# Prisma-Multimodal/ViT-Prisma

Measured on NVIDIA H100. Metric: SAE training tokens/sec (TopK SAE, d_model=768, dict=768x32, k=32), higher is better.
Workload: dtype fp32

## Files before the change

include/prisma_b200.h:

```cpp
#ifndef PRISMA_B200_H
#define PRISMA_B200_H

#include <stdint.h>

#ifdef __cplusplus
extern "C" {
#endif

typedef struct CUstream_st* pb_stream_t;

#if defined(__GNUC__)
#define PB_API __attribute__((visibility("default")))
#else
#define PB_API
#endif

enum { PB_OK = 0, PB_EINVAL = -1, PB_ECUDA = -2, PB_EUNSUPPORTED = -3, PB_ENODEVICE = -4 };
enum { PB_F32 = 0, PB_BF16 = 1 };
enum { PB_ACT_NONE = 0, PB_ACT_RELU = 1, PB_ACT_GELU = 2, PB_ACT_SILU = 3, PB_ACT_GELU_NEW = 4,
       PB_ACT_GELU_FAST = 5, PB_ACT_QUICK_GELU = 6, PB_ACT_TANH_RELU = 7, PB_ACT_EXP = 8 };
enum { PB_GEMM_AUTO = 0, PB_GEMM_SIMT = 1, PB_GEMM_TC = 2 };

PB_API int pb_version(void);
PB_API const char* pb_last_error(void);
PB_API unsigned long long pb_launch_count(void);
PB_API int pb_device_info(int* sm_count, int* cc_major, int* cc_minor);
PB_API int pb_abi_sizeof(int which);

typedef struct {
  int32_t M, N, K;
  int32_t dtype, act, impl;
  const void* A;  int64_t lda;
  const void* B;  int64_t ldb;
  const void* A_lo; const void* B_lo;
  const void* bias;
  const void* residual; int64_t ldr;
  void* out0; int64_t ld0;
  void* out1; int64_t ld1;
  float* out1_lo;
  int32_t n_split, split_n;
  void* out_split[4];
} PbGemm;
PB_API int pb_gemm(const PbGemm* g, pb_stream_t stream);
PB_API int pb_split_tf32(const float* x, float* lo, int64_t n, pb_stream_t stream);

typedef struct {
  int64_t rows; int32_t cols;
  int32_t dtype_in, dtype_out;
  float eps;
  const void* x; const void* w; const void* b;
  float* scale; float* norm_f32; void* out; float* out_lo;
  const float* scale_in;
} PbLayerNorm;
PB_API int pb_layernorm(const PbLayerNorm* p, pb_stream_t stream);

typedef struct {
  int32_t B, T, H, dh, dtype;
  float attn_scale;
  const void* q; const void* k; const void* v;
  void* scores; void* pattern; void* z;
} PbAttention;
PB_API int pb_attention(const PbAttention* p, pb_stream_t stream);
PB_API int pb_attn_scores(const PbAttention* p, pb_stream_t stream);
PB_API int pb_softmax_rows(const void* x, void* y, int64_t rows, int32_t cols, int32_t dtype,
                    pb_stream_t stream);
PB_API int pb_attn_pv(const PbAttention* p, pb_stream_t stream);

PB_API int pb_add(const void* a, const void* b, void* out, int64_t n, int32_t dtype, pb_stream_t s);
PB_API int pb_mul(const void* a, const void* b, void* out, int64_t n, int32_t dtype, pb_stream_t s);
PB_API int pb_activation(const void* x, void* y, int64_t n, int32_t act, int32_t dtype, pb_stream_t s);
PB_API int pb_l2_normalize_rows(const void* x, void* out, int64_t rows, int32_t cols, float eps,
                         int32_t dtype, pb_stream_t s);
PB_API int pb_mean_tokens(const void* x, void* out, int32_t B, int32_t T, int32_t d, int32_t dtype,
                   pb_stream_t s);
PB_API int pb_im2col_patches(const void* images, void* patches, int32_t B, int32_t C, int32_t S,
                      int32_t P, int32_t dtype, pb_stream_t s);
PB_API int pb_embed_assemble(const void* embed, const void* cls, const void* pos, void* full,
                      int32_t B, int32_t n_patches, int32_t d, int32_t use_cls, int32_t dtype,
                      pb_stream_t s);
PB_API int pb_cast(const void* x, int32_t dtype_in, void* y, int32_t dtype_out, int64_t n, pb_stream_t s);

typedef struct {
  const void *ln1_w, *ln1_b, *wqkv, *wqkv_lo, *bqkv, *wo, *wo_lo, *bo;
  const void *ln2_w, *ln2_b, *win, *win_lo, *bin, *wout, *wout_lo, *bout;
} PbVitLayerW;

typedef struct {
  float* ln1_scale;  float* ln1_norm_f32;  void* ln1_out;
  void *q, *k, *v;
  void *scores, *pattern;
  void* z;
  void* attn_out;    void* resid_mid;
  float* ln2_scale;  float* ln2_norm_f32;  void* ln2_out;
  void* pre;         void* post;
  void* mlp_out;     void* resid_post;
} PbVitLayerSpill;

typedef struct {
  int32_t batch, n_channels, image_size, patch_size, n_patches, n_tokens;
  int32_t d_model, n_heads, d_head, d_mlp, n_classes;
  int32_t n_layers_run;
  int32_t run_head;
  int32_t use_cls, layer_norm_pre, normalize_output, head_proj ;
  int32_t pool_gaap;
  int32_t act, dtype, gemm_impl;
  float eps, attn_scale;
  const void* images;
  const void *patch_w, *patch_w_lo, *patch_b, *cls, *pos;
  const void *lnpre_w, *lnpre_b, *lnf_w, *lnf_b, *head_w, *head_w_lo, *head_b;
  const PbVitLayerW* layers_host;
  void* patches;
  void* embed;
  void* full_embed;
  float* lnpre_scale; float* lnpre_norm_f32; void* lnpre_out;
  const PbVitLayerSpill* spills_host;
  float* lnf_scale; float* lnf_norm_f32; void* lnf_out;
  void* pooled;
  void* pre_normalize;
  void* out;
  float* lo_scratch;
} PbVitForward;
PB_API int pb_vit_forward(const PbVitForward* f, pb_stream_t stream);

typedef struct {
  int32_t rows, d, F, k;
  int32_t norm_mode;
  int32_t training;
  int32_t step;
  int32_t renorm_decoder;
  float lr, beta1, beta2, adam_eps, max_grad_norm ;
  const float* x;
  float* W_encT; float* W_encT_lo ; float* W_dec; float* b_enc; float* b_dec;
  float *sae_in, *mu, *sd, *xsum;
  int32_t* idx; float* val;
  float* feat_count;
  float *sae_out, *g, *dval;
  int32_t *csc_off, *csc_cursor, *csc_entries;
  float *gW_dec, *gW_encT, *gb_enc, *gb_dec;
  float *gcol, *gbdec2;
  float* fired;
  void* scalars;
  float *m_dec, *v_dec, *m_enc, *v_enc, *m_be, *v_be, *m_bd, *v_bd;
  float* since_fired; float* act_freq;
  int32_t global_rows; int32_t dist;
  void* work; int64_t work_bytes;
  float* enc_norm_max;
  int32_t pre_zeroed;
} PbSaeStep;

PB_API int pb_sae_prep(const float* x, const float* b_dec, float* sae_in, float* sae_in_lo, float* mu, float* sd,
                       float* xsum, int32_t rows, int32_t d, int32_t norm_mode, pb_stream_t stream);
PB_API int pb_sae_topk(const float* hidden_pre, int32_t rows, int32_t F, int32_t k, int32_t* idx, float* val,
                       float* feat_count, void* scratch, int64_t scratch_bytes, pb_stream_t stream);
PB_API int pb_sae_scatter_acts(const int32_t* idx, const float* val, float* dense, int32_t rows, int32_t k, int32_t F,
                               int32_t relu, pb_stream_t stream);
PB_API int pb_sae_step_reset(const PbSaeStep* s, int32_t* fb_count, pb_stream_t stream);
PB_API int pb_sae_decode(const PbSaeStep* s, pb_stream_t stream);
PB_API int pb_sae_backward(const PbSaeStep* s, pb_stream_t stream);
PB_API int pb_sae_adam(const PbSaeStep* s, pb_stream_t stream);
PB_API int pb_sae_mse(const float* x, const float* out, float* xsum_scratch, float* result, int32_t rows, int32_t d,
                      pb_stream_t stream);
PB_API int pb_unit_norm_rows(float* W, float* W_lo, int32_t F, int32_t d, pb_stream_t stream);

typedef struct {
  int32_t rows, d, F, k;
  int32_t c_keep;
  int32_t m_cand;
  int32_t phases;
  float err_coef;
  const float* sae_in;
  const float* W_encT;
  const float* b_enc;
  const float* enc_norm_max;
  int32_t* cand; int64_t cand_bytes;
  int32_t* idx; float* val;
  float* feat_count;
  int32_t* fb_count;
  int32_t* fb_rows;
  float* fb_scratch; int64_t fb_scratch_bytes;
} PbSaeEncode;
PB_API int pb_sae_fused_workspace(int32_t rows, int32_t F, int32_t c_keep, int64_t* cand_bytes, int64_t* fb_scratch_bytes);
PB_API int pb_sae_encode_topk_fused(const PbSaeEncode* e, pb_stream_t stream);
PB_API int pb_rownorm_max(const float* W, int32_t F, int32_t d, float* out, pb_stream_t stream);

PB_API int pb_transpose(const float* in, float* out, float* out_lo, int32_t rows, int32_t cols, pb_stream_t stream);
PB_API int pb_colsum(const float* x, float* out, int32_t rows, int32_t cols, int32_t accumulate, pb_stream_t stream);
PB_API int pb_gemv_rows(const float* W, const float* v, float* out, int32_t F, int32_t d, int32_t accumulate, pb_stream_t stream);
PB_API int pb_sae_dense_stats(const float* acts, int32_t rows, int32_t F, float* fired, float* l1_sum, void* scalars, pb_stream_t stream);
PB_API int pb_sae_dense_loss(const float* x, const float* out_n, const float* mu, const float* sd, const float* xsum, float* sae_out,
                             float* g, float* resid, void* scalars, int32_t rows, int32_t global_rows, int32_t d, int32_t norm_mode,
                             pb_stream_t stream);
PB_API int pb_sae_dense_dhid(float* d_acts, const float* acts, float* lo, float l1_grad, int64_t n, pb_stream_t stream);
PB_API int pb_sae_grad_finish(const float* gW_dec, const float* gW_encT, const float* gb_enc, const float* gb_dec, int32_t F, int32_t d,
                              void* scalars, float max_grad_norm, int32_t rows, pb_stream_t stream);
PB_API int pb_sae_ghost_gather(const float* hidden_pre, const int32_t* dead_idx, int32_t nd, int32_t rows, int32_t F, float* E, int32_t ldE,
                               pb_stream_t stream);
PB_API int pb_gather_rows(const float* W, const int32_t* idx, int32_t n, int32_t n_pad, int32_t d, float* out, pb_stream_t stream);
PB_API int pb_scatter_add_rows(float* dst, const int32_t* idx, int32_t n, int32_t d, const float* src, float scale, pb_stream_t stream);
PB_API int pb_mul_inplace(float* y, const float* x, int64_t n, pb_stream_t stream);
PB_API int pb_sae_ghost_rows(const float* resid, const float* rsum, float* G0, const void* scalars, float* ghost_sum, int32_t rows,
                             int32_t d, pb_stream_t stream);

PB_API int pb_gated_fwd(const float* pi, const float* b_gate, const float* r_mag, const float* b_mag, float* acts, float* acts_lo,
                        float* pi_act, float* pi_act_lo, float* fired, float* piact_colsum, void* scalars, int32_t rows, int32_t F,
                        pb_stream_t stream);
PB_API int pb_gated_aux(const float* via, const float* sae_in, float* ga, float* aux_sum, int32_t rows, int32_t d, pb_stream_t stream);
PB_API int pb_gated_bwd(float* d_acts, float* D_lo, const float* d_pia, const float* pi, const float* b_gate, const float* r_mag,
                        const float* b_mag, const float* wnorm, float l1_grad, float* gb_gate, float* gb_mag, float* gr_mag, float* dsum,
                        int32_t rows, int32_t F, pb_stream_t stream);
PB_API int pb_row_norms(const float* W, float* out, int32_t F, int32_t d, pb_stream_t stream);
PB_API int pb_gated_l1_rows(float* gW_dec, const float* W_dec, const float* piact_colsum, const float* wnorm, float l1_grad, float* l1_sum,
                            int32_t F, int32_t d, pb_stream_t stream);
PB_API int pb_sumsq(const float* a, int64_t n, float* acc, pb_stream_t stream);
PB_API int pb_sae_clip_finish(void* scalars, float max_grad_norm, int32_t rows, int32_t d, pb_stream_t stream);
PB_API int pb_adam_vec(float* p, const float* g, float* m, float* v, int32_t n, const void* scalars, float lr, float beta1, float beta2,
                       float eps, int32_t step, pb_stream_t stream);

#define PB_P2P_MAX_RANKS 8
typedef struct {
  int32_t rank, world, d, F, step, global_rows;
  float lr, beta1, beta2, adam_eps, max_grad_norm;
  float* gW_dec[PB_P2P_MAX_RANKS]; float* gW_encT[PB_P2P_MAX_RANKS]; float* gb_enc[PB_P2P_MAX_RANKS]; float* gb_dec[PB_P2P_MAX_RANKS];
  float* fired[PB_P2P_MAX_RANKS]; float* xsum[PB_P2P_MAX_RANKS];
  float* W_dec[PB_P2P_MAX_RANKS]; float* W_encT[PB_P2P_MAX_RANKS]; float* W_encT_lo[PB_P2P_MAX_RANKS]; float* b_enc[PB_P2P_MAX_RANKS];
  float* norm_parts[PB_P2P_MAX_RANKS]; uint32_t* flags[PB_P2P_MAX_RANKS];
  float *gb_enc_red, *gb_dec_red, *fired_red, *part_accum;
  float* b_dec; void* scalars;
  float *m_dec, *v_dec, *m_enc, *v_enc, *m_be, *v_be, *m_bd, *v_bd;
  float* since_fired; float* act_freq;
  const float *mc_gW_dec, *mc_gW_encT;
  float *mc_W_dec, *mc_W_encT, *mc_b_enc;
  int32_t defer_dec;
} PbP2PStep;
PB_API int pb_p2p_alloc(int64_t bytes, void** dev_ptr, unsigned char* handle64);
PB_API int pb_p2p_open(const unsigned char* handle64, void** peer_ptr);
PB_API int pb_p2p_close(void* peer_ptr);
PB_API int pb_p2p_free(void* dev_ptr);
PB_API int pb_p2p_barrier(const PbP2PStep* s, uint32_t epoch, pb_stream_t stream);
PB_API int pb_p2p_sum_xsum(const PbP2PStep* s, float* xsum_global, pb_stream_t stream);
PB_API int pb_p2p_reduce_scatter(const PbP2PStep* s, pb_stream_t stream);
PB_API int pb_p2p_adam_allgather(const PbP2PStep* s, pb_stream_t stream);
PB_API int pb_p2p_wmax(const PbP2PStep* s, float* enc_norm_max, pb_stream_t stream);
PB_API int pb_p2p_push_dec(const PbP2PStep* s, pb_stream_t stream);
PB_API int pb_mc_supported(int32_t* supported);
PB_API int pb_mc_round_size(int32_t world, int64_t bytes, int64_t* rounded);
PB_API int pb_mc_create(int32_t world, int64_t bytes, uint64_t* mc_handle, int32_t* fd);
PB_API int pb_mc_import(int32_t fd, uint64_t* mc_handle);
PB_API int pb_mc_add_device(uint64_t mc_handle);
PB_API int pb_mc_bind_alloc(uint64_t mc_handle, int64_t bytes, void** uc_ptr, void** mc_ptr, uint64_t* mem_handle);

#ifdef __cplusplus
}
#endif
#endif
```

vit-prisma_b200/csrc/common.cuh:

```cuda
#pragma once
#include <cuda_runtime.h>
#include <cuda_bf16.h>
#include <stdint.h>
#include <stdio.h>
#include <string.h>
#include <math.h>
#include "../../include/prisma_b200.h"

void pb_set_error(const char* fmt, ...);

#define PB_CHECK_ARG(cond, ...)                                   \
  do {                                                            \
    if (!(cond)) {                                                \
      pb_set_error(__VA_ARGS__);                                  \
      return PB_EINVAL;                                           \
    }                                                             \
  } while (0)

#define PB_CUDA(call)                                                                  \
  do {                                                                                 \
    cudaError_t e__ = (call);                                                          \
    if (e__ != cudaSuccess) {                                                          \
      pb_set_error("%s:%d: %s -> %s", __FILE__, __LINE__, #call, cudaGetErrorString(e__)); \
      return PB_ECUDA;                                                                 \
    }                                                                                  \
  } while (0)

extern unsigned long long g_pb_launches;

#define PB_LAUNCH_CHECK()                                                              \
  do {                                                                                 \
    ++g_pb_launches;                                                                   \
    cudaError_t e__ = cudaGetLastError();                                              \
    if (e__ != cudaSuccess) {                                                          \
      pb_set_error("%s:%d: kernel launch -> %s", __FILE__, __LINE__, cudaGetErrorString(e__)); \
      return PB_ECUDA;                                                                 \
    }                                                                                  \
  } while (0)

#define PB_TRY(expr)                \
  do {                              \
    int rc__ = (expr);              \
    if (rc__ != PB_OK) return rc__; \
  } while (0)

int pb_sm_count();

typedef __nv_bfloat16 bf16;

__device__ __forceinline__ float ld_as_float(const float* p) { return *p; }
__device__ __forceinline__ float ld_as_float(const bf16* p) { return __bfloat162float(*p); }
__device__ __forceinline__ void st_from_float(float* p, float v) { *p = v; }
__device__ __forceinline__ void st_from_float(bf16* p, float v) { *p = __float2bfloat16_rn(v); }
template <typename T> __device__ __forceinline__ float round_to(float v);
template <> __device__ __forceinline__ float round_to<float>(float v) { return v; }
template <> __device__ __forceinline__ float round_to<bf16>(float v) {
  return __bfloat162float(__float2bfloat16_rn(v));
}

struct alignas(8) bf16x4 { __nv_bfloat162 lo, hi; };
__device__ __forceinline__ void ld4(const float* p, float (&v)[4]) {
  float4 t = *reinterpret_cast<const float4*>(p);
  v[0] = t.x; v[1] = t.y; v[2] = t.z; v[3] = t.w;
}
__device__ __forceinline__ void ld4(const bf16* p, float (&v)[4]) {
  bf16x4 t = *reinterpret_cast<const bf16x4*>(p);
  float2 a = __bfloat1622float2(t.lo), b = __bfloat1622float2(t.hi);
  v[0] = a.x; v[1] = a.y; v[2] = b.x; v[3] = b.y;
}
__device__ __forceinline__ void st4(float* p, const float (&v)[4]) {
  *reinterpret_cast<float4*>(p) = make_float4(v[0], v[1], v[2], v[3]);
}
__device__ __forceinline__ void st4(bf16* p, const float (&v)[4]) {
  bf16x4 t;
  t.lo = __floats2bfloat162_rn(v[0], v[1]);
  t.hi = __floats2bfloat162_rn(v[2], v[3]);
  *reinterpret_cast<bf16x4*>(p) = t;
}

__device__ __forceinline__ float tf32_trunc(float x) {
  return __uint_as_float(__float_as_uint(x) & 0xFFFFE000u);
}
__device__ __forceinline__ float tf32_lo(float x) {
  uint32_t r;
  asm("cvt.rna.tf32.f32 %0, %1;" : "=r"(r) : "f"(x - tf32_trunc(x)));
  return __uint_as_float(r);
}

__device__ __forceinline__ float apply_act(float x, int act) {
  switch (act) {
    case PB_ACT_RELU: return fmaxf(x, 0.f);
    case PB_ACT_GELU: return 0.5f * x * (1.f + erff(x * 0.70710678118654752440f));
    case PB_ACT_SILU: return x / (1.f + expf(-x));
    case PB_ACT_GELU_NEW: {
      float inner = 0.79788456080286535588f * (x + 0.044715f * x * x * x);
      return 0.5f * x * (1.f + tanhf(inner));
    }
    case PB_ACT_GELU_FAST: return 0.5f * x * (1.f + tanhf(x * 0.7978845608f * (1.f + 0.044715f * x * x)));
    case PB_ACT_QUICK_GELU: return x / (1.f + expf(-1.702f * x));
    case PB_ACT_TANH_RELU: return tanhf(fmaxf(x, 0.f));
    case PB_ACT_EXP: return expf(x);
    default: return x;
  }
}

__device__ __forceinline__ float warp_sum(float v) {
#pragma unroll
  for (int o = 16; o > 0; o >>= 1) v += __shfl_xor_sync(0xffffffffu, v, o);
  return v;
}
__device__ __forceinline__ float warp_max(float v) {
#pragma unroll
  for (int o = 16; o > 0; o >>= 1) v = fmaxf(v, __shfl_xor_sync(0xffffffffu, v, o));
  return v;
}

static inline int64_t ceil_div64(int64_t a, int64_t b) { return (a + b - 1) / b; }

__device__ __forceinline__ void pb_pdl_trigger() { asm volatile("griddepcontrol.launch_dependents;"); }
__device__ __forceinline__ void pb_pdl_wait() { asm volatile("griddepcontrol.wait;" ::: "memory"); }
__device__ __forceinline__ void pb_pdl() { pb_pdl_trigger(); pb_pdl_wait(); }

bool pb_pdl_enabled();

template <typename... KArgs, typename... Args>
static inline cudaError_t pb_launch_pdl(void (*kern)(KArgs...), dim3 grid, dim3 block, size_t smem, cudaStream_t st, Args&&... args) {
  cudaLaunchConfig_t cfg;
  memset(&cfg, 0, sizeof(cfg));
  cfg.gridDim = grid;
  cfg.blockDim = block;
  cfg.dynamicSmemBytes = smem;
  cfg.stream = st;
  cudaLaunchAttribute attr[1];
  attr[0].id = cudaLaunchAttributeProgrammaticStreamSerialization;
  attr[0].val.programmaticStreamSerializationAllowed = 1;
  cfg.attrs = attr;
  cfg.numAttrs = pb_pdl_enabled() ? 1 : 0;
  return cudaLaunchKernelEx(&cfg, kern, static_cast<KArgs>(args)...);
}
#define PB_LAUNCH_PDL(kern, grid, block, smem, st, ...)                                  \
  do {                                                                                   \
    cudaError_t le__ = pb_launch_pdl(kern, dim3(grid), dim3(block), (size_t)(smem), st, __VA_ARGS__); \
    ++g_pb_launches;                                                                     \
    if (le__ != cudaSuccess) {                                                           \
      pb_set_error("%s:%d: kernel launch -> %s", __FILE__, __LINE__, cudaGetErrorString(le__)); \
      return PB_ECUDA;                                                                   \
    }                                                                                    \
  } while (0)
```

vit-prisma_b200/csrc/p2p.cu:

```cuda
#include "common.cuh"
#include "sae_optim.cuh"

#define PB_MAX_RANKS 8

__device__ __forceinline__ float4 mc_ld_reduce4(const float* mc_addr) {
  float4 v;
  asm volatile("multimem.ld_reduce.relaxed.sys.global.add.v4.f32 {%0, %1, %2, %3}, [%4];"
               : "=f"(v.x), "=f"(v.y), "=f"(v.z), "=f"(v.w)
               : "l"(mc_addr)
               : "memory");
  return v;
}
__device__ __forceinline__ void mc_st4(float* mc_addr, const float (&v)[4]) {
  asm volatile("multimem.st.global.v4.f32 [%0], {%1, %2, %3, %4};" ::"l"(mc_addr), "f"(v[0]), "f"(v[1]), "f"(v[2]), "f"(v[3]) : "memory");
}
__device__ __forceinline__ void mc_st1(float* mc_addr, float v) {
  asm volatile("multimem.st.global.f32 [%0], %1;" ::"l"(mc_addr), "f"(v) : "memory");
}

struct P2PTables {
  int rank, world;
  float* gW_dec[PB_MAX_RANKS];
  float* gW_encT[PB_MAX_RANKS];
  float* gb_enc[PB_MAX_RANKS];
// ... 34 lines not shown
  return PB_OK;
}

__global__ void k_p2p_barrier(P2PTables t, unsigned int epoch) {
  const int r = threadIdx.x;
  if (r < t.world) {
    __threadfence_system();
    asm volatile("st.release.sys.global.u32 [%0], %1;" ::"l"(t.flags[r] + t.rank), "r"(epoch) : "memory");
    const unsigned int* mine = t.flags[t.rank] + r;
    const long long t0 = clock64();
    for (;;) {
      unsigned int v;
      asm volatile("ld.acquire.sys.global.u32 %0, [%1];" : "=r"(v) : "l"(mine) : "memory");
      if ((int)(v - epoch) >= 0) break;
      if (clock64() - t0 > 20000000000LL) {
        printf("p2p barrier timeout: rank %d waiting for rank %d at epoch %u (have %u)\n", t.rank, r, epoch, v);
        __trap();
      }
    }
    __threadfence_system();
  }
}

__global__ void k_p2p_sum_small(P2PTables t, float* __restrict__ out, int which, int n) {
  for (int i = blockIdx.x * blockDim.x + threadIdx.x; i < n; i += gridDim.x * blockDim.x) {
    float acc = 0.f;
    for (int r = 0; r < t.world; ++r) {
      const float* src = which == 0 ? t.xsum[r] : which == 1 ? t.gb_enc[r] : which == 2 ? t.gb_dec[r] : t.fired[r];
      acc += src[i];
    }
    out[i] = acc;
  }
}

__global__ void __launch_bounds__(256) k_p2p_sum_small3(P2PTables t, float* __restrict__ gb_enc_red, float* __restrict__ gb_dec_red,
                                                       float* __restrict__ fired_red, int F, int d, float* __restrict__ part_accum) {
  if (blockIdx.x == 0 && threadIdx.x < 4) part_accum[threadIdx.x] = 0.f;
  const int n = 2 * F + d;
  for (int i = blockIdx.x * blockDim.x + threadIdx.x; i < n; i += gridDim.x * blockDim.x) {
    const int which = i < F ? 0 : i < 2 * F ? 1 : 2;
    const int j = which == 0 ? i : which == 1 ? i - F : i - 2 * F;
    float acc = 0.f;
    for (int r = 0; r < t.world; ++r) acc += (which == 0 ? t.gb_enc[r] : which == 1 ? t.fired[r] : t.gb_dec[r])[j];
    (which == 0 ? gb_enc_red : which == 1 ? fired_red : gb_dec_red)[j] = acc;
  }
}

template <int W, int U>
__device__ __forceinline__ float rs_peer_slice(const P2PTables& t, int m, int64_t base4, int64_t n4, float4* __restrict__ own, int64_t tid,
                                               int64_t stride) {
  const float4* src[W];
#pragma unroll
  for (int j = 0; j < W; ++j) {
    const int r = (t.rank + j) % t.world;
    src[j] = j < t.world ? reinterpret_cast<const float4*>(m == 0 ? t.gW_dec[r] : t.gW_encT[r]) + base4 : nullptr;
  }
  float nsq = 0.f;
  int64_t i = tid;
  for (; i + (U - 1) * stride < n4; i += U * stride) {
    float4 v[U][W];
#pragma unroll
    for (int u = 0; u < U; ++u)
#pragma unroll
      for (int r = 0; r < W; ++r)
        if (r < t.world) v[u][r] = src[r][i + u * stride];
#pragma unroll
    for (int u = 0; u < U; ++u) {
      float4 acc = v[u][0];
#pragma unroll
      for (int r = 1; r < W; ++r)
        if (r < t.world) { acc.x += v[u][r].x; acc.y += v[u][r].y; acc.z += v[u][r].z; acc.w += v[u][r].w; }
      own[i + u * stride] = acc;
      nsq += acc.x * acc.x + acc.y * acc.y + acc.z * acc.z + acc.w * acc.w;
    }
  }
  for (; i < n4; i += stride) {
    float4 acc = src[0][i];
#pragma unroll
    for (int r = 1; r < W; ++r)
      if (r < t.world) { const float4 b = src[r][i]; acc.x += b.x; acc.y += b.y; acc.z += b.z; acc.w += b.w; }
    own[i] = acc;
    nsq += acc.x * acc.x + acc.y * acc.y + acc.z * acc.z + acc.w * acc.w;
  }
  return nsq;
}

template <int W, int U>
__global__ void __launch_bounds__(256, 3) k_p2p_reduce_scatter(P2PTables t, int f0, int f1, int d, const float* __restrict__ gb_enc_red,
                                                              const float* __restrict__ gb_dec_red, int F, float* __restrict__ part_accum,
                                                              const float* __restrict__ mc_gW_dec, const float* __restrict__ mc_gW_encT) {
  const int64_t n4 = (int64_t)(f1 - f0) * d / 4;
  const int64_t base4 = (int64_t)f0 * d / 4;
  float nsq = 0.f;
  const int64_t tid = (int64_t)blockIdx.x * blockDim.x + threadIdx.x, stride = (int64_t)gridDim.x * blockDim.x;
  for (int m = 0; m < 2; ++m) {
    float4* own = reinterpret_cast<float4*>(m == 0 ? t.gW_dec[t.rank] : t.gW_encT[t.rank]) + base4;
    const float* mc = m == 0 ? mc_gW_dec : mc_gW_encT;
    if constexpr (W == 0) {
      const float* src = mc + 4 * base4;
      int64_t i = tid;
      for (; i + 3 * stride < n4; i += 4 * stride) {
        const float4 a0 = mc_ld_reduce4(src + 4 * i), a1 = mc_ld_reduce4(src + 4 * (i + stride)), a2 = mc_ld_reduce4(src + 4 * (i + 2 * stride)),
                     a3 = mc_ld_reduce4(src + 4 * (i + 3 * stride));
        own[i] = a0; own[i + stride] = a1; own[i + 2 * stride] = a2; own[i + 3 * stride] = a3;
        nsq += a0.x * a0.x + a0.y * a0.y + a0.z * a0.z + a0.w * a0.w + a1.x * a1.x + a1.y * a1.y + a1.z * a1.z + a1.w * a1.w +
               a2.x * a2.x + a2.y * a2.y + a2.z * a2.z + a2.w * a2.w + a3.x * a3.x + a3.y * a3.y + a3.z * a3.z + a3.w * a3.w;
      }
      for (; i < n4; i += stride) {
        const float4 a = mc_ld_reduce4(src + 4 * i);
        own[i] = a;
        nsq += a.x * a.x + a.y * a.y + a.z * a.z + a.w * a.w;
      }
      continue;
    }
    if constexpr (W != 0) nsq += rs_peer_slice<W, U>(t, m, base4, n4, own, tid, stride);
  }
  if (t.rank == 0) {
    for (int i = blockIdx.x * blockDim.x + threadIdx.x; i < F; i += gridDim.x * blockDim.x) nsq += gb_enc_red[i] * gb_enc_red[i];
    for (int i = blockIdx.x * blockDim.x + threadIdx.x; i < d; i += gridDim.x * blockDim.x) nsq += gb_dec_red[i] * gb_dec_red[i];
  }
  nsq = warp_sum(nsq);
  __shared__ float red[8];
  if ((threadIdx.x & 31) == 0) red[threadIdx.x >> 5] = nsq;
  __syncthreads();
  if (threadIdx.x == 0) {
    float a = 0.f;
    for (int i = 0; i < 8; ++i) a += red[i];
    atomicAdd(part_accum, a);
  }
}
__global__ void k_p2p_publish_norm(P2PTables t, float* part_accum) {
  const int r = threadIdx.x;
  if (r < t.world) t.norm_parts[r][t.rank] = *part_accum;
}

__global__ void k_p2p_finalize(P2PTables t, SaeScalars* sc, float max_norm, float inv_elems_global, float inv_rows_global) {
  float tot = 0.f;
  for (int r = 0; r < t.world; ++r) tot += t.norm_parts[t.rank][r];
  sae_publish_scalars(sc, tot, max_norm, inv_elems_global, inv_rows_global);
}

struct AdamPeerOut {
  float* const (&wdec_rot)[PB_MAX_RANKS];
  float* const (&wenc_rot)[PB_MAX_RANKS];
  float* const (&wlo_rot)[PB_MAX_RANKS];
  float *own_dec, *mc_W_dec, *mc_W_encT;
  int world, defer_dec;
  int64_t base;
  __device__ __forceinline__ void dec(int c4, const float (&w)[4]) const {
    if (defer_dec) st4(own_dec + base + 4 * c4, w);
    else if (mc_W_dec) mc_st4(mc_W_dec + base + 4 * c4, w);
    else for (int j = 0; j < world; ++j) st4(wdec_rot[j] + base + 4 * c4, w);
  }
  __device__ __forceinline__ void enc(int c4, const float (&p)[4], const float (&lo)[4]) const {
    if (mc_W_encT) {
      mc_st4(mc_W_encT + base + 4 * c4, p);
    } else {
      for (int j = 0; j < world; ++j) {
        st4(wenc_rot[j] + base + 4 * c4, p);
        if (wlo_rot[j]) st4(wlo_rot[j] + base + 4 * c4, lo);
      }
    }
  }
};

template <int CHUNKS>
__global__ void __launch_bounds__(256) k_p2p_adam_allgather(P2PTables t, int f0, int f1, int d, const float* __restrict__ gb_enc_red,
                                                           float* __restrict__ m_dec, float* __restrict__ v_dec, float* __restrict__ m_enc,
                                                           float* __restrict__ v_enc, float* __restrict__ m_be, float* __restrict__ v_be,
                                                           const SaeScalars* __restrict__ sc, AdamHyper h, float* __restrict__ mc_W_dec,
                                                           float* __restrict__ mc_W_encT, float* __restrict__ mc_b_enc, float* __restrict__ wmax_accum,
                                                           int defer_dec) {
  const int lane = threadIdx.x & 31, warp = threadIdx.x >> 5, nw = blockDim.x >> 5;
  float enc_best = 0.f, enc_best_lo = 0.f;
  const int nvec = d >> 2;
  const float clip = sc->clip_coef;
  float* W_dec = t.W_dec[t.rank];
  float* W_encT = t.W_encT[t.rank];
  const float* gWd = t.gW_dec[t.rank];
  const float* gWe = t.gW_encT[t.rank];
  float *wdec_rot[PB_MAX_RANKS], *wenc_rot[PB_MAX_RANKS], *wlo_rot[PB_MAX_RANKS];
#pragma unroll
  for (int j = 0; j < PB_MAX_RANKS; ++j) {
    const int r = (t.rank + j) % t.world;
    wdec_rot[j] = t.W_dec[r]; wenc_rot[j] = t.W_encT[r]; wlo_rot[j] = t.W_encT_lo[r];
  }
  for (int f = f0 + blockIdx.x * nw + warp; f < f1; f += gridDim.x * nw) {
    const int64_t base = (int64_t)f * d;
    float esq, elo;
    sae_adam_feature<CHUNKS>(W_dec + base, gWd + base, m_dec + base, v_dec + base, W_encT + base, gWe + base, m_enc + base, v_enc + base,
                             clip, h, nvec, true,
                             AdamPeerOut{wdec_rot, wenc_rot, wlo_rot, W_dec, mc_W_dec, mc_W_encT, t.world, defer_dec, base}, esq, elo);
    enc_best = fmaxf(enc_best, warp_sum(esq));
    enc_best_lo = fmaxf(enc_best_lo, warp_sum(elo));
    if (lane == 0) {
      float mm = m_be[f], vv = v_be[f];
      const float nb = adam_update(t.b_enc[t.rank][f], gb_enc_red[f] * clip, mm, vv, h);
      m_be[f] = mm;
      v_be[f] = vv;
      if (mc_b_enc) mc_st1(mc_b_enc + f, nb);
      else for (int r = 0; r < t.world; ++r) t.b_enc[r][f] = nb;
    }
  }
  if (wmax_accum && lane == 0 && enc_best > 0.f) {
    atomicMax(reinterpret_cast<unsigned int*>(wmax_accum), __float_as_uint(sqrtf(enc_best)));
    atomicMax(reinterpret_cast<unsigned int*>(wmax_accum) + 1, __float_as_uint(sqrtf(enc_best_lo)));
  }
}

__global__ void k_p2p_wmax_reduce(P2PTables t, float* __restrict__ enc_norm_max) {
  float a = 0.f, b = 0.f;
  for (int r = 0; r < t.world; ++r) {
    a = fmaxf(a, t.norm_parts[t.rank][PB_MAX_RANKS + r]);
    b = fmaxf(b, t.norm_parts[t.rank][2 * PB_MAX_RANKS + r]);
  }
  enc_norm_max[0] = a;
  enc_norm_max[1] = b;
}

__global__ void __launch_bounds__(256) k_p2p_small_updates(P2PTables t, const float* __restrict__ wmax_accum, float* __restrict__ b_dec,
                                                          const float* __restrict__ gb_dec_red, float* __restrict__ m_bd,
                                                          float* __restrict__ v_bd, const float* __restrict__ fired_red,
                                                          float* __restrict__ since_fired, float* __restrict__ act_freq,
                                                          const SaeScalars* __restrict__ sc, AdamHyper h, int d, int F) {
  if (blockIdx.x == 0 && threadIdx.x < t.world) {
    t.norm_parts[threadIdx.x][PB_MAX_RANKS + t.rank] = wmax_accum[0];
    t.norm_parts[threadIdx.x][2 * PB_MAX_RANKS + t.rank] = wmax_accum[1];
  }
  const float clip = sc->clip_coef;
  for (int i = blockIdx.x * blockDim.x + threadIdx.x; i < max(F, d); i += gridDim.x * blockDim.x) {
    if (i < d) {
      float mm = m_bd[i], vv = v_bd[i];
      b_dec[i] = adam_update(b_dec[i], gb_dec_red[i] * clip, mm, vv, h);
      m_bd[i] = mm;
      v_bd[i] = vv;
    }
    if (i < F) dead_feature_counters(since_fired, act_freq, i, fired_red[i], since_fired ? since_fired[i] : 0.f, act_freq ? act_freq[i] : 0.f);
  }
}

static int fill_tables(const PbP2PStep* s, P2PTables* t) {
  PB_CHECK_ARG(s && s->world >= 1 && s->world <= PB_MAX_RANKS && s->rank >= 0 && s->rank < s->world, "pb_p2p: bad rank/world");
  t->rank = s->rank;
  t->world = s->world;
  for (int r = 0; r < s->world; ++r) {
    t->gW_dec[r] = s->gW_dec[r]; t->gW_encT[r] = s->gW_encT[r]; t->gb_enc[r] = s->gb_enc[r]; t->gb_dec[r] = s->gb_dec[r];
    t->fired[r] = s->fired[r]; t->xsum[r] = s->xsum[r]; t->W_dec[r] = s->W_dec[r]; t->W_encT[r] = s->W_encT[r];
    t->W_encT_lo[r] = s->W_encT_lo[r]; t->b_enc[r] = s->b_enc[r]; t->norm_parts[r] = s->norm_parts[r]; t->flags[r] = s->flags[r];
  }
  return PB_OK;
}

extern "C" int pb_p2p_barrier(const PbP2PStep* s, uint32_t epoch, pb_stream_t stream) {
  P2PTables t;
  PB_TRY(fill_tables(s, &t));
  k_p2p_barrier<<<1, 32, 0, (cudaStream_t)stream>>>(t, epoch);
  PB_LAUNCH_CHECK();
  return PB_OK;
}

extern "C" int pb_p2p_sum_xsum(const PbP2PStep* s, float* xsum_global, pb_stream_t stream) {
  P2PTables t;
  PB_TRY(fill_tables(s, &t));
  k_p2p_sum_small<<<(s->d + 255) / 256, 256, 0, (cudaStream_t)stream>>>(t, xsum_global, 0, s->d);
  PB_LAUNCH_CHECK();
  return PB_OK;
}

extern "C" int pb_p2p_reduce_scatter(const PbP2PStep* s, pb_stream_t stream) {
  P2PTables t;
  PB_TRY(fill_tables(s, &t));
  PB_CHECK_ARG(s->gb_enc_red && s->gb_dec_red && s->fired_red && s->part_accum, "pb_p2p_reduce_scatter: reduction buffers missing");
  PB_CHECK_ARG((s->F % s->world) == 0 && (((int64_t)(s->F / s->world) * s->d) % 4) == 0, "pb_p2p_reduce_scatter: F must divide evenly by world");
  cudaStream_t st = (cudaStream_t)stream;
  const int per = s->F / s->world, f0 = s->rank * per, f1 = f0 + per;
  k_p2p_sum_small3<<<(2 * s->F + s->d + 255) / 256, 256, 0, st>>>(t, s->gb_enc_red, s->gb_dec_red, s->fired_red, s->F, s->d, s->part_accum);
  PB_LAUNCH_CHECK();
  PB_CHECK_ARG(!s->mc_gW_dec == !s->mc_gW_encT, "pb_p2p_reduce_scatter: both multicast gradient views or none");
#define PB_RS(W_, U_) k_p2p_reduce_scatter<W_, U_><<<pb_sm_count() * 3, 256, 0, st>>>(t, f0, f1, s->d, s->gb_enc_red, s->gb_dec_red, s->F, s->part_accum, s->mc_gW_dec, s->mc_gW_encT)
  if (s->mc_gW_dec) PB_RS(0, 0);
  else if (s->world == 2) PB_RS(2, 4);
  else if (s->world == 4) PB_RS(4, 2);
  else if (s->world == 8) PB_RS(8, 1);
  else PB_RS(PB_MAX_RANKS, 1);
#undef PB_RS
  PB_LAUNCH_CHECK();
  k_p2p_publish_norm<<<1, 32, 0, st>>>(t, s->part_accum);
  PB_LAUNCH_CHECK();
  return PB_OK;
}

extern "C" int pb_p2p_adam_allgather(const PbP2PStep* s, pb_stream_t stream) {
  P2PTables t;
  PB_TRY(fill_tables(s, &t));
  PB_CHECK_ARG(s->m_dec && s->v_dec && s->m_enc && s->v_enc && s->m_be && s->v_be && s->m_bd && s->v_bd && s->scalars && s->b_dec,
               "pb_p2p_adam_allgather: optimizer state missing");
  PB_CHECK_ARG(s->step >= 1, "pb_p2p_adam_allgather: step counter starts at 1");
  cudaStream_t st = (cudaStream_t)stream;
  const int per = s->F / s->world, f0 = s->rank * per, f1 = f0 + per;
  const AdamHyper h = adam_hyper(s->lr, s->beta1, s->beta2, s->adam_eps, s->step);
  k_p2p_finalize<<<1, 1, 0, st>>>(t, (SaeScalars*)s->scalars, s->max_grad_norm, 1.f / ((float)s->global_rows * (float)s->d),
                                  1.f / (float)s->global_rows);
  PB_LAUNCH_CHECK();
  const int d = s->d;
  int grid = pb_sm_count() * 4;
  if (grid > (per + 7) / 8) grid = (per + 7) / 8;
  PB_CHECK_ARG((!s->mc_W_dec == !s->mc_W_encT) && (!s->mc_W_dec == !s->mc_b_enc), "pb_p2p_adam_allgather: all three multicast parameter views or none");
  PB_DISPATCH_CHUNKS(chunks_for(d), (k_p2p_adam_allgather<C_><<<grid, 256, 0, st>>>(t, f0, f1, d, s->gb_enc_red, s->m_dec, s->v_dec, s->m_enc,
                                     s->v_enc, s->m_be, s->v_be, (const SaeScalars*)s->scalars, h, s->mc_W_dec, s->mc_W_encT, s->mc_b_enc,
                                     s->part_accum + 1, s->defer_dec)));
  PB_LAUNCH_CHECK();
  k_p2p_small_updates<<<((s->F > d ? s->F : d) + 255) / 256, 256, 0, st>>>(t, s->part_accum + 1, s->b_dec, s->gb_dec_red, s->m_bd, s->v_bd, s->fired_red, s->since_fired,
                                                        s->act_freq, (const SaeScalars*)s->scalars, h, d, s->F);
  PB_LAUNCH_CHECK();
  return PB_OK;
}

__global__ void __launch_bounds__(256) k_p2p_push_dec(P2PTables t, int f0, int f1, int d, float* __restrict__ mc_W_dec) {
  const int64_t n4 = (int64_t)(f1 - f0) * d / 4, base4 = (int64_t)f0 * d / 4;
  const float4* own = reinterpret_cast<const float4*>(t.W_dec[t.rank]) + base4;
  for (int64_t i = (int64_t)blockIdx.x * blockDim.x + threadIdx.x; i < n4; i += (int64_t)gridDim.x * blockDim.x) {
    const float4 v = own[i];
    if (mc_W_dec) {
      const float w[4] = {v.x, v.y, v.z, v.w};
      mc_st4(mc_W_dec + 4 * (base4 + i), w);
    } else {
      for (int j = 1; j < t.world; ++j)
        (reinterpret_cast<float4*>(t.W_dec[(t.rank + j) % t.world]) + base4)[i] = v;
    }
  }
}

extern "C" int pb_p2p_push_dec(const PbP2PStep* s, pb_stream_t stream) {
  P2PTables t;
  PB_TRY(fill_tables(s, &t));
  const int per = s->F / s->world, f0 = s->rank * per, f1 = f0 + per;
  k_p2p_push_dec<<<pb_sm_count() * 2, 256, 0, (cudaStream_t)stream>>>(t, f0, f1, s->d, s->mc_W_dec);
  PB_LAUNCH_CHECK();
  return PB_OK;
}

extern "C" int pb_p2p_wmax(const PbP2PStep* s, float* enc_norm_max, pb_stream_t stream) {
  P2PTables t;
  PB_TRY(fill_tables(s, &t));
  PB_CHECK_ARG(enc_norm_max, "pb_p2p_wmax: output missing");
// ... 8 lines not shown
```

vit-prisma_b200/csrc/sae.cu:

```cuda
#include "common.cuh"
#include "tc_common.cuh"
#include "sae_optim.cuh"

template <int CHUNKS>
__global__ void __launch_bounds__(256) k_sae_prep(const float* __restrict__ x, const float* __restrict__ b_dec, float* __restrict__ sae_in,
                                                  float* __restrict__ sae_in_lo, float* __restrict__ mu_out, float* __restrict__ std_out,
                                                  int rows, int d, int norm_mode, float eps) {
  pb_pdl();
  const int lane = threadIdx.x & 31;
  const int row = blockIdx.x * (blockDim.x >> 5) + (threadIdx.x >> 5);
  if (row >= rows) return;
  const int nvec = d >> 2;
  const float* xr = x + (int64_t)row * d;
  float v[CHUNKS][4];
  float sum = 0.f;
#pragma unroll
  for (int i = 0; i < CHUNKS; ++i) {
    const int c4 = i * 32 + lane;
    if (c4 < nvec) { ld4(xr + 4 * c4, v[i]); sum += (v[i][0] + v[i][1]) + (v[i][2] + v[i][3]); }
    else v[i][0] = v[i][1] = v[i][2] = v[i][3] = 0.f;
  }
  float mu = 0.f, inv = 1.f, sd = 1.f;
  if (norm_mode == 1) {
    mu = warp_sum(sum) / (float)d;
    float sq = 0.f;
#pragma unroll
    for (int i = 0; i < CHUNKS; ++i) {
      const int c4 = i * 32 + lane;
      if (c4 < nvec) {
#pragma unroll
        for (int j = 0; j < 4; ++j) { v[i][j] -= mu; sq += v[i][j] * v[i][j]; }
      }
    }
    sd = sqrtf(warp_sum(sq) / (float)(d - 1));
    inv = 1.f / (sd + eps);
  } else if (norm_mode == 2) {
    float sq = 0.f;
#pragma unroll
    for (int i = 0; i < CHUNKS; ++i)
#pragma unroll
      for (int j = 0; j < 4; ++j) sq += v[i][j] * v[i][j];
    sd = sqrtf(warp_sum(sq)) / sqrtf((float)d);
    inv = 1.f / sd;
  }
  if (lane == 0) {
    if (mu_out) mu_out[row] = mu;
    if (std_out) std_out[row] = sd;
  }
#pragma unroll
  for (int i = 0; i < CHUNKS; ++i) {
    const int c4 = i * 32 + lane;
    if (c4 < nvec) {
      float bd[4], o[4], lo[4];
      ld4(b_dec + 4 * c4, bd);
#pragma unroll
      for (int j = 0; j < 4; ++j) {
        o[j] = (norm_mode == 1 ? v[i][j] / (sd + eps) : v[i][j] * inv) - bd[j];
        lo[j] = tf32_lo(o[j]);
      }
      (void)inv;
      st4(sae_in + (int64_t)row * d + 4 * c4, o);
      if (sae_in_lo) st4(sae_in_lo + (int64_t)row * d + 4 * c4, lo);
    }
  }
}

__global__ void __launch_bounds__(256) k_colsum(const float* __restrict__ x, float* __restrict__ out, int rows, int d, int rows_per_cta) {
  pb_pdl();
  const int r0 = blockIdx.x * rows_per_cta, r1 = min(rows, r0 + rows_per_cta);
  for (int c = threadIdx.x; c < d; c += blockDim.x) {
    float acc = 0.f;
    for (int r = r0; r < r1; ++r) acc += x[(int64_t)r * d + c];
    atomicAdd(out + c, acc);
  }
}

__device__ __forceinline__ bool key_gt(float va, int ia, float vb, int ib) { return va > vb || (va == vb && ia < ib); }

template <int IPT>
__global__ void __launch_bounds__(256) k_topk(const float* __restrict__ vals, const int* __restrict__ idx_map, int64_t row_stride, int F,
                                              int seg_len, int k, int* __restrict__ out_idx, float* __restrict__ out_val,
                                              int64_t out_row_stride, float* __restrict__ feat_count, int cand_cap) {
  extern __shared__ __align__(16) unsigned char smem_raw[];
  float* best_v = reinterpret_cast<float*>(smem_raw);
  int* best_i = reinterpret_cast<int*>(best_v + 256);
  float* cand_v = reinterpret_cast<float*>(best_i + 256);
  int* cand_i = reinterpret_cast<int*>(cand_v + cand_cap);
  __shared__ float tau_v;
  __shared__ int tau_i, cand_n;
  const int t = threadIdx.x;
  const int row = blockIdx.x, seg = blockIdx.y;
  const int s0 = seg * seg_len, s1 = min(F, s0 + seg_len);
  const float* vr = vals + (int64_t)row * row_stride;
  const int* mr = idx_map ? idx_map + (int64_t)row * row_stride : nullptr;

  float v[IPT];
  float bv = -INFINITY;
  int bi = 0x7fffffff;
#pragma unroll
  for (int i = 0; i < IPT; ++i) {
    const int p = s0 + t + 256 * i;
    v[i] = p < s1 ? vr[p] : -INFINITY;
    const int gi = p < s1 ? (mr ? mr[p] : p) : 0x7fffffff;
    if (key_gt(v[i], gi, bv, bi)) { bv = v[i]; bi = gi; }
  }
  best_v[t] = bv;
  best_i[t] = bi;
  if (t == 0) cand_n = 0;
  __syncthreads();
  {
    int rank = 0;
    for (int j = 0; j < 256; ++j) rank += key_gt(best_v[j], best_i[j], bv, bi) ? 1 : 0;
    const int kk = min(k, 256);
    if (rank == kk - 1) { tau_v = bv; tau_i = bi; }
  }
  __syncthreads();
  const float tv = tau_v;
  const int ti = tau_i;
#pragma unroll
  for (int i = 0; i < IPT; ++i) {
    const int p = s0 + t + 256 * i;
    if (p < s1) {
      const int gi = mr ? mr[p] : p;
      if (!key_gt(tv, ti, v[i], gi)) {
        const int slot = atomicAdd(&cand_n, 1);
        if (slot < cand_cap) { cand_v[slot] = v[i]; cand_i[slot] = gi; }
      }
    }
  }
  __syncthreads();
  const int C = min(cand_n, cand_cap);
  for (int c = t; c < C; c += 256) {
    const float cv = cand_v[c];
    const int ci = cand_i[c];
    int rank = 0;
    for (int j = 0; j < C; ++j) rank += key_gt(cand_v[j], cand_i[j], cv, ci) ? 1 : 0;
    if (rank < k) {
      const int64_t o = (int64_t)row * out_row_stride + (int64_t)seg * k + rank;
      out_idx[o] = ci;
      out_val[o] = cv;
      if (feat_count) atomicAdd(feat_count + ci, 1.0f);
    }
  }
  if (C < k) {
    for (int r = C + t; r < k; r += 256) {
      const int64_t o = (int64_t)row * out_row_stride + (int64_t)seg * k + r;
      out_idx[o] = 0x7fffffff;
      out_val[o] = -INFINITY;
    }
  }
}

__global__ void __launch_bounds__(256) k_scatter_acts(const int* __restrict__ idx, const float* __restrict__ val, float* __restrict__ dense,
                                                      int rows, int k, int F, int relu) {
  const int64_t n = (int64_t)rows * k;
  for (int64_t e = (int64_t)blockIdx.x * blockDim.x + threadIdx.x; e < n; e += (int64_t)gridDim.x * blockDim.x) {
    const int r = (int)(e / k);
    float v = val[e];
    if (relu) v = fmaxf(v, 0.f);
    dense[(int64_t)r * F + idx[e]] = v;
  }
}

template <int CHUNKS>
__global__ void __launch_bounds__(256) k_sae_decode(const float* __restrict__ x, const float* __restrict__ xsum, const float* __restrict__ mu,
                                                    const float* __restrict__ sd, const int* __restrict__ idx, const float* __restrict__ val,
                                                    const float* __restrict__ W_dec, const float* __restrict__ b_dec,
                                                    float* __restrict__ sae_out, float* __restrict__ g_out, float* __restrict__ dval,
                                                    SaeScalars* __restrict__ sc, int rows, int d, int k, int norm_mode, int training,
                                                    float inv_rows) {
  pb_pdl();
  const int lane = threadIdx.x & 31;
  const int row = blockIdx.x * (blockDim.x >> 5) + (threadIdx.x >> 5);
  const bool active = row < rows;
  const int nvec = d >> 2;
  float loss_part = 0.f, pos_part = 0.f;
  if (active) {
    const int* ir = idx + (int64_t)row * k;
    const float* vr = val + (int64_t)row * k;
    float acc[CHUNKS][4];
#pragma unroll
    for (int i = 0; i < CHUNKS; ++i) {
      const int c4 = i * 32 + lane;
      if (c4 < nvec) ld4(b_dec + 4 * c4, acc[i]);
      else acc[i][0] = acc[i][1] = acc[i][2] = acc[i][3] = 0.f;
    }
    for (int j0 = 0; j0 < k; j0 += 32) {
      const int jn = min(32, k - j0);
      const int my_i = lane < jn ? ir[j0 + lane] : 0;
      const float my_a = lane < jn ? fmaxf(vr[j0 + lane], 0.f) : 0.f;
      pos_part += (float)__popc(__ballot_sync(0xffffffffu, my_a > 0.f));
#pragma unroll 4
      for (int j = 0; j < jn; ++j) {
        const float a = __shfl_sync(0xffffffffu, my_a, j);
        const float* wr = W_dec + (int64_t)__shfl_sync(0xffffffffu, my_i, j) * d;
#pragma unroll
        for (int i = 0; i < CHUNKS; ++i) {
          const int c4 = i * 32 + lane;
          if (c4 < nvec) {
            float w[4];
            ld4(wr + 4 * c4, w);
#pragma unroll
            for (int q = 0; q < 4; ++q) acc[i][q] = fmaf(a, w[q], acc[i][q]);
          }
        }
      }
    }
    const float m = norm_mode ? mu[row] : 0.f;
    const float s = norm_mode ? sd[row] : 1.f;
    float nsq = 0.f;
    float e[CHUNKS][4];
#pragma unroll
    for (int i = 0; i < CHUNKS; ++i) {
      const int c4 = i * 32 + lane;
      if (c4 < nvec) {
// ... 256 lines not shown
    const int c4 = i * 32 + lane;
    if (c4 < nvec) {
#pragma unroll
      for (int q = 0; q < 4; ++q)
        if (bd[i][q] != 0.f) atomicAdd(&sm_bd[4 * c4 + q], bd[i][q]);
    }
  }
  nsq = warp_sum(nsq);
  __shared__ float red[8];
  if (lane == 0) red[warp] = nsq;
  __syncthreads();
  if (threadIdx.x == 0) {
    float a = 0.f;
    for (int i = 0; i < nw; ++i) a += red[i];
    atomicAdd(&sc->gnorm_sq, a);
  }
  for (int c = threadIdx.x; c < d; c += blockDim.x)
    if (sm_bd[c] != 0.f) atomicAdd(gbdec2 + c, sm_bd[c]);
}

template <int CHUNKS>
__global__ void __launch_bounds__(256) k_sae_grads_long(const int* __restrict__ off, const int* __restrict__ entries, const float* __restrict__ val,
                                                        const float* __restrict__ dval, const float* __restrict__ g,
                                                        const float* __restrict__ sae_in, const float* __restrict__ W_encT,
                                                        float* __restrict__ gW_dec, float* __restrict__ gW_encT, float* __restrict__ gb_enc,
                                                        float* __restrict__ gbdec2, float* __restrict__ fired, int d, int k,
                                                        const SaeWorkHeader* __restrict__ work, const int* __restrict__ work_chunks) {
  pb_pdl();
  extern __shared__ __align__(16) float sm_bd[];
  const int lane = threadIdx.x & 31, warp = threadIdx.x >> 5, nw = blockDim.x >> 5;
  const int nvec = d >> 2;
  const int n_items = work->n_chunks;
  if (n_items == 0) return;
  for (int c = threadIdx.x; c < d; c += blockDim.x) sm_bd[c] = 0.f;
  __syncthreads();
  float bd[CHUNKS][4];
#pragma unroll
  for (int i = 0; i < CHUNKS; ++i) bd[i][0] = bd[i][1] = bd[i][2] = bd[i][3] = 0.f;
  for (int item = blockIdx.x * nw + warp; item < n_items; item += gridDim.x * nw) {
    const int f = work_chunks[2 * item], p0 = work_chunks[2 * item + 1];
    const int p1 = min(off[f + 1], p0 + SAE_LONG_CHUNK);
    float ad[CHUNKS][4], ae[CHUNKS][4];
#pragma unroll
    for (int i = 0; i < CHUNKS; ++i) ad[i][0] = ad[i][1] = ad[i][2] = ad[i][3] = ae[i][0] = ae[i][1] = ae[i][2] = ae[i][3] = 0.f;
    const int n = p1 - p0;
    int my_b = 0;
    float my_a = 0.f, my_dp = 0.f;
    if (lane < n) {
      const int e = entries[p0 + lane];
      my_b = e / k;
      my_a = fmaxf(val[e], 0.f);
      my_dp = dval[e];
    }
    float gbe = 0.f;
    const float npos = (float)__popc(__ballot_sync(0xffffffffu, my_a > 0.f));
#pragma unroll 2
    for (int j = 0; j < n; ++j) {
      const float a = __shfl_sync(0xffffffffu, my_a, j), dp = __shfl_sync(0xffffffffu, my_dp, j);
      const int b = __shfl_sync(0xffffffffu, my_b, j);
      gbe += dp;
      const float* gr = g + (int64_t)b * d;
      const float* sr = sae_in + (int64_t)b * d;
#pragma unroll
      for (int i = 0; i < CHUNKS; ++i) {
        const int c4 = i * 32 + lane;
        if (c4 < nvec) {
          float gv[4], sv[4];
          ld4(gr + 4 * c4, gv);
          ld4(sr + 4 * c4, sv);
#pragma unroll
          for (int q = 0; q < 4; ++q) { ad[i][q] = fmaf(a, gv[q], ad[i][q]); ae[i][q] = fmaf(dp, sv[q], ae[i][q]); }
        }
      }
    }
#pragma unroll
    for (int i = 0; i < CHUNKS; ++i) {
      const int c4 = i * 32 + lane;
      if (c4 < nvec) {
        atomicAdd(reinterpret_cast<float4*>(gW_dec + (int64_t)f * d + 4 * c4), make_float4(ad[i][0], ad[i][1], ad[i][2], ad[i][3]));
        atomicAdd(reinterpret_cast<float4*>(gW_encT + (int64_t)f * d + 4 * c4), make_float4(ae[i][0], ae[i][1], ae[i][2], ae[i][3]));
        if (gbe != 0.f) {
          float w[4];
          ld4(W_encT + (int64_t)f * d + 4 * c4, w);
#pragma unroll
          for (int q = 0; q < 4; ++q) bd[i][q] = fmaf(gbe, w[q], bd[i][q]);
        }
      }
    }
    if (lane == 0) {
      atomicAdd(gb_enc + f, gbe);
      atomicAdd(fired + f, npos);
    }
  }
#pragma unroll
  for (int i = 0; i < CHUNKS; ++i) {
    const int c4 = i * 32 + lane;
    if (c4 < nvec) {
#pragma unroll
      for (int q = 0; q < 4; ++q)
        if (bd[i][q] != 0.f) atomicAdd(&sm_bd[4 * c4 + q], bd[i][q]);
    }
  }
  __syncthreads();
  for (int c = threadIdx.x; c < d; c += blockDim.x)
    if (sm_bd[c] != 0.f) atomicAdd(gbdec2 + c, sm_bd[c]);
}

__global__ void __launch_bounds__(256) k_sae_norm_long(const float* __restrict__ gW_dec, const float* __restrict__ gW_encT,
                                                       const float* __restrict__ gb_enc, SaeScalars* __restrict__ sc, int d,
                                                       const SaeWorkHeader* work, const int* __restrict__ work_feats) {
  pb_pdl();
  const int lane = threadIdx.x & 31, warp = threadIdx.x >> 5, nw = blockDim.x >> 5;
  const int n = *reinterpret_cast<const volatile int*>(&work->n_long);
  float nsq = 0.f;
  for (int li = blockIdx.x * nw + warp; li < n; li += gridDim.x * nw) {
    const int f = work_feats[li];
    for (int c = lane; c < d; c += 32) {
      const float a = gW_dec[(int64_t)f * d + c], b = gW_encT[(int64_t)f * d + c];
      nsq += a * a + b * b;
    }
    if (lane == 0) nsq += gb_enc[f] * gb_enc[f];
  }
  nsq = warp_sum(nsq);
  if (lane == 0 && nsq != 0.f) atomicAdd(&sc->gnorm_sq, nsq);
}

__global__ void k_sae_gbdec(const float* __restrict__ gcol, const float* __restrict__ gbdec2, float* __restrict__ gb_dec, int d) {
  const int c = blockIdx.x * blockDim.x + threadIdx.x;
  if (c < d) gb_dec[c] = gcol[c] - gbdec2[c];
}

__global__ void __launch_bounds__(256) k_sae_finalize(const float* __restrict__ gcol, const float* __restrict__ gbdec2, float* __restrict__ gb_dec,
                                                      SaeScalars* __restrict__ sc, int d, float max_norm, float inv_elems, float inv_rows) {
  pb_pdl();
  __shared__ float red[8];
  float s = 0.f;
  for (int c = threadIdx.x; c < d; c += blockDim.x) {
    const float v = gcol[c] - gbdec2[c];
    gb_dec[c] = v;
    s += v * v;
  }
  s = warp_sum(s);
  if ((threadIdx.x & 31) == 0) red[threadIdx.x >> 5] = s;
  __syncthreads();
  if (threadIdx.x == 0) {
    float t = sc->gnorm_sq;
    for (int i = 0; i < 8; ++i) t += red[i];
    sae_publish_scalars(sc, t, max_norm, inv_elems, inv_rows);
  }
}

struct AdamRowsOut {
  float *W_dec, *W_encT, *W_encT_lo;
  int64_t base;
  __device__ __forceinline__ void dec(int c4, const float (&w)[4]) const { st4(W_dec + base + 4 * c4, w); }
  __device__ __forceinline__ void enc(int c4, const float (&p)[4], const float (&lo)[4]) const {
    st4(W_encT + base + 4 * c4, p);
    if (W_encT_lo) st4(W_encT_lo + base + 4 * c4, lo);
  }
};

template <int CHUNKS>
__global__ void __launch_bounds__(256) k_sae_adam_rows(float* __restrict__ W_dec, float* __restrict__ W_encT, float* __restrict__ W_encT_lo,
                                                       float* __restrict__ b_enc, const float* __restrict__ gW_dec,
                                                       const float* __restrict__ gW_encT, const float* __restrict__ gb_enc,
                                                       float* __restrict__ m_dec, float* __restrict__ v_dec, float* __restrict__ m_enc,
                                                       float* __restrict__ v_enc, float* __restrict__ m_be, float* __restrict__ v_be,
                                                       const float* __restrict__ fired, float* __restrict__ since_fired,
                                                       float* __restrict__ act_freq, const SaeScalars* __restrict__ sc, AdamHyper h,
                                                       int F, int d, int renorm, float* __restrict__ enc_norm_max) {
  const int lane = threadIdx.x & 31, warp = threadIdx.x >> 5, nw = blockDim.x >> 5;
  const int nvec = d >> 2;
  const float clip = sc->clip_coef;
  float enc_best = 0.f, enc_best_lo = 0.f;
  for (int f = blockIdx.x * nw + warp; f < F; f += gridDim.x * nw) {
    const int64_t base = (int64_t)f * d;
    float esq, elo;
    sae_adam_feature<CHUNKS>(W_dec + base, gW_dec + base, m_dec + base, v_dec + base, W_encT + base, gW_encT + base, m_enc + base,
                             v_enc + base, clip, h, nvec, renorm, AdamRowsOut{W_dec, W_encT, W_encT_lo, base}, esq, elo);
    if (enc_norm_max) { enc_best = fmaxf(enc_best, warp_sum(esq)); enc_best_lo = fmaxf(enc_best_lo, warp_sum(elo)); }
    if (lane == 0) {
      float mm = m_be[f], vv = v_be[f];
      b_enc[f] = adam_update(b_enc[f], gb_enc[f] * clip, mm, vv, h);
      m_be[f] = mm;
      v_be[f] = vv;
      dead_feature_counters(since_fired, act_freq, f, fired[f], since_fired ? since_fired[f] : 0.f, act_freq ? act_freq[f] : 0.f);
    }
  }
  if (enc_norm_max && lane == 0 && enc_best > 0.f) {
    atomicMax(reinterpret_cast<unsigned int*>(enc_norm_max), __float_as_uint(sqrtf(enc_best)));
    atomicMax(reinterpret_cast<unsigned int*>(enc_norm_max) + 1, __float_as_uint(sqrtf(enc_best_lo)));
  }
}

constexpr int AB_MAX_STAGES = 12;
constexpr int AB_THREADS = 32 * (1 + AB_MAX_STAGES);

struct AdamSlotOut {
  float *wd, *we;
  __device__ __forceinline__ void dec(int c4, const float (&w)[4]) const { st4(wd + 4 * c4, w); }
  __device__ __forceinline__ void enc(int c4, const float (&p)[4], const float (&)[4]) const { st4(we + 4 * c4, p); }
};

__device__ __forceinline__ void bulk_load(uint32_t dst, const void* src, uint32_t bytes, uint32_t bar) {
  asm volatile("cp.async.bulk.shared::cluster.global.mbarrier::complete_tx::bytes [%0], [%1], %2, [%3];" ::"r"(dst), "l"(src), "r"(bytes), "r"(bar)
               : "memory");
}
__device__ __forceinline__ void bulk_store(void* dst, uint32_t src, uint32_t bytes) {
  asm volatile("cp.async.bulk.global.shared::cta.bulk_group [%0], [%1], %2;" ::"l"(dst), "r"(src), "r"(bytes) : "memory");
}

template <int CHUNKS>
__global__ void __launch_bounds__(AB_THREADS, 1)
k_sae_adam_bulk(float* __restrict__ W_dec, float* __restrict__ W_encT, float* __restrict__ b_enc, const float* __restrict__ gW_dec,
                const float* __restrict__ gW_encT, const float* __restrict__ gb_enc, float* __restrict__ m_dec, float* __restrict__ v_dec,
                float* __restrict__ m_enc, float* __restrict__ v_enc, float* __restrict__ m_be, float* __restrict__ v_be,
                const float* __restrict__ fired, float* __restrict__ since_fired, float* __restrict__ act_freq,
                const SaeScalars* __restrict__ sc, AdamHyper h, int F, int d, int renorm, float* __restrict__ enc_norm_max, int S,
                float* __restrict__ b_dec, const float* __restrict__ gb_dec, float* __restrict__ m_bd, float* __restrict__ v_bd) {
  pb_pdl_trigger();
  extern __shared__ __align__(128) unsigned char ab_smem[];
  const uint32_t s0 = smem_u32(ab_smem);
  const uint32_t row_bytes = (uint32_t)d * 4u, stage_bytes = 8u * row_bytes;
  auto full_bar = [&](int s) { return s0 + 8u * s; };
  auto empty_bar = [&](int s) { return s0 + 8u * (S + s); };
  const uint32_t data0 = s0 + 256u;
  float* data_generic = reinterpret_cast<float*>(ab_smem + 256);
  const int warp = threadIdx.x >> 5, lane = threadIdx.x & 31;
  const int n_mine = F > (int)blockIdx.x ? (F - (int)blockIdx.x + (int)gridDim.x - 1) / (int)gridDim.x : 0;
  if (threadIdx.x == 0) {
    for (int s = 0; s < S; ++s) { mbar_init(full_bar(s), 1); mbar_init(empty_bar(s), 1); }
    asm volatile("fence.mbarrier_init.release.cluster;" ::: "memory");
  }
  __syncthreads();
  pb_pdl_wait();
  if (warp == 0) {
    if (blockIdx.x == 0 && b_dec) {
      const float clip0 = sc->clip_coef;
      for (int c = lane; c < d; c += 32) {
        float mm = m_bd[c], vv = v_bd[c];
        b_dec[c] = adam_update(b_dec[c], gb_dec[c] * clip0, mm, vv, h);
        m_bd[c] = mm;
        v_bd[c] = vv;
      }
    }
    if (lane == 0) {
      for (int i = 0; i < n_mine; ++i) {
        const int s = i % S;
        const uint32_t ph = (uint32_t)(i / S) & 1u;
        const int64_t base = (int64_t)(blockIdx.x + (int64_t)i * gridDim.x) * d;
        mbar_wait(empty_bar(s), ph ^ 1u);
        mbar_expect_tx(full_bar(s), stage_bytes);
        const uint32_t dst = data0 + (uint32_t)s * stage_bytes;
        bulk_load(dst + 0 * row_bytes, W_dec + base, row_bytes, full_bar(s));
        bulk_load(dst + 1 * row_bytes, gW_dec + base, row_bytes, full_bar(s));
        bulk_load(dst + 2 * row_bytes, m_dec + base, row_bytes, full_bar(s));
        bulk_load(dst + 3 * row_bytes, v_dec + base, row_bytes, full_bar(s));
        bulk_load(dst + 4 * row_bytes, W_encT + base, row_bytes, full_bar(s));
        bulk_load(dst + 5 * row_bytes, gW_encT + base, row_bytes, full_bar(s));
        bulk_load(dst + 6 * row_bytes, m_enc + base, row_bytes, full_bar(s));
        bulk_load(dst + 7 * row_bytes, v_enc + base, row_bytes, full_bar(s));
      }
    }
    return;
  }
  const int nvec = d >> 2;
  const float clip = sc->clip_coef;
  float enc_best = 0.f, enc_best_lo = 0.f;
  for (int i = warp - 1; i < n_mine; i += S) {
    const int s = i % S;
    const uint32_t ph = (uint32_t)(i / S) & 1u;
    const int f = blockIdx.x + i * gridDim.x;
    const int64_t base = (int64_t)f * d;
    float be = 0.f, gbe = 0.f, mbe = 0.f, vbe = 0.f, fr = 0.f, sf = 0.f, af = 0.f;
    if (lane == 0) {
      be = b_enc[f]; gbe = gb_enc[f]; mbe = m_be[f]; vbe = v_be[f]; fr = fired[f];
      if (since_fired) sf = since_fired[f];
      if (act_freq) af = act_freq[f];
    }
    mbar_wait(full_bar(s), ph);
    float* st = data_generic + (size_t)s * 8 * d;
    float esq, elo;
    sae_adam_feature<CHUNKS>(st, st + d, st + 2 * d, st + 3 * d, st + 4 * d, st + 5 * d, st + 6 * d, st + 7 * d, clip, h, nvec, renorm,
                             AdamSlotOut{st, st + 4 * d}, esq, elo);
    enc_best = fmaxf(enc_best, warp_sum(esq));
    enc_best_lo = fmaxf(enc_best_lo, warp_sum(elo));
    __syncwarp();
    asm volatile("fence.proxy.async.shared::cta;" ::: "memory");
    __syncwarp();
    if (lane == 0) {
      const uint32_t src = data0 + (uint32_t)s * stage_bytes;
      bulk_store(W_dec + base, src + 0 * row_bytes, row_bytes);
      bulk_store(m_dec + base, src + 2 * row_bytes, row_bytes);
      bulk_store(v_dec + base, src + 3 * row_bytes, row_bytes);
      bulk_store(W_encT + base, src + 4 * row_bytes, row_bytes);
      bulk_store(m_enc + base, src + 6 * row_bytes, row_bytes);
      bulk_store(v_enc + base, src + 7 * row_bytes, row_bytes);
      asm volatile("cp.async.bulk.commit_group;" ::: "memory");
      b_enc[f] = adam_update(be, gbe * clip, mbe, vbe, h);
      m_be[f] = mbe;
      v_be[f] = vbe;
      dead_feature_counters(since_fired, act_freq, f, fr, sf, af);
      asm volatile("cp.async.bulk.wait_group.read 0;" ::: "memory");
      mbar_arrive(empty_bar(s));
    }
  }
  if (enc_norm_max && lane == 0 && enc_best > 0.f) {
    atomicMax(reinterpret_cast<unsigned int*>(enc_norm_max), __float_as_uint(sqrtf(enc_best)));
    atomicMax(reinterpret_cast<unsigned int*>(enc_norm_max) + 1, __float_as_uint(sqrtf(enc_best_lo)));
  }
  asm volatile("cp.async.bulk.wait_group 0;" ::: "memory");
}

__global__ void __launch_bounds__(256) k_sae_adam_vec(float* __restrict__ p, const float* __restrict__ g, float* __restrict__ m,
                                                      float* __restrict__ v, const SaeScalars* __restrict__ sc, AdamHyper h, int n) {
  const float clip = sc->clip_coef;
  for (int i = blockIdx.x * blockDim.x + threadIdx.x; i < n; i += gridDim.x * blockDim.x) {
    float mm = m[i], vv = v[i];
    p[i] = adam_update(p[i], g[i] * clip, mm, vv, h);
    m[i] = mm;
    v[i] = vv;
  }
}

template <int CHUNKS>
__global__ void __launch_bounds__(256) k_unit_rows(float* __restrict__ W, float* __restrict__ W_lo, int F, int d) {
  const int lane = threadIdx.x & 31, warp = threadIdx.x >> 5, nw = blockDim.x >> 5;
  const int nvec = d >> 2;
  for (int f = blockIdx.x * nw + warp; f < F; f += gridDim.x * nw) {
    float w[CHUNKS][4];
    float nsq = 0.f;
#pragma unroll
    for (int i = 0; i < CHUNKS; ++i) {
      const int c4 = i * 32 + lane;
      if (c4 < nvec) {
        ld4(W + (int64_t)f * d + 4 * c4, w[i]);
#pragma unroll
        for (int q = 0; q < 4; ++q) nsq += w[i][q] * w[i][q];
      }
    }
    const float nrm = sqrtf(warp_sum(nsq));
#pragma unroll
    for (int i = 0; i < CHUNKS; ++i) {
      const int c4 = i * 32 + lane;
      if (c4 < nvec) {
        float lo[4];
#pragma unroll
        for (int q = 0; q < 4; ++q) { w[i][q] = w[i][q] / nrm; lo[q] = tf32_lo(w[i][q]); }
        st4(W + (int64_t)f * d + 4 * c4, w[i]);
        if (W_lo) st4(W_lo + (int64_t)f * d + 4 * c4, lo);
      }
    }
  }
}

static int persistent_grid(int warps_per_cta, int items) {
  int ctas = pb_sm_count() * 4;
  const int need = (items + warps_per_cta - 1) / warps_per_cta;
  if (ctas > need) ctas = need;
  return ctas < 1 ? 1 : ctas;
}

extern "C" int pb_sae_prep(const float* x, const float* b_dec, float* sae_in, float* sae_in_lo, float* mu, float* sd, float* xsum, int32_t rows,
                           int32_t d, int32_t norm_mode, pb_stream_t stream) {
  PB_CHECK_ARG(x && b_dec && sae_in && rows >= 0 && d > 0, "pb_sae_prep: bad arguments");
  PB_CHECK_ARG(norm_mode == 0 || (mu && sd), "pb_sae_prep: mu/std buffers required when normalising");
  if (rows == 0) return PB_OK;
  cudaStream_t st = (cudaStream_t)stream;
  const int ch = chunks_for(d);
  PB_DISPATCH_CHUNKS(ch, PB_LAUNCH_PDL(k_sae_prep<C_>, (rows + 7) / 8, 256, 0, st, x, b_dec, sae_in, sae_in_lo, mu, sd, rows, d, norm_mode, 1e-5f));
  if (xsum) {
    PB_CUDA(cudaMemsetAsync(xsum, 0, sizeof(float) * d, st));
    const int rpc = 8;
    k_colsum<<<(rows + rpc - 1) / rpc, 256, 0, st>>>(x, xsum, rows, d, rpc);
    PB_LAUNCH_CHECK();
  }
  return PB_OK;
}

static int launch_topk(const float* vals, const int* map, int64_t row_stride, int F, int seg_len, int nseg, int k, int* oi, float* ov,
                       int64_t out_stride, float* feat_count, int rows, cudaStream_t st) {
  const int ipt_needed = (seg_len + 255) / 256;
  const int ipt = ipt_needed <= 8 ? 8 : ipt_needed <= 24 ? 24 : ipt_needed <= 48 ? 48 : 96;
  int cap = ipt * k;
  if (cap > seg_len) cap = seg_len;
  if (cap < k) cap = k;
  const size_t smem = 256 * 8 + (size_t)cap * 8;
  if (smem > 200 * 1024) { pb_set_error("pb_sae_topk: k=%d too large for the candidate buffer", k); return PB_EUNSUPPORTED; }
  dim3 grid(rows, nseg);
#define PB_TOPK(IPT)                                                                                                      \
  do {                                                                                                                    \
    auto kern = k_topk<IPT>;                                                                                              \
    if (smem > 48 * 1024) PB_CUDA(cudaFuncSetAttribute(kern, cudaFuncAttributeMaxDynamicSharedMemorySize, (int)smem));    \
    kern<<<grid, 256, smem, st>>>(vals, map, row_stride, F, seg_len, k, oi, ov, out_stride, feat_count, cap);             \
  } while (0)
  if (ipt == 8) PB_TOPK(8);
  else if (ipt == 24) PB_TOPK(24);
  else if (ipt == 48) PB_TOPK(48);
  else PB_TOPK(96);
#undef PB_TOPK
  PB_LAUNCH_CHECK();
  return PB_OK;
}

extern "C" int pb_sae_topk(const float* hidden_pre, int32_t rows, int32_t F, int32_t k, int32_t* idx, float* val, float* feat_count,
                           void* scratch, int64_t scratch_bytes, pb_stream_t stream) {
  PB_CHECK_ARG(hidden_pre && idx && val && rows >= 0 && F > 0 && k > 0 && k <= F, "pb_sae_topk: bad arguments");
  PB_CHECK_ARG(k <= 256, "pb_sae_topk: k=%d > 256 unsupported", k);
  if (rows == 0) return PB_OK;
  cudaStream_t st = (cudaStream_t)stream;
  const int SEG = 256 * 96;
  if (F <= SEG) return launch_topk(hidden_pre, nullptr, F, F, F, 1, k, idx, val, k, feat_count, rows, st);
  const int nseg = (F + SEG - 1) / SEG;
  const int seg_len = ((F + nseg - 1) / nseg + 255) / 256 * 256;
  const int64_t need = (int64_t)rows * nseg * k * 8;
  PB_CHECK_ARG(scratch && scratch_bytes >= need, "pb_sae_topk: scratch too small (%lld < %lld)", (long long)scratch_bytes, (long long)need);
  int* ci = (int*)scratch;
  float* cv = (float*)(ci + (int64_t)rows * nseg * k);
  PB_TRY(launch_topk(hidden_pre, nullptr, F, F, seg_len, nseg, k, ci, cv, (int64_t)nseg * k, nullptr, rows, st));
  return launch_topk(cv, ci, (int64_t)nseg * k, nseg * k, nseg * k, 1, k, idx, val, k, feat_count, rows, st);
}

extern "C" int pb_sae_scatter_acts(const int32_t* idx, const float* val, float* dense, int32_t rows, int32_t k, int32_t F, int32_t relu,
                                   pb_stream_t stream) {
  PB_CHECK_ARG(idx && val && dense && rows >= 0, "pb_sae_scatter_acts: bad arguments");
  if (rows == 0) return PB_OK;
  cudaStream_t st = (cudaStream_t)stream;
  PB_CUDA(cudaMemsetAsync(dense, 0, sizeof(float) * (size_t)rows * F, st));
  k_scatter_acts<<<pb_sm_count() * 4, 256, 0, st>>>(idx, val, dense, rows, k, F, relu);
  PB_LAUNCH_CHECK();
  return PB_OK;
}

__global__ void k_sae_fwd_scalars(SaeScalars* sc, float inv_elems, float inv_rows) {
  sc->mse = sc->loss_sum * inv_elems;
  sc->l0 = sc->pos_count * inv_rows;
}

__global__ void __launch_bounds__(256) k_sae_step_reset(float* __restrict__ feat_count, int F, float* __restrict__ scalars, float* __restrict__ gcol,
                                                        float* __restrict__ gbdec2, int d, int* __restrict__ work_hdr, int* __restrict__ fb_count) {
  pb_pdl();
  const int i = blockIdx.x * blockDim.x + threadIdx.x;
  for (int f = i; f < F; f += gridDim.x * blockDim.x) feat_count[f] = 0.f;
  if (i < d) { gcol[i] = 0.f; gbdec2[i] = 0.f; }
  if (i < 8) scalars[i] = 0.f;
  if (i < 4 && work_hdr) work_hdr[i] = 0;
  if (i < 2 && fb_count) fb_count[i] = 0;
}

extern "C" int pb_sae_step_reset(const PbSaeStep* s, int32_t* fb_count, pb_stream_t stream) {
  PB_CHECK_ARG(s && s->feat_count && s->scalars && s->gcol && s->gbdec2, "pb_sae_step_reset: missing pointers");
  PB_CHECK_ARG(!s->work || s->work_bytes >= (int64_t)sizeof(SaeWorkHeader), "pb_sae_step_reset: work buffer too small");
  const int n = s->F > s->d ? s->F : s->d;
  int grid = (n + 255) / 256;
  if (grid > pb_sm_count() * 2) grid = pb_sm_count() * 2;
  if (grid * 256 < s->d) grid = (s->d + 255) / 256;
  PB_LAUNCH_PDL(k_sae_step_reset, grid, 256, 0, (cudaStream_t)stream, s->feat_count, s->F, (float*)s->scalars, s->gcol, s->gbdec2, s->d, (int*)s->work, fb_count);
  return PB_OK;
}

extern "C" int pb_sae_decode(const PbSaeStep* s, pb_stream_t stream) {
  PB_CHECK_ARG(s && s->x && s->xsum && s->idx && s->val && s->W_dec && s->b_dec && s->scalars, "pb_sae_decode: missing pointers");
  PB_CHECK_ARG(!s->training || (s->g && s->dval), "pb_sae_decode: training needs g and dval buffers");
  if (s->rows == 0) return PB_OK;
  cudaStream_t st = (cudaStream_t)stream;
  const int d = s->d, ch = chunks_for(d);
  PB_DISPATCH_CHUNKS(ch, PB_LAUNCH_PDL(k_sae_decode<C_>, (s->rows + 7) / 8, 256, 0, st,
      s->x, s->xsum, s->mu, s->sd, s->idx, s->val, s->W_dec, s->b_dec, s->sae_out, s->g, s->dval, (SaeScalars*)s->scalars, s->rows, d, s->k,
      s->norm_mode, s->training, 1.f / (float)(s->global_rows > 0 ? s->global_rows : s->rows)));
  if (!s->training) {
    k_sae_fwd_scalars<<<1, 1, 0, st>>>((SaeScalars*)s->scalars, 1.f / ((float)s->rows * (float)d), 1.f / (float)s->rows);
    PB_LAUNCH_CHECK();
  }
  return PB_OK;
}

extern "C" int pb_sae_backward(const PbSaeStep* s, pb_stream_t stream) {
  PB_CHECK_ARG(s && s->idx && s->val && s->dval && s->g && s->sae_in && s->W_encT && s->feat_count && s->csc_off && s->csc_cursor &&
               s->csc_entries && s->gW_dec && s->gW_encT && s->gb_enc && s->gb_dec && s->gcol && s->gbdec2 && s->fired && s->scalars,
               "pb_sae_backward: missing pointers");
  if (s->rows == 0) return PB_OK;
  cudaStream_t st = (cudaStream_t)stream;
  const int d = s->d, F = s->F, ch = chunks_for(d);
  {
    const int per = ((F + 1023) / 1024 + 3) / 4 * 4;
    PB_CHECK_ARG(per <= 128, "pb_sae_backward: d_sae=%d too large for the offset scan (max 131072)", F);
    if (per <= 8) PB_LAUNCH_PDL(k_scan_counts<8>, 1, 1024, 0, st, s->feat_count, s->csc_off, s->csc_cursor, F);
    else if (per <= 24) PB_LAUNCH_PDL(k_scan_counts<24>, 1, 1024, 0, st, s->feat_count, s->csc_off, s->csc_cursor, F);
    else if (per <= 48) PB_LAUNCH_PDL(k_scan_counts<48>, 1, 1024, 0, st, s->feat_count, s->csc_off, s->csc_cursor, F);
    else if (per <= 64) PB_LAUNCH_PDL(k_scan_counts<64>, 1, 1024, 0, st, s->feat_count, s->csc_off, s->csc_cursor, F);
    else PB_LAUNCH_PDL(k_scan_counts<128>, 1, 1024, 0, st, s->feat_count, s->csc_off, s->csc_cursor, F);
  }
  const int64_t n = (int64_t)s->rows * s->k;
  PB_LAUNCH_PDL(k_csc_fill, pb_sm_count() * 4, 256, 0, st, (const int*)s->idx, s->csc_cursor, s->csc_entries, n);
  if (!s->pre_zeroed) {
    PB_CUDA(cudaMemsetAsync(s->gcol, 0, sizeof(float) * d, st));
    PB_CUDA(cudaMemsetAsync(s->gbdec2, 0, sizeof(float) * d, st));
  }
  const int rpc = 8;
  PB_LAUNCH_PDL(k_colsum, (s->rows + rpc - 1) / rpc, 256, 0, st, (const float*)s->g, s->gcol, s->rows, d, rpc);
  const int64_t cap = n / SAE_LONG_CHUNK + F + 1;
  const int64_t need = (int64_t)sizeof(SaeWorkHeader) + 4 * (int64_t)F + 8 * cap;
  PB_CHECK_ARG(s->work && s->work_bytes >= need, "pb_sae_backward: work buffer too small (%lld < %lld bytes)", (long long)s->work_bytes,
               (long long)need);
  SaeWorkHeader* wh = (SaeWorkHeader*)s->work;
  int* work_feats = (int*)(wh + 1);
  int* work_chunks = work_feats + F;
  if (!s->pre_zeroed) PB_CUDA(cudaMemsetAsync(wh, 0, sizeof(SaeWorkHeader), st));
  const int grid = persistent_grid(8, F);
  PB_DISPATCH_CHUNKS(ch, PB_LAUNCH_PDL(k_sae_grads<C_>, grid, 256, sizeof(float) * d, st, s->csc_off, s->csc_entries, s->val, s->dval, s->g, s->sae_in,
                                       s->W_encT, s->gW_dec, s->gW_encT, s->gb_enc, s->gbdec2, s->fired, (SaeScalars*)s->scalars, F, d, s->k, wh,
                                       work_feats, work_chunks));
  PB_DISPATCH_CHUNKS(ch, PB_LAUNCH_PDL(k_sae_grads_long<C_>, pb_sm_count() * 4, 256, sizeof(float) * d, st, s->csc_off, s->csc_entries, s->val, s->dval,
                                       s->g, s->sae_in, s->W_encT, s->gW_dec, s->gW_encT, s->gb_enc, s->gbdec2, s->fired, d, s->k, wh, work_chunks));
  if (!s->dist) {
    PB_LAUNCH_PDL(k_sae_norm_long, pb_sm_count(), 256, 0, st, s->gW_dec, s->gW_encT, s->gb_enc, (SaeScalars*)s->scalars, d, wh, work_feats);
  }
  if (s->dist) {
    k_sae_gbdec<<<(d + 255) / 256, 256, 0, st>>>(s->gcol, s->gbdec2, s->gb_dec, d);
    PB_LAUNCH_CHECK();
    return PB_OK;
  }
  PB_LAUNCH_PDL(k_sae_finalize, 1, 256, 0, st, s->gcol, s->gbdec2, s->gb_dec, (SaeScalars*)s->scalars, d, s->max_grad_norm,
                1.f / ((float)s->rows * (float)d), 1.f / (float)s->rows);
  return PB_OK;
}

extern "C" int pb_sae_adam(const PbSaeStep* s, pb_stream_t stream) {
  PB_CHECK_ARG(s && s->W_dec && s->W_encT && s->b_enc && s->b_dec && s->gW_dec && s->gW_encT && s->gb_enc && s->gb_dec && s->m_dec &&
               s->v_dec && s->m_enc && s->v_enc && s->m_be && s->v_be && s->m_bd && s->v_bd && s->fired && s->scalars,
               "pb_sae_adam: missing pointers");
  PB_CHECK_ARG(s->step >= 1, "pb_sae_adam: step counter starts at 1");
  cudaStream_t st = (cudaStream_t)stream;
  const int d = s->d, F = s->F, ch = chunks_for(d);
  const AdamHyper h = adam_hyper(s->lr, s->beta1, s->beta2, s->adam_eps, s->step);
  const int grid = persistent_grid(8, F);
  if (s->enc_norm_max) PB_CUDA(cudaMemsetAsync(s->enc_norm_max, 0, 2 * sizeof(float), st));
  if (!s->W_encT_lo && d >= 64) {
    const size_t stage = (size_t)8 * d * 4;
    int S = (int)((200 * 1024) / stage);
    if (S > 12) S = 12;
    if (S >= 3) {
      const size_t smem = 256 + (size_t)S * stage;
      int g2 = pb_sm_count();
      if (g2 > F) g2 = F;
      PB_DISPATCH_CHUNKS(ch, {
        auto kern = k_sae_adam_bulk<C_>;
        PB_CUDA(cudaFuncSetAttribute(kern, cudaFuncAttributeMaxDynamicSharedMemorySize, (int)smem));
        PB_LAUNCH_PDL(kern, g2, 32 * (1 + S), smem, st, s->W_dec, s->W_encT, s->b_enc, s->gW_dec, s->gW_encT, s->gb_enc, s->m_dec, s->v_dec,
                      s->m_enc, s->v_enc, s->m_be, s->v_be, s->fired, s->since_fired, s->act_freq, (const SaeScalars*)s->scalars, h, F, d,
                      s->renorm_decoder, s->enc_norm_max, S, s->b_dec, s->gb_dec, s->m_bd, s->v_bd);
      });
      return PB_OK;
    }
  }
  PB_DISPATCH_CHUNKS(ch, (k_sae_adam_rows<C_><<<grid, 256, 0, st>>>(s->W_dec, s->W_encT, s->W_encT_lo, s->b_enc, s->gW_dec, s->gW_encT, s->gb_enc,
                                                                     s->m_dec, s->v_dec, s->m_enc, s->v_enc, s->m_be, s->v_be, s->fired,
                                                                     s->since_fired, s->act_freq, (const SaeScalars*)s->scalars, h,
                                                                     F, d, s->renorm_decoder, s->enc_norm_max)));
  PB_LAUNCH_CHECK();
  k_sae_adam_vec<<<(d + 255) / 256, 256, 0, st>>>(s->b_dec, s->gb_dec, s->m_bd, s->v_bd, (const SaeScalars*)s->scalars, h, d);
  PB_LAUNCH_CHECK();
  return PB_OK;
}

extern "C" int pb_adam_vec(float* p, const float* g, float* m, float* v, int32_t n, const void* scalars, float lr, float beta1, float beta2,
                           float eps, int32_t step, pb_stream_t stream) {
  PB_CHECK_ARG(p && g && m && v && scalars && n >= 0 && step >= 1, "pb_adam_vec: bad arguments");
  if (n == 0) return PB_OK;
  const int grid = (n + 255) / 256 < pb_sm_count() * 8 ? (n + 255) / 256 : pb_sm_count() * 8;
  k_sae_adam_vec<<<grid, 256, 0, (cudaStream_t)stream>>>(p, g, m, v, (const SaeScalars*)scalars, adam_hyper(lr, beta1, beta2, eps, step), n);
  PB_LAUNCH_CHECK();
  return PB_OK;
}

extern "C" int pb_unit_norm_rows(float* W, float* W_lo, int32_t F, int32_t d, pb_stream_t stream) {
  PB_CHECK_ARG(W && F >= 0 && d > 0, "pb_unit_norm_rows: bad arguments");
  if (F == 0) return PB_OK;
  const int ch = chunks_for(d);
  cudaStream_t st = (cudaStream_t)stream;
  PB_DISPATCH_CHUNKS(ch, (k_unit_rows<C_><<<persistent_grid(8, F), 256, 0, st>>>(W, W_lo, F, d)));
  PB_LAUNCH_CHECK();
  return PB_OK;
}

__global__ void __launch_bounds__(256) k_sae_mse_rows(const float* __restrict__ x, const float* __restrict__ xsum, const float* __restrict__ out,
                                                      float* __restrict__ acc, int rows, int d, float inv_rows) {
  const int lane = threadIdx.x & 31;
  const int row = blockIdx.x * (blockDim.x >> 5) + (threadIdx.x >> 5);
  float part = 0.f;
  if (row < rows) {
    float nsq = 0.f, esq = 0.f;
    for (int c = lane; c < d; c += 32) {
      const float xv = x[(int64_t)row * d + c];
      const float xc = xv - xsum[c] * inv_rows;
      const float e = out[(int64_t)row * d + c] - xv;
      nsq += xc * xc;
      esq += e * e;
    }
    part = warp_sum(esq) / sqrtf(warp_sum(nsq));
  }
  if (lane == 0 && row < rows) atomicAdd(acc, part);
}
__global__ void k_scale_scalar(float* v, float s) { v[0] *= s; }

extern "C" int pb_sae_mse(const float* x, const float* out, float* xsum_scratch, float* result, int32_t rows, int32_t d, pb_stream_t stream) {
  PB_CHECK_ARG(x && out && xsum_scratch && result && rows > 0 && d > 0, "pb_sae_mse: bad arguments");
  cudaStream_t st = (cudaStream_t)stream;
  PB_CUDA(cudaMemsetAsync(xsum_scratch, 0, sizeof(float) * d, st));
  PB_CUDA(cudaMemsetAsync(result, 0, sizeof(float), st));
  const int rpc = 32;
  k_colsum<<<(rows + rpc - 1) / rpc, 256, 0, st>>>(x, xsum_scratch, rows, d, rpc);
  PB_LAUNCH_CHECK();
  k_sae_mse_rows<<<(rows + 7) / 8, 256, 0, st>>>(x, xsum_scratch, out, result, rows, d, 1.f / (float)rows);
  PB_LAUNCH_CHECK();
  k_scale_scalar<<<1, 1, 0, st>>>(result, 1.f / ((float)rows * (float)d));
  PB_LAUNCH_CHECK();
  return PB_OK;
}

int pb_abi_sizeof_p2p(int which);
int pb_abi_sizeof_sae(int which) {
  if (which == 6) return (int)sizeof(PbSaeStep);
  if (which == 7) return (int)sizeof(SaeScalars);
  return pb_abi_sizeof_p2p(which);
}
```

vit-prisma_b200/csrc/sae_fused.cu:

```cuda
#include "tc_common.cuh"
#include "gemm_epi.cuh"
#include <limits.h>

namespace {

__device__ __forceinline__ int f2ord(float v) {
  const int k = __float_as_int(v);
  return k ^ ((k >> 31) & 0x7fffffff);
}
__device__ __forceinline__ float ord2f(int k) { return __int_as_float(k ^ ((k >> 31) & 0x7fffffff)); }
__device__ __forceinline__ bool key_gt_f(float va, int ia, float vb, int ib) { return va > vb || (va == vb && ia < ib); }

constexpr int FZ_SEG = 128;
constexpr int FZ_BM = 128;
constexpr int FZ_BN = 2 * FZ_SEG;
constexpr int FZ_BK = 32;
constexpr int FZ_KSTEPS = 4;
constexpr int FZ_A_BYTES = FZ_BM * 128;
constexpr int FZ_STAGE_BYTES = FZ_A_BYTES + FZ_BN * 128;
constexpr int FZ_STAGES = 4;
constexpr int FZ_SMEM = FZ_STAGES * FZ_STAGE_BYTES + 1024 + 256;

__device__ __forceinline__ void key_cas(int& a, int& b) {
  const int hi = max(a, b);
  b = min(a, b);
  a = hi;
}
__device__ __forceinline__ void key_sort8(int* v) {
  key_cas(v[0], v[2]); key_cas(v[1], v[3]); key_cas(v[4], v[6]); key_cas(v[5], v[7]);
  key_cas(v[0], v[4]); key_cas(v[1], v[5]); key_cas(v[2], v[6]); key_cas(v[3], v[7]);
  key_cas(v[0], v[1]); key_cas(v[2], v[3]); key_cas(v[4], v[5]); key_cas(v[6], v[7]);
  key_cas(v[2], v[4]); key_cas(v[3], v[5]);
  key_cas(v[1], v[4]); key_cas(v[3], v[6]);
  key_cas(v[1], v[2]); key_cas(v[3], v[4]); key_cas(v[5], v[6]);
}
__device__ __forceinline__ void key_merge8(int* a, const int* b) {
#pragma unroll
  for (int i = 0; i < 8; ++i) a[i] = max(a[i], b[7 - i]);
  key_cas(a[0], a[4]); key_cas(a[1], a[5]); key_cas(a[2], a[6]); key_cas(a[3], a[7]);
  key_cas(a[0], a[2]); key_cas(a[1], a[3]); key_cas(a[4], a[6]); key_cas(a[5], a[7]);
  key_cas(a[0], a[1]); key_cas(a[2], a[3]); key_cas(a[4], a[5]); key_cas(a[6], a[7]);
}
__device__ __forceinline__ void key_top8_of32(int (&v)[32]) {
  key_sort8(v); key_sort8(v + 8); key_sort8(v + 16); key_sort8(v + 24);
  key_merge8(v, v + 8);
  key_merge8(v + 16, v + 24);
  key_merge8(v, v + 16);
}

template <int C_KEEP>
__global__ void __launch_bounds__(TC_THREADS, 1)
k_enc_cand(const __grid_constant__ CUtensorMap tmA, const __grid_constant__ CUtensorMap tmB, int K, int M, int N,
           const float* __restrict__ bias, int* __restrict__ cand, int num_m_tiles, int num_n_tiles) {
  pb_pdl_trigger();
  extern __shared__ uint8_t smem_raw[];
  const uint32_t smem0 = smem_u32(smem_raw);
  const uint32_t ring = (smem0 + 1023u) & ~1023u;
  const uint32_t bar_base = ring + FZ_STAGES * FZ_STAGE_BYTES;
  auto full_bar = [&](int s) { return bar_base + 8u * s; };
  auto empty_bar = [&](int s) { return bar_base + 8u * (FZ_STAGES + s); };

  const int warp = threadIdx.x >> 5, lane = threadIdx.x & 31;
  const int wg = warp >> 2;
  const int num_kb = (K + FZ_BK - 1) / FZ_BK;
  const int num_tiles = num_m_tiles * num_n_tiles;
  const int nseg = N / FZ_SEG;
  auto tile_m = [&](int tile) { return tile % num_m_tiles; };
  auto tile_n = [&](int tile) { return tile / num_m_tiles; };

  if (threadIdx.x == 0) {
    prefetch_tmap(&tmA);
    prefetch_tmap(&tmB);
    for (int s = 0; s < FZ_STAGES; ++s) { mbar_init(full_bar(s), 1); mbar_init(empty_bar(s), 2); }
    asm volatile("fence.mbarrier_init.release.cluster;" ::: "memory");
  }
  __syncthreads();
  pb_pdl_wait();

  if (wg == 0) {
    reg_dealloc<40>();
    if (threadIdx.x == 0) {
      uint32_t it = 0;
      for (int tile = blockIdx.x; tile < num_tiles; tile += gridDim.x) {
        const int m0 = tile_m(tile) * FZ_BM, n0 = tile_n(tile) * FZ_BN;
        for (int kb = 0; kb < num_kb; ++kb, ++it) {
          const int s = it % FZ_STAGES;
          const uint32_t ph = (it / FZ_STAGES) & 1;
          mbar_wait<false>(empty_bar(s), ph ^ 1);
          mbar_expect_tx(full_bar(s), FZ_STAGE_BYTES);
          const uint32_t sa = ring + s * FZ_STAGE_BYTES;
          tma_load_2d(sa, &tmA, full_bar(s), kb * FZ_BK, m0);
          tma_load_2d(sa + FZ_A_BYTES, &tmB, full_bar(s), kb * FZ_BK, n0);
        }
      }
    }
    return;
  }
  reg_alloc<232>();
  const int c = wg - 1, wq = warp & 3, tid = threadIdx.x & 127;
  float acc[128];
  uint32_t it = 0;
  for (int tile = blockIdx.x; tile < num_tiles; tile += gridDim.x) {
    const int m0 = tile_m(tile) * FZ_BM, n0 = tile_n(tile) * FZ_BN;
    int prev_s = -1;
    for (int kb = 0; kb < num_kb; ++kb, ++it) {
      const int s = it % FZ_STAGES;
      const uint32_t ph = (it / FZ_STAGES) & 1;
      mbar_wait<false>(full_bar(s), ph);
      const uint32_t sa = ring + s * FZ_STAGE_BYTES + c * 64 * 128;
      const uint32_t sb = ring + s * FZ_STAGE_BYTES + FZ_A_BYTES;
      wgmma_fence();
#pragma unroll
      for (int k = 0; k < FZ_KSTEPS; ++k) wgmma_tf32_n256(acc, make_smem_desc(sa + 32 * k), make_smem_desc(sb + 32 * k), (kb | k) != 0 ? 1u : 0u);
      wgmma_commit();
      wgmma_wait<1>();
      if (prev_s >= 0 && tid == 0) mbar_arrive(empty_bar(prev_s));
      prev_s = s;
    }
    wgmma_wait<0>();
    wgmma_fence_acc(acc);
    if (tid == 0) mbar_arrive(empty_bar(prev_s));

    const int row = m0 + 64 * c + 16 * wq + (lane >> 2);
#pragma unroll
    for (int g = 0; g < 2; ++g) {
      const int f0 = n0 + g * FZ_SEG;
      if (f0 >= N) break;
      int s0[32], s1[32];
#pragma unroll
      for (int j = 0; j < 16; ++j) {
        const int col = 8 * j + 2 * (lane & 3);
        const float2 bb = *reinterpret_cast<const float2*>(bias + f0 + col);
        const float* a = acc + 64 * g + 4 * j;
        s0[2 * j] = (f2ord(a[0] + bb.x) & ~127) | col;
        s0[2 * j + 1] = (f2ord(a[1] + bb.y) & ~127) | (col + 1);
        s1[2 * j] = (f2ord(a[2] + bb.x) & ~127) | col;
        s1[2 * j + 1] = (f2ord(a[3] + bb.y) & ~127) | (col + 1);
      }
      key_top8_of32(s0);
      key_top8_of32(s1);
#pragma unroll
      for (int off = 1; off <= 2; off <<= 1) {
        int t0[8], t1[8];
#pragma unroll
        for (int i = 0; i < 8; ++i) { t0[i] = __shfl_xor_sync(0xffffffffu, s0[i], off); t1[i] = __shfl_xor_sync(0xffffffffu, s1[i], off); }
        key_merge8(s0, t0);
        key_merge8(s1, t1);
      }
      if ((lane & 3) == 0) {
#pragma unroll
        for (int h = 0; h < 2; ++h) {
          const int* sv = h == 0 ? s0 : s1;
          if (row + 8 * h < M) {
            int* dst = cand + ((int64_t)(row + 8 * h) * nseg + f0 / FZ_SEG) * C_KEEP;
            if (C_KEEP % 4 == 0) {
#pragma unroll
              for (int i = 0; i < C_KEEP / 4; ++i) reinterpret_cast<int4*>(dst)[i] = make_int4(sv[4 * i], sv[4 * i + 1], sv[4 * i + 2], sv[4 * i + 3]);
            } else {
#pragma unroll
              for (int i = 0; i < C_KEEP / 2; ++i) reinterpret_cast<int2*>(dst)[i] = make_int2(sv[2 * i], sv[2 * i + 1]);
            }
          }
        }
      }
    }
  }
}

__device__ __forceinline__ float warp_dot(const float4* __restrict__ a4, const float4* __restrict__ w4, int nvec, int lane) {
  float acc = 0.f;
  for (int i = lane; i < nvec; i += 32) {
    const float4 a = a4[i], w = __ldg(w4 + i);
    acc = fmaf(a.x, w.x, acc); acc = fmaf(a.y, w.y, acc); acc = fmaf(a.z, w.z, acc); acc = fmaf(a.w, w.w, acc);
  }
  return warp_sum(acc);
}
__device__ __forceinline__ void warp_dot2(const float4* __restrict__ a4, const float4* __restrict__ w0, const float4* __restrict__ w1, int nvec,
                                          int lane, float& o0, float& o1) {
  float x = 0.f, y = 0.f;
  for (int i = lane; i < nvec; i += 32) {
    const float4 a = a4[i], u = __ldg(w0 + i), v = __ldg(w1 + i);
    x = fmaf(a.x, u.x, x); x = fmaf(a.y, u.y, x); x = fmaf(a.z, u.z, x); x = fmaf(a.w, u.w, x);
    y = fmaf(a.x, v.x, y); y = fmaf(a.y, v.y, y); y = fmaf(a.z, v.z, y); y = fmaf(a.w, v.w, y);
  }
  o0 = warp_sum(x);
  o1 = warp_sum(y);
}

constexpr int SEL_MAX_CAND = 128;
constexpr int SEL_EXTEND = 16;
constexpr int SEL_TAU_RANK = 96;
constexpr int SEL_SLOTS = 512;

__device__ __forceinline__ unsigned long long sel_pack(int key, int pos) {
  return ((unsigned long long)((unsigned)key ^ 0x80000000u) << 32) | (unsigned)(0xFFFFFFFFu - (unsigned)pos);
}
__device__ __forceinline__ int sel_key(unsigned long long it) { return (int)((unsigned)(it >> 32) ^ 0x80000000u); }
__device__ __forceinline__ int sel_pos(unsigned long long it) { return (int)(0xFFFFFFFFu - (unsigned)it); }

template <int SPT>
__global__ void __launch_bounds__(256) k_cand_select(const int* __restrict__ cand, int nseg, int c_keep, const float* __restrict__ sae_in,
                                                     const float* __restrict__ W_encT, const float* __restrict__ b_enc,
                                                     const float* __restrict__ wnorm_max, float err_scale, int d, int k, int m_cand,
                                                     int* __restrict__ out_idx, float* __restrict__ out_val, float* __restrict__ feat_count,
                                                     int* __restrict__ fb_count, int* __restrict__ fb_rows, int* __restrict__ stats) {
  pb_pdl();
  extern __shared__ __align__(16) unsigned char sm_raw[];
  float* a_row = reinterpret_cast<float*>(sm_raw);
  __shared__ unsigned long long items[SEL_SLOTS];
  __shared__ int ex_idx[SEL_MAX_CAND], win_idx[64], warp_tau[8];
  __shared__ float ex_val[SEL_MAX_CAND];
  __shared__ float red[2][8];
  __shared__ int g_n, u_below, sat_key;
  __shared__ float tau_exact, a_norm, a_lo_norm;
  const int t = threadIdx.x, lane = t & 31, warp = t >> 5;
  const int row = blockIdx.x;
  const int nvec = d >> 2;
  const int nkeys = nseg * c_keep;

  {
    const float4* src = reinterpret_cast<const float4*>(sae_in + (int64_t)row * d);
    float4* dst = reinterpret_cast<float4*>(a_row);
    float nsq = 0.f, lsq = 0.f;
    for (int i = t; i < nvec; i += 256) {
      const float4 v = src[i];
      dst[i] = v;
      nsq += v.x * v.x + v.y * v.y + v.z * v.z + v.w * v.w;
      const float lx = v.x - tf32_trunc(v.x), ly = v.y - tf32_trunc(v.y), lz = v.z - tf32_trunc(v.z), lw = v.w - tf32_trunc(v.w);
      lsq += lx * lx + ly * ly + lz * lz + lw * lw;
    }
    nsq = warp_sum(nsq);
    lsq = warp_sum(lsq);
    if (lane == 0) { red[0][warp] = nsq; red[1][warp] = lsq; }
  }
  int key[SPT][8];
  int bk = INT_MIN;
  const int* kr = cand + (int64_t)row * nkeys;
#pragma unroll
  for (int i = 0; i < SPT; ++i) {
    const int sg = t + 256 * i;
#pragma unroll
    for (int j = 0; j < 8; j += 2) {
      int2 v = make_int2(INT_MIN, INT_MIN);
      if (sg < nseg && j < c_keep) v = *reinterpret_cast<const int2*>(kr + sg * c_keep + j);
      key[i][j] = v.x;
      key[i][j + 1] = v.y;
    }
    bk = max(bk, key[i][0]);
  }
  {
    int v = bk;
#pragma unroll
    for (int kk = 2; kk <= 32; kk <<= 1) {
#pragma unroll
      for (int j = kk >> 1; j > 0; j >>= 1) {
        const int o = __shfl_xor_sync(0xffffffffu, v, j);
        const bool keep_max = ((lane & kk) == 0) == ((lane & j) == 0);
        v = keep_max ? max(v, o) : min(v, o);
      }
    }
    const int nthr = min(256, nseg);
    const int m_tau = min(SEL_TAU_RANK, nthr);
    const int cnt_w = max(0, min(32, nthr - 32 * warp));
    const int q_w = (m_tau * cnt_w + nthr - 1) / nthr;
    const int rep = __shfl_sync(0xffffffffu, v, max(q_w - 1, 0));
    if (lane == 0) warp_tau[warp] = q_w > 0 ? rep : INT_MAX;
  }
  if (t == 0) { g_n = 0; u_below = INT_MIN; }
  __syncthreads();
  if (t == 0) {
    float s0 = 0.f, s1 = 0.f;
    for (int i = 0; i < 8; ++i) { s0 += red[0][i]; s1 += red[1][i]; }
    a_norm = sqrtf(s0);
    a_lo_norm = sqrtf(s1);
  }
  int tau = INT_MAX;
#pragma unroll
  for (int w = 0; w < 8; ++w) tau = min(tau, warp_tau[w]);
  int lower = INT_MIN;
#pragma unroll
  for (int i = 0; i < SPT; ++i) {
    const int sg = t + 256 * i;
    if (sg < nseg) {
#pragma unroll
      for (int j = 0; j < 8; ++j) {
        if (j < c_keep) {
          if (key[i][j] >= tau) {
            const int slot = atomicAdd(&g_n, 1);
            if (slot < SEL_SLOTS) items[slot] = sel_pack(key[i][j], sg * c_keep + j);
          } else {
            lower = max(lower, key[i][j]);
          }
        }
      }
    }
  }
  if (lower != INT_MIN) atomicMax(&u_below, lower);
  __syncthreads();
  const bool overflow = g_n > SEL_SLOTS;
  const int G = min(g_n, SEL_SLOTS);
  const int n_sort = G <= 256 ? 256 : SEL_SLOTS;
  for (int i = G + t; i < n_sort; i += 256) items[i] = 0ull;
  __syncthreads();
  for (int kk = 2; kk <= n_sort; kk <<= 1) {
    for (int j = kk >> 1; j > 0; j >>= 1) {
      for (int p = t; p < (n_sort >> 1); p += 256) {
        const int i = 2 * j * (p / j) + (p % j);
        const int o = i + j;
        const unsigned long long x = items[i], y = items[o];
        const bool desc = (i & kk) == 0;
        if ((x < y) == desc) { items[i] = y; items[o] = x; }
      }
      __syncthreads();
    }
  }
  const int Gs = min(G, SEL_MAX_CAND);
  const float4* a4 = reinterpret_cast<const float4*>(a_row);
  int m_prev = 0, m_cur = min(m_cand, Gs);
  bool ok = false;
  for (;;) {
    if (t == 0) sat_key = INT_MIN;
    for (int c = m_prev + 2 * warp; c < m_cur; c += 16) {
      const unsigned long long it0 = items[c];
      const int f0 = (sel_pos(it0) / c_keep) * FZ_SEG + (sel_key(it0) & 127);
      if (c + 1 < m_cur) {
        const unsigned long long it1 = items[c + 1];
        const int f1 = (sel_pos(it1) / c_keep) * FZ_SEG + (sel_key(it1) & 127);
        float v0, v1;
        warp_dot2(a4, reinterpret_cast<const float4*>(W_encT + (int64_t)f0 * d), reinterpret_cast<const float4*>(W_encT + (int64_t)f1 * d), nvec,
                  lane, v0, v1);
        if (lane == 0) { ex_val[c] = v0 + b_enc[f0]; ex_idx[c] = f0; ex_val[c + 1] = v1 + b_enc[f1]; ex_idx[c + 1] = f1; }
      } else {
        const float v0 = warp_dot(a4, reinterpret_cast<const float4*>(W_encT + (int64_t)f0 * d), nvec, lane);
        if (lane == 0) { ex_val[c] = v0 + b_enc[f0]; ex_idx[c] = f0; }
      }
    }
    __syncthreads();
    if (t < m_cur) {
      const float v = ex_val[t];
      const int f = ex_idx[t];
      int rank = 0;
      for (int j = 0; j < m_cur; ++j) rank += key_gt_f(ex_val[j], ex_idx[j], v, f) ? 1 : 0;
      if (rank < k) {
        out_idx[(int64_t)row * k + rank] = f;
        out_val[(int64_t)row * k + rank] = v;
        win_idx[rank] = f;
        if (rank == k - 1) tau_exact = v;
      }
    }
    if (m_cur > 0) {
      const int key_m = sel_key(items[m_cur - 1]);
      int sat = INT_MIN;
#pragma unroll
      for (int i = 0; i < SPT; ++i) {
        if (t + 256 * i < nseg) {
          int last = key[i][3];
          if (c_keep == 6) last = key[i][5];
          if (c_keep == 8) last = key[i][7];
          if (last >= key_m) sat = max(sat, last);
        }
      }
      if (sat != INT_MIN) atomicMax(&sat_key, sat);
    }
    __syncthreads();
    {
      const int u_rest = m_cur < G ? sel_key(items[m_cur]) : u_below;
      const int u = max(u_rest, sat_key);
      const float u_val = u == INT_MIN ? -INFINITY : ord2f((u & ~127) | 127);
      const float acc_err = (float)((d + 7) / 8) * 4.76837158e-7f * a_norm * wnorm_max[0];
      const float E = err_scale * (a_lo_norm * wnorm_max[0] + a_norm * wnorm_max[1]) + acc_err + fabsf(tau_exact) * 1.2207031e-4f;
      ok = !overflow && m_cur >= k && (u_val + E < tau_exact);
    }
    if (ok || m_cur >= Gs) break;
    __syncthreads();
    m_prev = m_cur;
    m_cur = min(m_cur + SEL_EXTEND, Gs);
  }
  if (ok) {
    if (t < k && feat_count) atomicAdd(feat_count + win_idx[t], 1.0f);
    if (stats && t == 0) atomicAdd(stats, m_cur);
  } else if (t == 0) {
    fb_rows[atomicAdd(fb_count, 1)] = row;
  }
}

__global__ void __launch_bounds__(256) k_topk_fallback(const int* __restrict__ fb_count, const int* __restrict__ fb_rows,
                                                       const float* __restrict__ sae_in, const float* __restrict__ W_encT,
                                                       const float* __restrict__ b_enc, float* __restrict__ scratch, int d, int F, int k, int cap,
                                                       int* __restrict__ out_idx, float* __restrict__ out_val, float* __restrict__ feat_count) {
  pb_pdl();
  const int n_items = *fb_count;
  if (n_items == 0) return;
  extern __shared__ __align__(16) unsigned char sm_raw[];
  float* a_row = reinterpret_cast<float*>(sm_raw);
  float* cand_v = a_row + d;
  int* cand_i = reinterpret_cast<int*>(cand_v + cap);
  __shared__ float best_v[256];
  __shared__ int best_i[256];
  __shared__ float tau_v;
  __shared__ int tau_i, cand_n;
  const int t = threadIdx.x, lane = t & 31, warp = t >> 5;
  const int nvec = d >> 2;
  float* h = scratch + (int64_t)blockIdx.x * F;
  for (int item = blockIdx.x; item < n_items; item += gridDim.x) {
    const int row = fb_rows[item];
    __syncthreads();
    for (int i = t; i < nvec; i += 256) reinterpret_cast<float4*>(a_row)[i] = reinterpret_cast<const float4*>(sae_in + (int64_t)row * d)[i];
    if (t == 0) cand_n = 0;
    __syncthreads();
    const float4* a4 = reinterpret_cast<const float4*>(a_row);
    for (int f = 2 * warp; f < F; f += 16) {
      float v0, v1;
      warp_dot2(a4, reinterpret_cast<const float4*>(W_encT + (int64_t)f * d), reinterpret_cast<const float4*>(W_encT + (int64_t)(f + 1) * d), nvec, lane,
                v0, v1);
      if (lane == 0) { h[f] = v0 + b_enc[f]; h[f + 1] = v1 + b_enc[f + 1]; }
    }
    __syncthreads();
    float bv = -INFINITY;
    int bi = 0x7fffffff;
    for (int p = t; p < F; p += 256) {
      const float v = h[p];
      if (key_gt_f(v, p, bv, bi)) { bv = v; bi = p; }
    }
    best_v[t] = bv;
    best_i[t] = bi;
    __syncthreads();
    {
      int rank = 0;
      for (int j = 0; j < 256; ++j) rank += key_gt_f(best_v[j], best_i[j], bv, bi) ? 1 : 0;
      if (rank == min(k, 256) - 1) { tau_v = bv; tau_i = bi; }
    }
    __syncthreads();
    const float tv = tau_v;
    const int ti = tau_i;
    for (int p = t; p < F; p += 256) {
      const float v = h[p];
      if (!key_gt_f(tv, ti, v, p)) {
        const int slot = atomicAdd(&cand_n, 1);
        if (slot < cap) { cand_v[slot] = v; cand_i[slot] = p; }
      }
    }
    __syncthreads();
    const int C = min(cand_n, cap);
    for (int c = t; c < C; c += 256) {
      const float cv = cand_v[c];
      const int ci = cand_i[c];
      int rank = 0;
      for (int j = 0; j < C; ++j) rank += key_gt_f(cand_v[j], cand_i[j], cv, ci) ? 1 : 0;
      if (rank < k) {
        out_idx[(int64_t)row * k + rank] = ci;
        out_val[(int64_t)row * k + rank] = cv;
        if (feat_count) atomicAdd(feat_count + ci, 1.0f);
      }
    }
  }
}

__global__ void __launch_bounds__(256) k_rownorm_max(const float* __restrict__ W, int F, int d, float* __restrict__ out) {
  const int lane = threadIdx.x & 31, warp = threadIdx.x >> 5, nw = blockDim.x >> 5;
  const int nvec = d >> 2;
  float best = 0.f, best_lo = 0.f;
  for (int f = blockIdx.x * nw + warp; f < F; f += gridDim.x * nw) {
    const float4* w4 = reinterpret_cast<const float4*>(W + (int64_t)f * d);
    float s = 0.f, l = 0.f;
    for (int i = lane; i < nvec; i += 32) {
      const float4 v = w4[i];
      s += v.x * v.x + v.y * v.y + v.z * v.z + v.w * v.w;
      const float lx = v.x - tf32_trunc(v.x), ly = v.y - tf32_trunc(v.y), lz = v.z - tf32_trunc(v.z), lw = v.w - tf32_trunc(v.w);
      l += lx * lx + ly * ly + lz * lz + lw * lw;
    }
    best = fmaxf(best, warp_sum(s));
    best_lo = fmaxf(best_lo, warp_sum(l));
  }
  if (lane == 0 && best > 0.f) {
    atomicMax(reinterpret_cast<unsigned int*>(out), __float_as_uint(sqrtf(best)));
    atomicMax(reinterpret_cast<unsigned int*>(out) + 1, __float_as_uint(sqrtf(best_lo)));
  }
}

template <int C_KEEP>
int launch_enc_cand(const PbSaeEncode* e, cudaStream_t st) {
  CUtensorMap tmA, tmB;
  PB_TRY(make_map(&tmA, e->sae_in, PB_F32, e->rows, e->d, e->d, FZ_BM));
  PB_TRY(make_map(&tmB, e->W_encT, PB_F32, e->F, e->d, e->d, FZ_BN));
  auto kern = k_enc_cand<C_KEEP>;
  static bool attr_done = false;
  if (!attr_done) {
    PB_CUDA(cudaFuncSetAttribute(kern, cudaFuncAttributeMaxDynamicSharedMemorySize, FZ_SMEM));
    attr_done = true;
  }
  const int num_m = (e->rows + FZ_BM - 1) / FZ_BM, num_n = (e->F + FZ_BN - 1) / FZ_BN;
  int grid = pb_sm_count();
  if (grid > num_m * num_n) grid = num_m * num_n;
  PB_LAUNCH_PDL(kern, grid, TC_THREADS, FZ_SMEM, st, tmA, tmB, e->d, e->rows, e->F, e->b_enc, e->cand, num_m, num_n);
  return PB_OK;
}

template <int SPT>
int launch_select(const PbSaeEncode* e, int nseg, float scale, cudaStream_t st) {
  const size_t smem = sizeof(float) * e->d;
  PB_LAUNCH_PDL(k_cand_select<SPT>, e->rows, 256, smem, st, (const int*)e->cand, nseg, e->c_keep, e->sae_in, e->W_encT, e->b_enc, e->enc_norm_max, scale,
                e->d, e->k, e->m_cand, e->idx, e->val, e->feat_count, e->fb_count, e->fb_rows, e->fb_count + 1);
  return PB_OK;
}

}

extern "C" int pb_sae_fused_workspace(int32_t rows, int32_t F, int32_t c_keep, int64_t* cand_bytes, int64_t* fb_scratch_bytes) {
  PB_CHECK_ARG(rows >= 0 && F > 0 && F % FZ_SEG == 0 && (c_keep == 4 || c_keep == 6 || c_keep == 8) && cand_bytes && fb_scratch_bytes,
               "pb_sae_fused_workspace: needs d_sae %% 128 == 0 and c_keep in {4, 6, 8}");
  *cand_bytes = (int64_t)rows * (F / FZ_SEG) * c_keep * 4;
  *fb_scratch_bytes = (int64_t)2 * pb_sm_count() * F * 4;
  return PB_OK;
}

extern "C" int pb_sae_encode_topk_fused(const PbSaeEncode* e, pb_stream_t stream) {
  PB_CHECK_ARG(e && e->sae_in && e->W_encT && e->b_enc && e->cand && e->enc_norm_max && e->idx && e->val && e->fb_count && e->fb_rows,
               "pb_sae_encode_topk_fused: missing pointers");
  PB_CHECK_ARG(e->rows >= 0 && e->d >= 32 && e->d % 4 == 0 && e->d <= 8192 && e->F % FZ_SEG == 0 && e->F >= FZ_SEG,
               "pb_sae_encode_topk_fused: needs d_in %% 4 == 0, 32 <= d_in <= 8192, d_sae %% 128 == 0 (d=%d F=%d)", e->d, e->F);
  PB_CHECK_ARG(e->c_keep == 4 || e->c_keep == 6 || e->c_keep == 8, "pb_sae_encode_topk_fused: c_keep must be 4, 6 or 8");
  PB_CHECK_ARG(e->k >= 1 && e->k <= 64 && e->k <= e->m_cand && e->m_cand <= SEL_MAX_CAND && e->k <= e->F,
               "pb_sae_encode_topk_fused: needs k <= 64 and k <= m_cand <= %d", SEL_MAX_CAND);
  PB_CHECK_ARG(pb_aligned16(e->sae_in) && pb_aligned16(e->W_encT) && pb_aligned16(e->b_enc) && pb_aligned16(e->cand),
               "pb_sae_encode_topk_fused: operands must be 16-byte aligned");
  const int nkeys = e->F / FZ_SEG * e->c_keep;
  PB_CHECK_ARG(e->F / FZ_SEG <= 256 * 4, "pb_sae_encode_topk_fused: d_sae=%d too large for the selection kernel (max 131072)", e->F);
  PB_CHECK_ARG(e->cand_bytes >= (int64_t)e->rows * nkeys * 4, "pb_sae_encode_topk_fused: candidate buffer too small");
  if (e->rows == 0) return PB_OK;
  cudaStream_t st = (cudaStream_t)stream;
  const int phases = (e->phases & 7) ? e->phases : (e->phases | 7);
  if (phases & 1) {
    if (e->c_keep == 4) PB_TRY(launch_enc_cand<4>(e, st));
    else if (e->c_keep == 6) PB_TRY(launch_enc_cand<6>(e, st));
    else PB_TRY(launch_enc_cand<8>(e, st));
  }
  if (phases & 2) {
    if (!(phases & 8)) PB_CUDA(cudaMemsetAsync(e->fb_count, 0, 2 * sizeof(int), st));
    const float coef = e->err_coef > 0.f ? e->err_coef : 1.05f;
    const int nseg = e->F / FZ_SEG, spt = (nseg + 255) / 256;
    if (spt <= 1) PB_TRY(launch_select<1>(e, nseg, coef, st));
    else if (spt <= 2) PB_TRY(launch_select<2>(e, nseg, coef, st));
    else PB_TRY(launch_select<4>(e, nseg, coef, st));
  }
  if (phases & 4) {
    PB_CHECK_ARG(e->fb_scratch && e->fb_scratch_bytes >= (int64_t)e->F * 4, "pb_sae_encode_topk_fused: fallback scratch missing");
    int grid = (int)(e->fb_scratch_bytes / ((int64_t)e->F * 4));
    if (grid > 2 * pb_sm_count()) grid = 2 * pb_sm_count();
    int cap = ((e->F + 255) / 256) * e->k;
    if (cap > e->F) cap = e->F;
    const size_t smem = sizeof(float) * e->d + 8 * (size_t)cap;
    PB_CHECK_ARG(smem <= 200 * 1024, "pb_sae_encode_topk_fused: k=%d x d_sae=%d too large for the exact-path candidate buffer", e->k, e->F);
    static size_t attr_smem = 0;
    if (smem > 48 * 1024 && smem > attr_smem) {
      PB_CUDA(cudaFuncSetAttribute(k_topk_fallback, cudaFuncAttributeMaxDynamicSharedMemorySize, (int)smem));
      attr_smem = smem;
    }
    PB_LAUNCH_PDL(k_topk_fallback, grid, 256, smem, st, (const int*)e->fb_count, (const int*)e->fb_rows, e->sae_in, e->W_encT, e->b_enc, e->fb_scratch,
                  e->d, e->F, e->k, cap, e->idx, e->val, e->feat_count);
  }
  return PB_OK;
}

extern "C" int pb_rownorm_max(const float* W, int32_t F, int32_t d, float* out, pb_stream_t stream) {
  PB_CHECK_ARG(W && out && F >= 0 && d > 0 && d % 4 == 0, "pb_rownorm_max: bad arguments");
  cudaStream_t st = (cudaStream_t)stream;
  PB_CUDA(cudaMemsetAsync(out, 0, 2 * sizeof(float), st));
  if (F == 0) return PB_OK;
  int grid = pb_sm_count() * 4;
  if (grid > (F + 7) / 8) grid = (F + 7) / 8;
  k_rownorm_max<<<grid, 256, 0, st>>>(W, F, d, out);
  PB_LAUNCH_CHECK();
  return PB_OK;
}

int pb_abi_sizeof_fused(int which) { return which == 9 ? (int)sizeof(PbSaeEncode) : -1; }
```

vit-prisma_b200/csrc/sae_optim.cuh:

```cuda
#pragma once
#include <stddef.h>
#include "common.cuh"

struct SaeScalars {
  float loss_sum;
  float gnorm_sq;
  float clip_coef;
  float mse;
  float l0;
  float pos_count;
  float grad_norm;
  float reserved;
};
static_assert(sizeof(SaeScalars) == 32, "SaeScalars is 8 floats");
static_assert(offsetof(SaeScalars, clip_coef) == 8, "SaeScalars.clip_coef is float 2");

__device__ __forceinline__ float sae_clip_coef(float norm, float max_norm) {
  return max_norm > 0.f ? fminf(1.f, max_norm / (norm + 1e-6f)) : 1.f;
}

__device__ __forceinline__ void sae_publish_scalars(SaeScalars* sc, float gnorm_sq, float max_norm, float inv_elems, float inv_rows) {
  const float norm = sqrtf(gnorm_sq);
  sc->gnorm_sq = gnorm_sq;
  sc->grad_norm = norm;
  sc->clip_coef = sae_clip_coef(norm, max_norm);
  sc->mse = sc->loss_sum * inv_elems;
  sc->l0 = sc->pos_count * inv_rows;
}

struct AdamHyper { float lr, beta1, beta2, eps, bc1, bc2_sqrt; };

static inline AdamHyper adam_hyper(float lr, float beta1, float beta2, float eps, int step) {
  AdamHyper h;
  h.lr = lr; h.beta1 = beta1; h.beta2 = beta2; h.eps = eps;
  h.bc1 = 1.f - powf(beta1, (float)step);
  h.bc2_sqrt = sqrtf(1.f - powf(beta2, (float)step));
  return h;
}

__device__ __forceinline__ float adam_update(float p, float gr, float& m, float& v, const AdamHyper& h) {
  m = fmaf(h.beta1, m, (1.f - h.beta1) * gr);
  v = fmaf(h.beta2, v, (1.f - h.beta2) * gr * gr);
  float sq, rc;
  asm("sqrt.approx.ftz.f32 %0, %1;" : "=f"(sq) : "f"(v));
  const float denom = fmaf(sq, __frcp_rn(h.bc2_sqrt), h.eps);
  asm("rcp.approx.ftz.f32 %0, %1;" : "=f"(rc) : "f"(denom));
  return fmaf(-(h.lr * __frcp_rn(h.bc1)) * m, rc, p);
}

__device__ __forceinline__ void dead_feature_counters(float* since_fired, float* act_freq, int f, float fired, float sf, float af) {
  if (since_fired) since_fired[f] = fired > 0.f ? 0.f : sf + 1.f;
  if (act_freq) act_freq[f] = af + fired;
}

template <int CHUNKS, class Out>
__device__ __forceinline__ void sae_adam_feature(const float* wd, const float* gd, float* md, float* vd, const float* we, const float* ge,
                                                 float* me, float* ve, float clip, const AdamHyper& h, int nvec, bool renorm,
                                                 const Out& out, float& esq, float& elo) {
  const int lane = threadIdx.x & 31;
  float w[CHUNKS][4], gq[CHUNKS][4];
  float par = 0.f;
#pragma unroll
  for (int i = 0; i < CHUNKS; ++i) {
    const int c4 = i * 32 + lane;
    if (c4 < nvec) {
      ld4(wd + 4 * c4, w[i]);
      ld4(gd + 4 * c4, gq[i]);
#pragma unroll
      for (int q = 0; q < 4; ++q) { gq[i][q] *= clip; par = fmaf(gq[i][q], w[i][q], par); }
    } else {
      w[i][0] = w[i][1] = w[i][2] = w[i][3] = gq[i][0] = gq[i][1] = gq[i][2] = gq[i][3] = 0.f;
    }
  }
  par = warp_sum(par);
  float nsq = 0.f;
#pragma unroll
  for (int i = 0; i < CHUNKS; ++i) {
    const int c4 = i * 32 + lane;
    if (c4 < nvec) {
      float mm[4], vv[4];
      ld4(md + 4 * c4, mm);
      ld4(vd + 4 * c4, vv);
#pragma unroll
      for (int q = 0; q < 4; ++q) {
        w[i][q] = adam_update(w[i][q], gq[i][q] - par * w[i][q], mm[q], vv[q], h);
        nsq += w[i][q] * w[i][q];
      }
      st4(md + 4 * c4, mm);
      st4(vd + 4 * c4, vv);
    }
  }
  const float inv_nrm = 1.f / sqrtf(warp_sum(nsq));
#pragma unroll
  for (int i = 0; i < CHUNKS; ++i) {
    const int c4 = i * 32 + lane;
    if (c4 < nvec) {
      if (renorm) {
#pragma unroll
        for (int q = 0; q < 4; ++q) w[i][q] = w[i][q] * inv_nrm;
      }
      out.dec(c4, w[i]);
    }
  }
  esq = 0.f;
  elo = 0.f;
#pragma unroll
  for (int i = 0; i < CHUNKS; ++i) {
    const int c4 = i * 32 + lane;
    if (c4 < nvec) {
      float p[4], gr[4], mm[4], vv[4], lo[4];
      ld4(we + 4 * c4, p);
      ld4(ge + 4 * c4, gr);
      ld4(me + 4 * c4, mm);
      ld4(ve + 4 * c4, vv);
#pragma unroll
      for (int q = 0; q < 4; ++q) {
        p[q] = adam_update(p[q], gr[q] * clip, mm[q], vv[q], h);
        lo[q] = tf32_lo(p[q]);
        esq = fmaf(p[q], p[q], esq);
        const float tl = p[q] - tf32_trunc(p[q]);
        elo = fmaf(tl, tl, elo);
      }
      st4(me + 4 * c4, mm);
      st4(ve + 4 * c4, vv);
      out.enc(c4, p, lo);
    }
  }
}

static inline int chunks_for(int d) {
  if (d % 4 != 0) return -1;
  const int nvec = d / 4;
  if (nvec <= 32) return 1;
  if (nvec <= 64) return 2;
  if (nvec <= 128) return 4;
  if (nvec <= 192) return 6;
  if (nvec <= 256) return 8;
  if (nvec <= 384) return 12;
  return -1;
}
#define PB_DISPATCH_CHUNKS(CH, ...)                                                    \
  switch (CH) {                                                                        \
    case 1: { constexpr int C_ = 1; __VA_ARGS__; } break;                              \
    case 2: { constexpr int C_ = 2; __VA_ARGS__; } break;                              \
    case 4: { constexpr int C_ = 4; __VA_ARGS__; } break;                              \
    case 6: { constexpr int C_ = 6; __VA_ARGS__; } break;                              \
    case 8: { constexpr int C_ = 8; __VA_ARGS__; } break;                              \
    case 12: { constexpr int C_ = 12; __VA_ARGS__; } break;                            \
    default: pb_set_error("sae: d_in=%d unsupported (needs d %% 4 == 0 and d <= 1536)", d); return PB_EUNSUPPORTED; \
  }
```

vit-prisma_b200/csrc/tc_common.cuh:

```cuda
#pragma once
#include "common.cuh"
#include <cuda.h>

namespace {


__device__ __forceinline__ uint32_t smem_u32(const void* p) { return (uint32_t)__cvta_generic_to_shared(p); }

__device__ __forceinline__ void mbar_init(uint32_t bar, uint32_t count) {
  asm volatile("mbarrier.init.shared::cta.b64 [%0], %1;" ::"r"(bar), "r"(count) : "memory");
}
__device__ __forceinline__ void mbar_expect_tx(uint32_t bar, uint32_t bytes) {
  asm volatile("mbarrier.arrive.expect_tx.shared::cta.b64 _, [%0], %1;" ::"r"(bar), "r"(bytes) : "memory");
}
template <bool REPORT = true>
__device__ __forceinline__ void mbar_wait(uint32_t bar, uint32_t parity) {
  const long long t0 = clock64();
  for (;;) {
    uint32_t done;
    asm volatile(
        "{\n\t.reg .pred p;\n\t"
        "mbarrier.try_wait.parity.shared::cta.b64 p, [%1], %2;\n\t"
        "selp.u32 %0, 1, 0, p;\n\t}"
        : "=r"(done)
        : "r"(bar), "r"(parity)
        : "memory");
    if (done) return;
    if (clock64() - t0 > 4000000000LL) {
      if (REPORT)
        printf("prisma: mbarrier wait timed out (block %d thread %d bar 0x%x parity %u)\n", blockIdx.x, threadIdx.x, bar, parity);
      __trap();
    }
  }
}
__device__ __forceinline__ void tma_load_2d(uint32_t dst, const CUtensorMap* map, uint32_t bar, int c0, int c1) {
  asm volatile("cp.async.bulk.tensor.2d.shared::cluster.global.mbarrier::complete_tx::bytes [%0], [%1, {%3, %4}], [%2];" ::"r"(dst),
               "l"(reinterpret_cast<uint64_t>(map)), "r"(bar), "r"(c0), "r"(c1)
               : "memory");
}
__device__ __forceinline__ void prefetch_tmap(const CUtensorMap* map) {
  asm volatile("prefetch.tensormap [%0];" ::"l"(reinterpret_cast<uint64_t>(map)) : "memory");
}
__device__ __forceinline__ void wgmma_fence() { asm volatile("wgmma.fence.sync.aligned;" ::: "memory"); }
__device__ __forceinline__ void wgmma_commit() { asm volatile("wgmma.commit_group.sync.aligned;" ::: "memory"); }
template <int N>
__device__ __forceinline__ void wgmma_wait() { asm volatile("wgmma.wait_group.sync.aligned %0;" ::"n"(N) : "memory"); }
template <int N>
__device__ __forceinline__ void wgmma_fence_acc(float (&d)[N]) {
#pragma unroll
  for (int i = 0; i < N; ++i) asm volatile("" : "+f"(d[i])::"memory");
}
#define PB_ACC64_REGS "%0, %1, %2, %3, %4, %5, %6, %7, %8, %9, %10, %11, %12, %13, %14, %15, %16, %17, %18, %19, %20, %21, %22, %23, %24, %25, %26, %27, %28, %29, %30, %31, %32, %33, %34, %35, %36, %37, %38, %39, %40, %41, %42, %43, %44, %45, %46, %47, %48, %49, %50, %51, %52, %53, %54, %55, %56, %57, %58, %59, %60, %61, %62, %63"
#define PB_ACC64_OUT "+f"(d[0]), "+f"(d[1]), "+f"(d[2]), "+f"(d[3]), "+f"(d[4]), "+f"(d[5]), "+f"(d[6]), "+f"(d[7]), "+f"(d[8]), "+f"(d[9]), "+f"(d[10]), "+f"(d[11]), "+f"(d[12]), "+f"(d[13]), "+f"(d[14]), "+f"(d[15]), "+f"(d[16]), "+f"(d[17]), "+f"(d[18]), "+f"(d[19]), "+f"(d[20]), "+f"(d[21]), "+f"(d[22]), "+f"(d[23]), "+f"(d[24]), "+f"(d[25]), "+f"(d[26]), "+f"(d[27]), "+f"(d[28]), "+f"(d[29]), "+f"(d[30]), "+f"(d[31]), "+f"(d[32]), "+f"(d[33]), "+f"(d[34]), "+f"(d[35]), "+f"(d[36]), "+f"(d[37]), "+f"(d[38]), "+f"(d[39]), "+f"(d[40]), "+f"(d[41]), "+f"(d[42]), "+f"(d[43]), "+f"(d[44]), "+f"(d[45]), "+f"(d[46]), "+f"(d[47]), "+f"(d[48]), "+f"(d[49]), "+f"(d[50]), "+f"(d[51]), "+f"(d[52]), "+f"(d[53]), "+f"(d[54]), "+f"(d[55]), "+f"(d[56]), "+f"(d[57]), "+f"(d[58]), "+f"(d[59]), "+f"(d[60]), "+f"(d[61]), "+f"(d[62]), "+f"(d[63])
__device__ __forceinline__ void wgmma_tf32_n128(float (&d)[64], uint64_t adesc, uint64_t bdesc, uint32_t accumulate) {
  asm volatile(
      "{\n\t.reg .pred p;\n\tsetp.ne.b32 p, %66, 0;\n\t"
      "wgmma.mma_async.sync.aligned.m64n128k8.f32.tf32.tf32 "
      "{" PB_ACC64_REGS "}, "
      "%64, %65, p, 1, 1;\n\t}"
      : PB_ACC64_OUT
      : "l"(adesc), "l"(bdesc), "r"(accumulate));
}
#define PB_ACC128_REGS "%0, %1, %2, %3, %4, %5, %6, %7, %8, %9, %10, %11, %12, %13, %14, %15, %16, %17, %18, %19, %20, %21, %22, %23, %24, %25, %26, %27, %28, %29, %30, %31, %32, %33, %34, %35, %36, %37, %38, %39, %40, %41, %42, %43, %44, %45, %46, %47, %48, %49, %50, %51, %52, %53, %54, %55, %56, %57, %58, %59, %60, %61, %62, %63, %64, %65, %66, %67, %68, %69, %70, %71, %72, %73, %74, %75, %76, %77, %78, %79, %80, %81, %82, %83, %84, %85, %86, %87, %88, %89, %90, %91, %92, %93, %94, %95, %96, %97, %98, %99, %100, %101, %102, %103, %104, %105, %106, %107, %108, %109, %110, %111, %112, %113, %114, %115, %116, %117, %118, %119, %120, %121, %122, %123, %124, %125, %126, %127"
#define PB_ACC128_OUT "+f"(d[0]), "+f"(d[1]), "+f"(d[2]), "+f"(d[3]), "+f"(d[4]), "+f"(d[5]), "+f"(d[6]), "+f"(d[7]), "+f"(d[8]), "+f"(d[9]), "+f"(d[10]), "+f"(d[11]), "+f"(d[12]), "+f"(d[13]), "+f"(d[14]), "+f"(d[15]), "+f"(d[16]), "+f"(d[17]), "+f"(d[18]), "+f"(d[19]), "+f"(d[20]), "+f"(d[21]), "+f"(d[22]), "+f"(d[23]), "+f"(d[24]), "+f"(d[25]), "+f"(d[26]), "+f"(d[27]), "+f"(d[28]), "+f"(d[29]), "+f"(d[30]), "+f"(d[31]), "+f"(d[32]), "+f"(d[33]), "+f"(d[34]), "+f"(d[35]), "+f"(d[36]), "+f"(d[37]), "+f"(d[38]), "+f"(d[39]), "+f"(d[40]), "+f"(d[41]), "+f"(d[42]), "+f"(d[43]), "+f"(d[44]), "+f"(d[45]), "+f"(d[46]), "+f"(d[47]), "+f"(d[48]), "+f"(d[49]), "+f"(d[50]), "+f"(d[51]), "+f"(d[52]), "+f"(d[53]), "+f"(d[54]), "+f"(d[55]), "+f"(d[56]), "+f"(d[57]), "+f"(d[58]), "+f"(d[59]), "+f"(d[60]), "+f"(d[61]), "+f"(d[62]), "+f"(d[63]), "+f"(d[64]), "+f"(d[65]), "+f"(d[66]), "+f"(d[67]), "+f"(d[68]), "+f"(d[69]), "+f"(d[70]), "+f"(d[71]), "+f"(d[72]), "+f"(d[73]), "+f"(d[74]), "+f"(d[75]), "+f"(d[76]), "+f"(d[77]), "+f"(d[78]), "+f"(d[79]), "+f"(d[80]), "+f"(d[81]), "+f"(d[82]), "+f"(d[83]), "+f"(d[84]), "+f"(d[85]), "+f"(d[86]), "+f"(d[87]), "+f"(d[88]), "+f"(d[89]), "+f"(d[90]), "+f"(d[91]), "+f"(d[92]), "+f"(d[93]), "+f"(d[94]), "+f"(d[95]), "+f"(d[96]), "+f"(d[97]), "+f"(d[98]), "+f"(d[99]), "+f"(d[100]), "+f"(d[101]), "+f"(d[102]), "+f"(d[103]), "+f"(d[104]), "+f"(d[105]), "+f"(d[106]), "+f"(d[107]), "+f"(d[108]), "+f"(d[109]), "+f"(d[110]), "+f"(d[111]), "+f"(d[112]), "+f"(d[113]), "+f"(d[114]), "+f"(d[115]), "+f"(d[116]), "+f"(d[117]), "+f"(d[118]), "+f"(d[119]), "+f"(d[120]), "+f"(d[121]), "+f"(d[122]), "+f"(d[123]), "+f"(d[124]), "+f"(d[125]), "+f"(d[126]), "+f"(d[127])
__device__ __forceinline__ void wgmma_tf32_n256(float (&d)[128], uint64_t adesc, uint64_t bdesc, uint32_t accumulate) {
  asm volatile(
      "{\n\t.reg .pred p;\n\tsetp.ne.b32 p, %130, 0;\n\t"
      "wgmma.mma_async.sync.aligned.m64n256k8.f32.tf32.tf32 "
      "{" PB_ACC128_REGS "}, "
      "%128, %129, p, 1, 1;\n\t}"
      : PB_ACC128_OUT
      : "l"(adesc), "l"(bdesc), "r"(accumulate));
}
__device__ __forceinline__ void wgmma_bf16_n128(float (&d)[64], uint64_t adesc, uint64_t bdesc, uint32_t accumulate) {
  asm volatile(
      "{\n\t.reg .pred p;\n\tsetp.ne.b32 p, %66, 0;\n\t"
      "wgmma.mma_async.sync.aligned.m64n128k16.f32.bf16.bf16 "
      "{" PB_ACC64_REGS "}, "
      "%64, %65, p, 1, 1, 0, 0;\n\t}"
      : PB_ACC64_OUT
      : "l"(adesc), "l"(bdesc), "r"(accumulate));
}

template <int N> __device__ __forceinline__ void reg_dealloc() { asm volatile("setmaxnreg.dec.sync.aligned.u32 %0;" ::"n"(N)); }
template <int N> __device__ __forceinline__ void reg_alloc() { asm volatile("setmaxnreg.inc.sync.aligned.u32 %0;" ::"n"(N)); }
__device__ __forceinline__ void wg_sync(int id) { asm volatile("bar.sync %0, 128;" ::"r"(id) : "memory"); }

__device__ __forceinline__ uint64_t make_smem_desc(uint32_t saddr) {
  uint64_t d = 0;
  d |= (uint64_t)((saddr & 0x3FFFFu) >> 4);
  d |= (uint64_t)1 << 16;
  d |= (uint64_t)(1024 >> 4) << 32;
  d |= (uint64_t)1 << 62;
  return d;
}

constexpr int TC_BM = 128;
constexpr int TC_BN = 128;
constexpr int TC_THREADS = 384;

template <typename T, int NPASS, int STAGES>
struct TcCfg {
  static constexpr int ES = sizeof(T);
  static constexpr int BK = 128 / ES;
  static constexpr int KSTEPS = 4;
  static constexpr int A_BYTES = TC_BM * 128;
  static constexpr int B_BYTES = TC_BN * 128;
  static constexpr int NOP = NPASS == 3 ? 2 : 1;
  static constexpr int STAGE_BYTES = NOP * (A_BYTES + B_BYTES);
  static constexpr int RING_BYTES = STAGES * STAGE_BYTES;
};

__device__ __forceinline__ void mbar_arrive(uint32_t bar) {
  asm volatile("mbarrier.arrive.shared::cta.b64 _, [%0];" ::"r"(bar) : "memory");
}

typedef CUresult (*EncodeTiledFn)(CUtensorMap*, CUtensorMapDataType, cuuint32_t, void*, const cuuint64_t*, const cuuint64_t*,
                                  const cuuint32_t*, const cuuint32_t*, CUtensorMapInterleave, CUtensorMapSwizzle,
                                  CUtensorMapL2promotion, CUtensorMapFloatOOBfill);

EncodeTiledFn get_encode_fn() {
  static EncodeTiledFn fn = nullptr;
  if (!fn) {
    void* p = nullptr;
    cudaDriverEntryPointQueryResult qres;
    if (cudaGetDriverEntryPoint("cuTensorMapEncodeTiled", &p, cudaEnableDefault, &qres) == cudaSuccess && qres == cudaDriverEntryPointSuccess)
      fn = (EncodeTiledFn)p;
  }
  return fn;
}

int make_map(CUtensorMap* map, const void* ptr, int dtype, int64_t rows, int64_t cols, int64_t ld, int box_rows) {
  EncodeTiledFn fn = get_encode_fn();
  if (!fn) { pb_set_error("gemm_tc: cuTensorMapEncodeTiled entry point unavailable"); return PB_ECUDA; }
  const int es = dtype == PB_BF16 ? 2 : 4;
  cuuint64_t gdim[2] = {(cuuint64_t)cols, (cuuint64_t)rows};
  cuuint64_t gstride[1] = {(cuuint64_t)ld * es};
  cuuint32_t box[2] = {(cuuint32_t)(128 / es), (cuuint32_t)box_rows};
  cuuint32_t estr[2] = {1, 1};
  CUresult rc = fn(map, dtype == PB_BF16 ? CU_TENSOR_MAP_DATA_TYPE_BFLOAT16 : CU_TENSOR_MAP_DATA_TYPE_FLOAT32, 2, const_cast<void*>(ptr), gdim,
                   gstride, box, estr, CU_TENSOR_MAP_INTERLEAVE_NONE, CU_TENSOR_MAP_SWIZZLE_128B, CU_TENSOR_MAP_L2_PROMOTION_L2_256B,
                   CU_TENSOR_MAP_FLOAT_OOB_FILL_NONE);
  if (rc != CUDA_SUCCESS) {
    pb_set_error("gemm_tc: cuTensorMapEncodeTiled failed (%d) rows=%lld cols=%lld ld=%lld", (int)rc, (long long)rows, (long long)cols, (long long)ld);
    return PB_ECUDA;
  }
  return PB_OK;
}

}
```

vit-prisma_b200/vit_prisma/b200/sae_engine.py:

```python
from __future__ import annotations

import ctypes as C
from typing import Optional

import torch

from . import _lib as L
from .ops import _need_cuda, _stream, cast as _cast


def ops_cast_f32(x: torch.Tensor) -> torch.Tensor:
    return _cast(x.contiguous(), torch.float32)

vp, i32, i64, f32 = C.c_void_p, C.c_int32, C.c_int64, C.c_float


class PbSaeStep(C.Structure):
    _fields_ = (
        [(n, i32) for n in ("rows", "d", "F", "k", "norm_mode", "training", "step", "renorm_decoder")]
        + [(n, f32) for n in ("lr", "beta1", "beta2", "adam_eps", "max_grad_norm")]
        + [(n, vp) for n in (
            "x", "W_encT", "W_encT_lo", "W_dec", "b_enc", "b_dec",
            "sae_in", "mu", "sd", "xsum", "idx", "val", "feat_count", "sae_out", "g", "dval",
            "csc_off", "csc_cursor", "csc_entries", "gW_dec", "gW_encT", "gb_enc", "gb_dec", "gcol", "gbdec2",
            "fired", "scalars", "m_dec", "v_dec", "m_enc", "v_enc", "m_be", "v_be", "m_bd", "v_bd",
            "since_fired", "act_freq")]
        + [("global_rows", i32), ("dist", i32), ("work", vp), ("work_bytes", i64), ("enc_norm_max", vp), ("pre_zeroed", i32)]
    )


class PbSaeEncode(C.Structure):
    _fields_ = (
        [(n, i32) for n in ("rows", "d", "F", "k", "c_keep", "m_cand", "phases")] + [("err_coef", f32)]
        + [(n, vp) for n in ("sae_in", "W_encT", "b_enc", "enc_norm_max", "cand")] + [("cand_bytes", i64)]
        + [(n, vp) for n in ("idx", "val", "feat_count", "fb_count", "fb_rows", "fb_scratch")] + [("fb_scratch_bytes", i64)]
    )


L.ABI_STRUCTS.append(PbSaeStep)
L.register_signatures({
    "pb_sae_prep": (i32, [vp, vp, vp, vp, vp, vp, vp, i32, i32, i32, vp]),
    "pb_sae_topk": (i32, [vp, i32, i32, i32, vp, vp, vp, vp, i64, vp]),
    "pb_sae_scatter_acts": (i32, [vp, vp, vp, i32, i32, i32, i32, vp]),
    "pb_sae_step_reset": (i32, [C.POINTER(PbSaeStep), vp, vp]),
    "pb_sae_decode": (i32, [C.POINTER(PbSaeStep), vp]),
    "pb_sae_backward": (i32, [C.POINTER(PbSaeStep), vp]),
    "pb_sae_adam": (i32, [C.POINTER(PbSaeStep), vp]),
    "pb_unit_norm_rows": (i32, [vp, vp, i32, i32, vp]),
    "pb_sae_mse": (i32, [vp, vp, vp, vp, i32, i32, vp]),
    "pb_sae_fused_workspace": (i32, [i32, i32, i32, C.POINTER(i64), C.POINTER(i64)]),
    "pb_sae_encode_topk_fused": (i32, [C.POINTER(PbSaeEncode), vp]),
    "pb_rownorm_max": (i32, [vp, i32, i32, vp, vp]),
    "pb_sumsq": (i32, [vp, i64, vp, vp]),
    "pb_sae_clip_finish": (i32, [vp, f32, i32, i32, vp]),
    "pb_adam_vec": (i32, [vp, vp, vp, vp, i32, vp, f32, f32, f32, f32, i32, vp]),
})

NORM_MODE = {"none": 0, None: 0, "layer_norm": 1, "constant_norm_rescale": 2}
SCALAR_NAMES = ("loss_sum", "gnorm_sq", "clip_coef", "mse", "l0", "pos_count", "grad_norm", "reserved")
TOPK_SEG = 256 * 96


def unit_norm_rows_(w: torch.Tensor, w_lo: Optional[torch.Tensor] = None) -> None:
    _need_cuda(w)
    assert w.is_contiguous() and w.dtype == torch.float32
    L.check(L.get_lib().pb_unit_norm_rows(w.data_ptr(), None if w_lo is None else w_lo.data_ptr(), w.shape[0], w.shape[1], _stream()),
            "pb_unit_norm_rows")


def sae_prep(x2: torch.Tensor, b_dec: torch.Tensor, norm_mode: str):
    _need_cuda(x2, b_dec)
    rows, d = x2.shape
    sae_in = torch.empty_like(x2)
    mu = torch.empty(rows, device=x2.device)
    sd = torch.empty(rows, device=x2.device)
    L.check(L.get_lib().pb_sae_prep(x2.data_ptr(), b_dec.data_ptr(), sae_in.data_ptr(), None, mu.data_ptr(), sd.data_ptr(), None,
                                    rows, d, NORM_MODE[norm_mode], _stream()), "pb_sae_prep")
    return sae_in, mu, sd


def topk_support(hidden_pre2: torch.Tensor, k: int):
    _need_cuda(hidden_pre2)
    rows, F = hidden_pre2.shape
    idx = torch.empty(rows, k, dtype=torch.int32, device=hidden_pre2.device)
    val = torch.empty(rows, k, device=hidden_pre2.device)
    nseg = (F + TOPK_SEG - 1) // TOPK_SEG
    scratch = torch.empty(max(rows * nseg * k * 8, 16), dtype=torch.uint8, device=hidden_pre2.device) if F > TOPK_SEG else None
    L.check(L.get_lib().pb_sae_topk(hidden_pre2.data_ptr(), rows, F, k, idx.data_ptr(), val.data_ptr(), None,
                                    None if scratch is None else scratch.data_ptr(), 0 if scratch is None else scratch.numel(),
                                    _stream()), "pb_sae_topk")
    return idx, val


def topk_dense(x: torch.Tensor, k: int) -> torch.Tensor:
    _need_cuda(x)
    lead, F = x.shape[:-1], x.shape[-1]
    x2 = x.reshape(-1, F).contiguous().float()
    idx, val = topk_support(x2, k)
    dense = torch.empty_like(x2)
    L.check(L.get_lib().pb_sae_scatter_acts(idx.data_ptr(), val.data_ptr(), dense.data_ptr(), x2.shape[0], k, F, 1, _stream()),
            "pb_sae_scatter_acts")
    return dense.view(*lead, F).to(x.dtype)


def sae_mse(x2: torch.Tensor, out2: torch.Tensor) -> torch.Tensor:
    _need_cuda(x2, out2)
    rows, d = x2.shape
    xsum = torch.empty(d, device=x2.device)
    res = torch.empty(1, device=x2.device)
    L.check(L.get_lib().pb_sae_mse(x2.data_ptr(), out2.data_ptr(), xsum.data_ptr(), res.data_ptr(), rows, d, _stream()), "pb_sae_mse")
    return res[0]


class SaeStepEngine:
    is_data_parallel = False

    def __init__(self, W_encT: torch.Tensor, W_dec: torch.Tensor, b_enc: torch.Tensor, b_dec: torch.Tensor, k: int,
                 normalize_activations: str = "layer_norm", max_grad_norm: float = 1.0, betas=(0.9, 0.999), adam_eps: float = 1e-8,
                 gemm_impl: int = L.GEMM_AUTO, encoder: str = "auto", c_keep: int = 8, m_cand: Optional[int] = None):
        _need_cuda(W_encT, W_dec, b_enc, b_dec)
        for t in (W_encT, W_dec, b_enc, b_dec):
            if t.dtype != torch.float32 or not t.is_contiguous():
                raise L.PrismaB200Error("SaeStepEngine: parameters must be contiguous fp32 CUDA tensors")
        self.F, self.d = W_dec.shape
        assert W_encT.shape == (self.F, self.d) and b_enc.shape == (self.F,) and b_dec.shape == (self.d,)
        self.k = int(k)
        self.W_encT, self.W_dec, self.b_enc, self.b_dec = W_encT, W_dec, b_enc, b_dec
        self.norm_mode = NORM_MODE[normalize_activations]
        self.max_grad_norm = float(max_grad_norm or 0.0)
        self.betas, self.adam_eps = betas, adam_eps
        self.gemm_impl = gemm_impl
        dev = W_dec.device
        z = lambda *s, dt=torch.float32: torch.zeros(*s, dtype=dt, device=dev)
        fused_ok = self.d % 4 == 0 and self.d >= 32 and self.F % 128 == 0 and self.k <= 48 and self.F <= 131072
        if encoder == "auto":
            encoder = "fused" if (fused_ok and gemm_impl == L.GEMM_AUTO) else "dense"
        if encoder == "fused" and not fused_ok:
            raise L.PrismaB200Error(f"fused encoder->TopK needs d_in % 4 == 0, d_sae % 128 == 0, k <= 48 (d={self.d} F={self.F} k={self.k})")
        import os
        self.encoder, self.c_keep = encoder, int(os.environ.get("PRISMA_SAE_C_KEEP", c_keep))
        self.m_cand = int(os.environ.get("PRISMA_SAE_M_CAND", 0)) or (int(m_cand) if m_cand else self.k + 8)
        self.enc_norm_max = z(2)
        self.fb_count = z(2, dt=torch.int32)
        self.W_encT_lo = torch.empty_like(W_encT) if encoder == "dense" else None
        self.refresh_lo()
        self.m_dec, self.v_dec, self.m_enc, self.v_enc = z(self.F, self.d), z(self.F, self.d), z(self.F, self.d), z(self.F, self.d)
        self.m_be, self.v_be, self.m_bd, self.v_bd = z(self.F), z(self.F), z(self.d), z(self.d)
        self.gW_dec, self.gW_encT = torch.empty(self.F, self.d, device=dev), torch.empty(self.F, self.d, device=dev)
        self.gb_enc, self.gb_dec = z(self.F), z(self.d)
        self.gcol, self.gbdec2, self.xsum = z(self.d), z(self.d), z(self.d)
        self.feat_count, self.fired = z(self.F), z(self.F)
        self.csc_off, self.csc_cursor = z(self.F + 1, dt=torch.int32), z(self.F, dt=torch.int32)
        self.scalars = z(8)
        self.step_count = 0
        self._rows = -1

    def refresh_lo(self) -> None:
        if self.W_encT_lo is not None:
            from . import ops
            self.W_encT_lo.copy_(ops.split_tf32(self.W_encT))
        L.check(L.get_lib().pb_rownorm_max(self.W_encT.data_ptr(), self.F, self.d, self.enc_norm_max.data_ptr(), _stream()), "pb_rownorm_max")

    def _ensure_rows(self, rows: int) -> None:
        if rows == self._rows:
            return
        dev, d, F, k = self.W_dec.device, self.d, self.F, self.k
        e = lambda *s, dt=torch.float32: torch.empty(*s, dtype=dt, device=dev)
        self.sae_in, self.g, self.sae_out = e(rows, d), e(rows, d), e(rows, d)
        self.mu, self.sd = e(rows), e(rows)
        if self.encoder == "fused":
            cb, sb = i64(0), i64(0)
            L.check(L.get_lib().pb_sae_fused_workspace(rows, F, self.c_keep, C.byref(cb), C.byref(sb)), "pb_sae_fused_workspace")
            self.cand = e(max(cb.value // 4, 4), dt=torch.int32)
            self.fb_rows = e(max(rows, 1), dt=torch.int32)
            self.fb_scratch = e(min(64, max(sb.value // (4 * F), 1)) * F)
            self.sae_in_lo = self.hidden_pre = None
        else:
            self.sae_in_lo, self.hidden_pre = e(rows, d), e(rows, F)
        self.idx, self.val, self.dval = e(rows, k, dt=torch.int32), e(rows, k), e(rows, k)
        self.csc_entries = e(rows * k, dt=torch.int32)
        self.work = e(8 + 4 * F + 8 * (rows * k // 32 + F + 1) + 64, dt=torch.uint8)
        nseg = (F + TOPK_SEG - 1) // TOPK_SEG
        self.topk_scratch = e(max(rows * nseg * k * 8, 16), dt=torch.uint8) if F > TOPK_SEG else None
        self._rows = rows

    def _desc(self, x: torch.Tensor, training: bool, lr: float = 0.0, since_fired=None, act_freq=None, want_out=True) -> PbSaeStep:
        s = PbSaeStep()
        s.rows, s.d, s.F, s.k = x.shape[0], self.d, self.F, self.k
        s.norm_mode, s.training, s.step, s.renorm_decoder = self.norm_mode, int(training), max(self.step_count, 1), 1
        s.lr, s.beta1, s.beta2, s.adam_eps, s.max_grad_norm = lr, self.betas[0], self.betas[1], self.adam_eps, self.max_grad_norm
        p = lambda t: None if t is None else t.data_ptr()
        s.x = p(x)
        s.W_encT, s.W_encT_lo, s.W_dec, s.b_enc, s.b_dec = p(self.W_encT), p(self.W_encT_lo), p(self.W_dec), p(self.b_enc), p(self.b_dec)
        s.sae_in, s.mu, s.sd, s.xsum = p(self.sae_in), p(self.mu), p(self.sd), p(self.xsum)
        s.idx, s.val, s.feat_count = p(self.idx), p(self.val), p(self.feat_count)
        s.sae_out, s.g, s.dval = (p(self.sae_out) if want_out else None), p(self.g), p(self.dval)
        s.csc_off, s.csc_cursor, s.csc_entries = p(self.csc_off), p(self.csc_cursor), p(self.csc_entries)
        s.gW_dec, s.gW_encT, s.gb_enc, s.gb_dec = p(self.gW_dec), p(self.gW_encT), p(self.gb_enc), p(self.gb_dec)
        s.gcol, s.gbdec2, s.fired, s.scalars = p(self.gcol), p(self.gbdec2), p(self.fired), p(self.scalars)
        s.m_dec, s.v_dec, s.m_enc, s.v_enc = p(self.m_dec), p(self.v_dec), p(self.m_enc), p(self.v_enc)
        s.m_be, s.v_be, s.m_bd, s.v_bd = p(self.m_be), p(self.v_be), p(self.m_bd), p(self.v_bd)
        s.since_fired, s.act_freq = p(since_fired), p(act_freq)
        s.work, s.work_bytes = p(self.work), self.work.numel()
        s.enc_norm_max = p(self.enc_norm_max)
        return s

    def _enc_desc(self, rows: int, phases: int = 0) -> PbSaeEncode:
        e = PbSaeEncode()
        e.rows, e.d, e.F, e.k, e.c_keep, e.m_cand, e.phases, e.err_coef = rows, self.d, self.F, self.k, self.c_keep, self.m_cand, phases, 0.0
        e.sae_in, e.W_encT, e.b_enc, e.enc_norm_max = self.sae_in.data_ptr(), self.W_encT.data_ptr(), self.b_enc.data_ptr(), self.enc_norm_max.data_ptr()
        e.cand, e.cand_bytes = self.cand.data_ptr(), self.cand.numel() * 4
        e.idx, e.val, e.feat_count = self.idx.data_ptr(), self.val.data_ptr(), self.feat_count.data_ptr()
        e.fb_count, e.fb_rows = self.fb_count.data_ptr(), self.fb_rows.data_ptr()
        e.fb_scratch, e.fb_scratch_bytes = self.fb_scratch.data_ptr(), self.fb_scratch.numel() * 4
        return e

    def _encoder_gemm(self, rows: int) -> None:
        lib, st = L.get_lib(), _stream()
        use_tc = self.gemm_impl != L.GEMM_SIMT
        g = L.PbGemm()
        g.M, g.N, g.K, g.dtype, g.impl = rows, self.F, self.d, L.PB_F32, self.gemm_impl
        g.A, g.lda, g.B, g.ldb = self.sae_in.data_ptr(), self.d, self.W_encT.data_ptr(), self.d
        if use_tc:
            g.A_lo, g.B_lo = self.sae_in_lo.data_ptr(), self.W_encT_lo.data_ptr()
        g.bias, g.out0, g.ld0 = self.b_enc.data_ptr(), self.hidden_pre.data_ptr(), self.F
        L.check(lib.pb_gemm(C.byref(g), st), "pb_gemm(encoder)")

    def encode_topk(self, x: torch.Tensor, pre_zeroed: bool = False) -> None:
        lib, st = L.get_lib(), _stream()
        rows = x.shape[0]
        self._ensure_rows(rows)
        L.check(lib.pb_sae_prep(x.data_ptr(), self.b_dec.data_ptr(), self.sae_in.data_ptr(),
                                self.sae_in_lo.data_ptr() if (self.sae_in_lo is not None and self.gemm_impl != L.GEMM_SIMT) else None,
                                self.mu.data_ptr(), self.sd.data_ptr(),
                                self.xsum.data_ptr(), rows, self.d, self.norm_mode, st), "pb_sae_prep")
        if not pre_zeroed:
            self.feat_count.zero_()
        if self.encoder == "fused":
            L.check(lib.pb_sae_encode_topk_fused(C.byref(self._enc_desc(rows, 8 if pre_zeroed else 0)), st), "pb_sae_encode_topk_fused")
            return
        self._encoder_gemm(rows)
        scratch = self.topk_scratch
        L.check(lib.pb_sae_topk(self.hidden_pre.data_ptr(), rows, self.F, self.k, self.idx.data_ptr(), self.val.data_ptr(),
                                self.feat_count.data_ptr(), None if scratch is None else scratch.data_ptr(),
                                0 if scratch is None else scratch.numel(), st), "pb_sae_topk")

    @torch.no_grad()
    def forward(self, x: torch.Tensor, want_out: bool = True):
        _need_cuda(x)
        x = ops_cast_f32(x)
        self.encode_topk(x)
        self.scalars.zero_()
        s = self._desc(x, training=False, want_out=want_out)
        L.check(L.get_lib().pb_sae_decode(C.byref(s), _stream()), "pb_sae_decode")
        return (self.sae_out if want_out else None), self.idx, self.val

    @torch.no_grad()
    def train_step(self, x: torch.Tensor, lr: float, since_fired: Optional[torch.Tensor] = None,
                   act_freq: Optional[torch.Tensor] = None, want_out: bool = False) -> torch.Tensor:
        _need_cuda(x)
        x = ops_cast_f32(x)
        lib, st = L.get_lib(), _stream()
        self._ensure_rows(x.shape[0])
        self.step_count += 1
        s = self._desc(x, training=True, lr=float(lr), since_fired=since_fired, act_freq=act_freq, want_out=want_out)
        s.pre_zeroed = 1
        L.check(lib.pb_sae_step_reset(C.byref(s), self.fb_count.data_ptr(), st), "pb_sae_step_reset")
        self.encode_topk(x, pre_zeroed=True)
        L.check(lib.pb_sae_decode(C.byref(s), st), "pb_sae_decode")
        L.check(lib.pb_sae_backward(C.byref(s), st), "pb_sae_backward")
        L.check(lib.pb_sae_adam(C.byref(s), st), "pb_sae_adam")
        return self.scalars

    def describe_encoder(self) -> str:
        if self.encoder == "fused":
            return (f"fused: one-pass tf32 wgmma GEMM with top-{self.c_keep}-per-128-features epilogue -> exact fp32 re-scoring of "
                    f">= {self.m_cand} candidates per token -> exact top-{self.k} with a completeness proof (no dense hidden_pre)")
        return "wgmma 3xTF32 GEMM -> dense hidden_pre -> exact k_topk" if self.gemm_impl != L.GEMM_SIMT else "exact FFMA GEMM -> k_topk"

    def fallback_rows(self) -> int:
        return int(self.fb_count[0].item()) if self.encoder == "fused" else 0

    def rescored_per_row(self, rows: int) -> float:
        fb, tot = self.fb_count.tolist()
        return tot / max(rows - fb, 1)

    def _optimizer_stages(self, s: PbSaeStep, x: torch.Tensor, lr: float, since_fired, act_freq):
        lib, st = L.get_lib(), _stream()
        kernel = "k_sae_adam_rows" if self.W_encT_lo is not None or self.d < 64 else "k_sae_adam_bulk"
        return [("adam (clip + decoder-parallel-gradient removal + Adam + row renorm)", lambda: L.check(lib.pb_sae_adam(C.byref(s), st)),
                 dict(bytes=60 * self.d * self.F, ncu=kernel))]

    def _clip_and_adam(self, x: torch.Tensor, lr: float, since_fired, act_freq, grads, extra) -> None:
        lib, st = L.get_lib(), _stream()
        self.scalars[1:2].zero_()
        acc = self.scalars[1:].data_ptr()
        for t in grads:
            L.check(lib.pb_sumsq(t.data_ptr(), t.numel(), acc, st), "pb_sumsq")
        L.check(lib.pb_sae_clip_finish(self.scalars.data_ptr(), self.max_grad_norm, x.shape[0], self.d, st), "pb_sae_clip_finish")
        s = self._desc(x, training=True, lr=lr, since_fired=since_fired, act_freq=act_freq, want_out=False)
        L.check(lib.pb_sae_adam(C.byref(s), st), "pb_sae_adam")
        for p, g, m, v in extra:
            L.check(lib.pb_adam_vec(p.data_ptr(), g.data_ptr(), m.data_ptr(), v.data_ptr(), p.numel(), self.scalars.data_ptr(), lr, self.betas[0],
                                    self.betas[1], self.adam_eps, self.step_count, st), "pb_adam_vec")

    @torch.no_grad()
    def time_stages(self, x: torch.Tensor, lr: float, since_fired=None, act_freq=None, reps: int = 5) -> dict:
        lib, st = L.get_lib(), _stream()
        x = ops_cast_f32(x)
        rows = x.shape[0]
        out = {}

        def timed(name, fn, **info):
            torch.cuda.synchronize()
            a, b = torch.cuda.Event(enable_timing=True), torch.cuda.Event(enable_timing=True)
            a.record()
            for _ in range(reps):
                fn()
            b.record()
            torch.cuda.synchronize()
            out[name] = dict(ms=a.elapsed_time(b) / reps, **info)

        for name, fn, info in self._encode_stages(x):
            timed(name, fn, **info)
        self.encode_topk(x)
        self.scalars.zero_()
        self.step_count += 1
        s = self._desc(x, training=True, lr=float(lr), since_fired=since_fired, act_freq=act_freq, want_out=False)
        self._prepare_timed_step(s, x)
        timed("decode (sparse decode + loss + d_hidden)", lambda: L.check(lib.pb_sae_decode(C.byref(s), st)),
              bytes=(12 * rows * self.d + 8 * rows * self.k), ncu=r"k_sae_decode")
        timed("backward (csc build + per-feature gradients + norm)", lambda: (self.scalars.zero_(), L.check(lib.pb_sae_backward(C.byref(s), st))),
              bytes=8 * self.d * self.F, ncu=r"k_sae_grads<")
        for name, fn, info in self._optimizer_stages(s, x, float(lr), since_fired, act_freq):
            timed(name, fn, **info)
        return out

    def _prepare_timed_step(self, s: PbSaeStep, x: torch.Tensor) -> None:
        pass

    def _encode_stages(self, x: torch.Tensor):
        rows = x.shape[0]
        if self.encoder == "fused":
            lib, st = L.get_lib(), _stream()
            self.encode_topk(x)
            flops = 2.0 * rows * self.d * self.F
            nkeys = (self.F // 128) * self.c_keep
            return [("encode + topk, fused (prep + tf32 candidate GEMM + select / exact re-score + exact path)", lambda: self.encode_topk(x),
                     dict(flops=flops, passes=1)),
                    ("candidate GEMM alone (one tf32 pass, top-c-per-segment epilogue)",
                     lambda: L.check(lib.pb_sae_encode_topk_fused(C.byref(self._enc_desc(rows, 1)), st)),
                     dict(flops=flops, passes=1, bytes=4 * self.d * self.F + 4 * rows * self.d + 4 * rows * nkeys, ncu=r"k_enc_cand")),
                    ("select + exact re-score alone", lambda: L.check(lib.pb_sae_encode_topk_fused(C.byref(self._enc_desc(rows, 2)), st)),
                     dict(bytes=4 * rows * nkeys + 4 * rows * self.d + 8 * rows * self.k, ncu=r"k_cand_select"))]
        return [("encode + topk (prep + encoder GEMM 3xTF32 + exact topk)", lambda: self.encode_topk(x),
                 dict(flops=2.0 * rows * self.d * self.F, passes=3, ncu=r"k_gemm_tc<float")),
                ("encoder GEMM alone (hidden_pre = sae_in @ W_enc + b_enc)", lambda: self._encoder_gemm(rows),
                 dict(flops=2.0 * rows * self.d * self.F, passes=3, bytes=8 * self.d * self.F + 8 * rows * self.d + 4 * rows * self.F))]

    def dense_feature_acts(self) -> torch.Tensor:
        rows = self.idx.shape[0]
        dense = torch.empty(rows, self.F, device=self.W_dec.device)
        L.check(L.get_lib().pb_sae_scatter_acts(self.idx.data_ptr(), self.val.data_ptr(), dense.data_ptr(), rows, self.k, self.F, 1,
                                                _stream()), "pb_sae_scatter_acts")
        return dense

    def scalars_dict(self) -> dict:
        vals = self.scalars.tolist()
        return dict(zip(SCALAR_NAMES, vals))

    def algorithmic_bytes(self, rows: int) -> int:
        return 80 * self.d * self.F + 8 * rows * self.d
```

Measured before the change: 2.562 million.

## Use fp16 operand copies for the fused candidate encoder GEMM

Adds fp16 shadow copies of sae_in (written in the prep kernel) and W_encT (written in the Adam kernels), and feeds them to the candidate-selection wgmma GEMM in place of tf32 fp32 operands. The aim is to halve operand bytes and use the faster fp16 tensor-core path for the candidate pass, while exact fp32 re-scoring keeps the final top-k exact. The Adam kernels also track the maximum fp16 rounding-error norm so the candidate error bound can be widened. The trade-off is extra writes in Adam and prep, plus a looser candidate bound that may send more rows to the fallback path.

```diff
diff --git a/include/prisma_b200.h b/include/prisma_b200.h
--- a/include/prisma_b200.h
+++ b/include/prisma_b200.h
@@ -16,7 +16,7 @@
 #endif
 
 enum { PB_OK = 0, PB_EINVAL = -1, PB_ECUDA = -2, PB_EUNSUPPORTED = -3, PB_ENODEVICE = -4 };
-enum { PB_F32 = 0, PB_BF16 = 1 };
+enum { PB_F32 = 0, PB_BF16 = 1, PB_F16 = 2  };
 enum { PB_ACT_NONE = 0, PB_ACT_RELU = 1, PB_ACT_GELU = 2, PB_ACT_SILU = 3, PB_ACT_GELU_NEW = 4,
        PB_ACT_GELU_FAST = 5, PB_ACT_QUICK_GELU = 6, PB_ACT_TANH_RELU = 7, PB_ACT_EXP = 8 };
 enum { PB_GEMM_AUTO = 0, PB_GEMM_SIMT = 1, PB_GEMM_TC = 2 };
@@ -146,10 +146,13 @@
   void* work; int64_t work_bytes;
   float* enc_norm_max;
   int32_t pre_zeroed;
+  void* W_encT16; float* enc16_lo_max;
 } PbSaeStep;
 
 PB_API int pb_sae_prep(const float* x, const float* b_dec, float* sae_in, float* sae_in_lo, float* mu, float* sd,
                        float* xsum, int32_t rows, int32_t d, int32_t norm_mode, pb_stream_t stream);
+PB_API int pb_sae_prep16(const float* x, const float* b_dec, float* sae_in, void* sae_in16, float* mu, float* sd,
+                         float* xsum, int32_t rows, int32_t d, int32_t norm_mode, pb_stream_t stream);
 PB_API int pb_sae_topk(const float* hidden_pre, int32_t rows, int32_t F, int32_t k, int32_t* idx, float* val,
                        float* feat_count, void* scratch, int64_t scratch_bytes, pb_stream_t stream);
 PB_API int pb_sae_scatter_acts(const int32_t* idx, const float* val, float* dense, int32_t rows, int32_t k, int32_t F,
@@ -178,10 +181,12 @@
   int32_t* fb_count;
   int32_t* fb_rows;
   float* fb_scratch; int64_t fb_scratch_bytes;
+  const void* sae_in16; const void* W_encT16; const float* enc16_lo_max;
 } PbSaeEncode;
 PB_API int pb_sae_fused_workspace(int32_t rows, int32_t F, int32_t c_keep, int64_t* cand_bytes, int64_t* fb_scratch_bytes);
 PB_API int pb_sae_encode_topk_fused(const PbSaeEncode* e, pb_stream_t stream);
 PB_API int pb_rownorm_max(const float* W, int32_t F, int32_t d, float* out, pb_stream_t stream);
+PB_API int pb_f16_copy(const float* W, int64_t rows, int32_t d, void* W16, float* lo_max, pb_stream_t stream);
 
 PB_API int pb_transpose(const float* in, float* out, float* out_lo, int32_t rows, int32_t cols, pb_stream_t stream);
 PB_API int pb_colsum(const float* x, float* out, int32_t rows, int32_t cols, int32_t accumulate, pb_stream_t stream);
diff --git a/vit-prisma_b200/csrc/common.cuh b/vit-prisma_b200/csrc/common.cuh
--- a/vit-prisma_b200/csrc/common.cuh
+++ b/vit-prisma_b200/csrc/common.cuh
@@ -1,6 +1,7 @@
 #pragma once
 #include <cuda_runtime.h>
 #include <cuda_bf16.h>
+#include <cuda_fp16.h>
 #include <stdint.h>
 #include <stdio.h>
 #include <string.h>
@@ -87,6 +88,19 @@
   return __uint_as_float(r);
 }
 
+__device__ __forceinline__ float f16_sat(float x) { return __half2float(__float2half_rn(fminf(fmaxf(x, -65504.f), 65504.f))); }
+__device__ __forceinline__ uint2 f16x4(const float (&v)[4], float& rsq) {
+  float h[4];
+#pragma unroll
+  for (int q = 0; q < 4; ++q) {
+    h[q] = f16_sat(v[q]);
+    const float r = v[q] - h[q];
+    rsq = fmaf(r, r, rsq);
+  }
+  const __half2 a = __floats2half2_rn(h[0], h[1]), b = __floats2half2_rn(h[2], h[3]);
+  return make_uint2(*reinterpret_cast<const uint32_t*>(&a), *reinterpret_cast<const uint32_t*>(&b));
+}
+
 __device__ __forceinline__ float apply_act(float x, int act) {
   switch (act) {
     case PB_ACT_RELU: return fmaxf(x, 0.f);
diff --git a/vit-prisma_b200/csrc/p2p.cu b/vit-prisma_b200/csrc/p2p.cu
--- a/vit-prisma_b200/csrc/p2p.cu
+++ b/vit-prisma_b200/csrc/p2p.cu
@@ -210,7 +210,7 @@
     else if (mc_W_dec) mc_st4(mc_W_dec + base + 4 * c4, w);
     else for (int j = 0; j < world; ++j) st4(wdec_rot[j] + base + 4 * c4, w);
   }
-  __device__ __forceinline__ void enc(int c4, const float (&p)[4], const float (&lo)[4]) const {
+  __device__ __forceinline__ void enc(int c4, const float (&p)[4], const float (&lo)[4], uint2) const {
     if (mc_W_encT) {
       mc_st4(mc_W_encT + base + 4 * c4, p);
     } else {
@@ -245,10 +245,10 @@
   }
   for (int f = f0 + blockIdx.x * nw + warp; f < f1; f += gridDim.x * nw) {
     const int64_t base = (int64_t)f * d;
-    float esq, elo;
+    float esq, elo, e16;
     sae_adam_feature<CHUNKS>(W_dec + base, gWd + base, m_dec + base, v_dec + base, W_encT + base, gWe + base, m_enc + base, v_enc + base,
                              clip, h, nvec, true,
-                             AdamPeerOut{wdec_rot, wenc_rot, wlo_rot, W_dec, mc_W_dec, mc_W_encT, t.world, defer_dec, base}, esq, elo);
+                             AdamPeerOut{wdec_rot, wenc_rot, wlo_rot, W_dec, mc_W_dec, mc_W_encT, t.world, defer_dec, base}, esq, elo, e16);
     enc_best = fmaxf(enc_best, warp_sum(esq));
     enc_best_lo = fmaxf(enc_best_lo, warp_sum(elo));
     if (lane == 0) {
diff --git a/vit-prisma_b200/csrc/sae.cu b/vit-prisma_b200/csrc/sae.cu
--- a/vit-prisma_b200/csrc/sae.cu
+++ b/vit-prisma_b200/csrc/sae.cu
@@ -4,8 +4,8 @@
 
 template <int CHUNKS>
 __global__ void __launch_bounds__(256) k_sae_prep(const float* __restrict__ x, const float* __restrict__ b_dec, float* __restrict__ sae_in,
-                                                  float* __restrict__ sae_in_lo, float* __restrict__ mu_out, float* __restrict__ std_out,
-                                                  int rows, int d, int norm_mode, float eps) {
+                                                  float* __restrict__ sae_in_lo, __half* __restrict__ sae_in16, float* __restrict__ mu_out,
+                                                  float* __restrict__ std_out, int rows, int d, int norm_mode, float eps) {
   pb_pdl();
   const int lane = threadIdx.x & 31;
   const int row = blockIdx.x * (blockDim.x >> 5) + (threadIdx.x >> 5);
@@ -61,6 +61,10 @@
       (void)inv;
       st4(sae_in + (int64_t)row * d + 4 * c4, o);
       if (sae_in_lo) st4(sae_in_lo + (int64_t)row * d + 4 * c4, lo);
+      if (sae_in16) {
+        float unused = 0.f;
+        *reinterpret_cast<uint2*>(sae_in16 + (int64_t)row * d + 4 * c4) = f16x4(o, unused);
+      }
     }
   }
 }
@@ -623,16 +627,23 @@
 
 struct AdamRowsOut {
   float *W_dec, *W_encT, *W_encT_lo;
+  __half* W_encT16;
   int64_t base;
   __device__ __forceinline__ void dec(int c4, const float (&w)[4]) const { st4(W_dec + base + 4 * c4, w); }
-  __device__ __forceinline__ void enc(int c4, const float (&p)[4], const float (&lo)[4]) const {
+  __device__ __forceinline__ void enc(int c4, const float (&p)[4], const float (&lo)[4], uint2 p16) const {
     st4(W_encT + base + 4 * c4, p);
     if (W_encT_lo) st4(W_encT_lo + base + 4 * c4, lo);
+    if (W_encT16) *reinterpret_cast<uint2*>(W_encT16 + base + 4 * c4) = p16;
   }
 };
+
+__device__ __forceinline__ void atomic_max_norm(float* out, float best_sq) {
+  if (best_sq > 0.f) atomicMax(reinterpret_cast<unsigned int*>(out), __float_as_uint(sqrtf(best_sq)));
+}
 
 template <int CHUNKS>
 __global__ void __launch_bounds__(256) k_sae_adam_rows(float* __restrict__ W_dec, float* __restrict__ W_encT, float* __restrict__ W_encT_lo,
+                                                       __half* __restrict__ W_encT16, float* __restrict__ enc16_lo_max,
                                                        float* __restrict__ b_enc, const float* __restrict__ gW_dec,
                                                        const float* __restrict__ gW_encT, const float* __restrict__ gb_enc,
                                                        float* __restrict__ m_dec, float* __restrict__ v_dec, float* __restrict__ m_enc,
@@ -643,13 +654,14 @@
   const int lane = threadIdx.x & 31, warp = threadIdx.x >> 5, nw = blockDim.x >> 5;
   const int nvec = d >> 2;
   const float clip = sc->clip_coef;
-  float enc_best = 0.f, enc_best_lo = 0.f;
+  float enc_best = 0.f, enc_best_lo = 0.f, enc_best16 = 0.f;
   for (int f = blockIdx.x * nw + warp; f < F; f += gridDim.x * nw) {
     const int64_t base = (int64_t)f * d;
-    float esq, elo;
+    float esq, elo, e16;
     sae_adam_feature<CHUNKS>(W_dec + base, gW_dec + base, m_dec + base, v_dec + base, W_encT + base, gW_encT + base, m_enc + base,
-                             v_enc + base, clip, h, nvec, renorm, AdamRowsOut{W_dec, W_encT, W_encT_lo, base}, esq, elo);
+                             v_enc + base, clip, h, nvec, renorm, AdamRowsOut{W_dec, W_encT, W_encT_lo, W_encT16, base}, esq, elo, e16);
     if (enc_norm_max) { enc_best = fmaxf(enc_best, warp_sum(esq)); enc_best_lo = fmaxf(enc_best_lo, warp_sum(elo)); }
+    if (enc16_lo_max) enc_best16 = fmaxf(enc_best16, warp_sum(e16));
     if (lane == 0) {
       float mm = m_be[f], vv = v_be[f];
       b_enc[f] = adam_update(b_enc[f], gb_enc[f] * clip, mm, vv, h);
@@ -662,6 +674,7 @@
     atomicMax(reinterpret_cast<unsigned int*>(enc_norm_max), __float_as_uint(sqrtf(enc_best)));
     atomicMax(reinterpret_cast<unsigned int*>(enc_norm_max) + 1, __float_as_uint(sqrtf(enc_best_lo)));
   }
+  if (enc16_lo_max && lane == 0) atomic_max_norm(enc16_lo_max, enc_best16);
 }
 
 constexpr int AB_MAX_STAGES = 12;
@@ -669,8 +682,12 @@
 
 struct AdamSlotOut {
   float *wd, *we;
+  __half* we16;
   __device__ __forceinline__ void dec(int c4, const float (&w)[4]) const { st4(wd + 4 * c4, w); }
-  __device__ __forceinline__ void enc(int c4, const float (&p)[4], const float (&)[4]) const { st4(we + 4 * c4, p); }
+  __device__ __forceinline__ void enc(int c4, const float (&p)[4], const float (&)[4], uint2 p16) const {
+    st4(we + 4 * c4, p);
+    if (we16) *reinterpret_cast<uint2*>(we16 + 4 * c4) = p16;
+  }
 };
 
 __device__ __forceinline__ void bulk_load(uint32_t dst, const void* src, uint32_t bytes, uint32_t bar) {
@@ -688,7 +705,8 @@
                 float* __restrict__ m_enc, float* __restrict__ v_enc, float* __restrict__ m_be, float* __restrict__ v_be,
                 const float* __restrict__ fired, float* __restrict__ since_fired, float* __restrict__ act_freq,
                 const SaeScalars* __restrict__ sc, AdamHyper h, int F, int d, int renorm, float* __restrict__ enc_norm_max, int S,
-                float* __restrict__ b_dec, const float* __restrict__ gb_dec, float* __restrict__ m_bd, float* __restrict__ v_bd) {
+                float* __restrict__ b_dec, const float* __restrict__ gb_dec, float* __restrict__ m_bd, float* __restrict__ v_bd,
+                __half* __restrict__ W_encT16, float* __restrict__ enc16_lo_max) {
   pb_pdl_trigger();
   extern __shared__ __align__(128) unsigned char ab_smem[];
   const uint32_t s0 = smem_u32(ab_smem);
@@ -737,7 +755,7 @@
   }
   const int nvec = d >> 2;
   const float clip = sc->clip_coef;
-  float enc_best = 0.f, enc_best_lo = 0.f;
+  float enc_best = 0.f, enc_best_lo = 0.f, enc_best16 = 0.f;
   for (int i = warp - 1; i < n_mine; i += S) {
     const int s = i % S;
     const uint32_t ph = (uint32_t)(i / S) & 1u;
@@ -751,11 +769,12 @@
     }
     mbar_wait(full_bar(s), ph);
     float* st = data_generic + (size_t)s * 8 * d;
-    float esq, elo;
+    float esq, elo, e16;
     sae_adam_feature<CHUNKS>(st, st + d, st + 2 * d, st + 3 * d, st + 4 * d, st + 5 * d, st + 6 * d, st + 7 * d, clip, h, nvec, renorm,
-                             AdamSlotOut{st, st + 4 * d}, esq, elo);
+                             AdamSlotOut{st, st + 4 * d, W_encT16 ? reinterpret_cast<__half*>(st + d) : nullptr}, esq, elo, e16);
     enc_best = fmaxf(enc_best, warp_sum(esq));
     enc_best_lo = fmaxf(enc_best_lo, warp_sum(elo));
+    if (W_encT16) enc_best16 = fmaxf(enc_best16, warp_sum(e16));
     __syncwarp();
     asm volatile("fence.proxy.async.shared::cta;" ::: "memory");
     __syncwarp();
@@ -767,6 +786,7 @@
       bulk_store(W_encT + base, src + 4 * row_bytes, row_bytes);
       bulk_store(m_enc + base, src + 6 * row_bytes, row_bytes);
       bulk_store(v_enc + base, src + 7 * row_bytes, row_bytes);
+      if (W_encT16) bulk_store(W_encT16 + base, src + 1 * row_bytes, row_bytes / 2);
       asm volatile("cp.async.bulk.commit_group;" ::: "memory");
       b_enc[f] = adam_update(be, gbe * clip, mbe, vbe, h);
       m_be[f] = mbe;
@@ -780,6 +800,7 @@
     atomicMax(reinterpret_cast<unsigned int*>(enc_norm_max), __float_as_uint(sqrtf(enc_best)));
     atomicMax(reinterpret_cast<unsigned int*>(enc_norm_max) + 1, __float_as_uint(sqrtf(enc_best_lo)));
   }
+  if (enc16_lo_max && lane == 0) atomic_max_norm(enc16_lo_max, enc_best16);
   asm volatile("cp.async.bulk.wait_group 0;" ::: "memory");
 }
 
@@ -832,14 +853,16 @@
   return ctas < 1 ? 1 : ctas;
 }
 
-extern "C" int pb_sae_prep(const float* x, const float* b_dec, float* sae_in, float* sae_in_lo, float* mu, float* sd, float* xsum, int32_t rows,
-                           int32_t d, int32_t norm_mode, pb_stream_t stream) {
+static int launch_prep(const float* x, const float* b_dec, float* sae_in, float* sae_in_lo, __half* sae_in16, float* mu, float* sd, float* xsum,
+                       int32_t rows, int32_t d, int32_t norm_mode, pb_stream_t stream) {
   PB_CHECK_ARG(x && b_dec && sae_in && rows >= 0 && d > 0, "pb_sae_prep: bad arguments");
   PB_CHECK_ARG(norm_mode == 0 || (mu && sd), "pb_sae_prep: mu/std buffers required when normalising");
+  PB_CHECK_ARG(!sae_in16 || ((uintptr_t)sae_in16 & 7) == 0, "pb_sae_prep16: sae_in16 must be 8-byte aligned");
   if (rows == 0) return PB_OK;
   cudaStream_t st = (cudaStream_t)stream;
   const int ch = chunks_for(d);
-  PB_DISPATCH_CHUNKS(ch, PB_LAUNCH_PDL(k_sae_prep<C_>, (rows + 7) / 8, 256, 0, st, x, b_dec, sae_in, sae_in_lo, mu, sd, rows, d, norm_mode, 1e-5f));
+  PB_DISPATCH_CHUNKS(ch, PB_LAUNCH_PDL(k_sae_prep<C_>, (rows + 7) / 8, 256, 0, st, x, b_dec, sae_in, sae_in_lo, sae_in16, mu, sd, rows, d, norm_mode,
+                                       1e-5f));
   if (xsum) {
     PB_CUDA(cudaMemsetAsync(xsum, 0, sizeof(float) * d, st));
     const int rpc = 8;
@@ -847,6 +870,16 @@
     PB_LAUNCH_CHECK();
   }
   return PB_OK;
+}
+
+extern "C" int pb_sae_prep(const float* x, const float* b_dec, float* sae_in, float* sae_in_lo, float* mu, float* sd, float* xsum, int32_t rows,
+                           int32_t d, int32_t norm_mode, pb_stream_t stream) {
+  return launch_prep(x, b_dec, sae_in, sae_in_lo, nullptr, mu, sd, xsum, rows, d, norm_mode, stream);
+}
+
+extern "C" int pb_sae_prep16(const float* x, const float* b_dec, float* sae_in, void* sae_in16, float* mu, float* sd, float* xsum, int32_t rows,
+                             int32_t d, int32_t norm_mode, pb_stream_t stream) {
+  return launch_prep(x, b_dec, sae_in, nullptr, (__half*)sae_in16, mu, sd, xsum, rows, d, norm_mode, stream);
 }
 
 static int launch_topk(const float* vals, const int* map, int64_t row_stride, int F, int seg_len, int nseg, int k, int* oi, float* ov,
@@ -1006,7 +1039,11 @@
   const int d = s->d, F = s->F, ch = chunks_for(d);
   const AdamHyper h = adam_hyper(s->lr, s->beta1, s->beta2, s->adam_eps, s->step);
   const int grid = persistent_grid(8, F);
+  PB_CHECK_ARG(!s->W_encT16 == !s->enc16_lo_max, "pb_sae_adam: W_encT16 and enc16_lo_max go together");
+  PB_CHECK_ARG(!s->W_encT16 || (d % 8 == 0 && ((uintptr_t)s->W_encT16 & 15) == 0), "pb_sae_adam: the fp16 copy of W_encT needs d %% 8 == 0");
+  __half* const W16 = (__half*)s->W_encT16;
   if (s->enc_norm_max) PB_CUDA(cudaMemsetAsync(s->enc_norm_max, 0, 2 * sizeof(float), st));
+  if (s->enc16_lo_max) PB_CUDA(cudaMemsetAsync(s->enc16_lo_max, 0, sizeof(float), st));
   if (!s->W_encT_lo && d >= 64) {
     const size_t stage = (size_t)8 * d * 4;
     int S = (int)((200 * 1024) / stage);
@@ -1020,12 +1057,13 @@
         PB_CUDA(cudaFuncSetAttribute(kern, cudaFuncAttributeMaxDynamicSharedMemorySize, (int)smem));
         PB_LAUNCH_PDL(kern, g2, 32 * (1 + S), smem, st, s->W_dec, s->W_encT, s->b_enc, s->gW_dec, s->gW_encT, s->gb_enc, s->m_dec, s->v_dec,
                       s->m_enc, s->v_enc, s->m_be, s->v_be, s->fired, s->since_fired, s->act_freq, (const SaeScalars*)s->scalars, h, F, d,
-                      s->renorm_decoder, s->enc_norm_max, S, s->b_dec, s->gb_dec, s->m_bd, s->v_bd);
+                      s->renorm_decoder, s->enc_norm_max, S, s->b_dec, s->gb_dec, s->m_bd, s->v_bd, W16, s->enc16_lo_max);
       });
       return PB_OK;
     }
   }
-  PB_DISPATCH_CHUNKS(ch, (k_sae_adam_rows<C_><<<grid, 256, 0, st>>>(s->W_dec, s->W_encT, s->W_encT_lo, s->b_enc, s->gW_dec, s->gW_encT, s->gb_enc,
+  PB_DISPATCH_CHUNKS(ch, (k_sae_adam_rows<C_><<<grid, 256, 0, st>>>(s->W_dec, s->W_encT, s->W_encT_lo, W16, s->enc16_lo_max, s->b_enc, s->gW_dec,
+                                                                     s->gW_encT, s->gb_enc,
                                                                      s->m_dec, s->v_dec, s->m_enc, s->v_enc, s->m_be, s->v_be, s->fired,
                                                                      s->since_fired, s->act_freq, (const SaeScalars*)s->scalars, h,
                                                                      F, d, s->renorm_decoder, s->enc_norm_max)));
diff --git a/vit-prisma_b200/csrc/sae_fused.cu b/vit-prisma_b200/csrc/sae_fused.cu
--- a/vit-prisma_b200/csrc/sae_fused.cu
+++ b/vit-prisma_b200/csrc/sae_fused.cu
@@ -14,7 +14,6 @@
 constexpr int FZ_SEG = 128;
 constexpr int FZ_BM = 128;
 constexpr int FZ_BN = 2 * FZ_SEG;
-constexpr int FZ_BK = 32;
 constexpr int FZ_KSTEPS = 4;
 constexpr int FZ_A_BYTES = FZ_BM * 128;
 constexpr int FZ_STAGE_BYTES = FZ_A_BYTES + FZ_BN * 128;
@@ -48,10 +47,11 @@
   key_merge8(v, v + 16);
 }
 
-template <int C_KEEP>
+template <int C_KEEP, typename T>
 __global__ void __launch_bounds__(TC_THREADS, 1)
 k_enc_cand(const __grid_constant__ CUtensorMap tmA, const __grid_constant__ CUtensorMap tmB, int K, int M, int N,
            const float* __restrict__ bias, int* __restrict__ cand, int num_m_tiles, int num_n_tiles) {
+  constexpr int FZ_BK = 128 / sizeof(T);
   pb_pdl_trigger();
   extern __shared__ uint8_t smem_raw[];
   const uint32_t smem0 = smem_u32(smem_raw);
@@ -111,7 +111,10 @@
       const uint32_t sb = ring + s * FZ_STAGE_BYTES + FZ_A_BYTES;
       wgmma_fence();
 #pragma unroll
-      for (int k = 0; k < FZ_KSTEPS; ++k) wgmma_tf32_n256(acc, make_smem_desc(sa + 32 * k), make_smem_desc(sb + 32 * k), (kb | k) != 0 ? 1u : 0u);
+      for (int k = 0; k < FZ_KSTEPS; ++k) {
+        if constexpr (sizeof(T) == 2) wgmma_f16_n256(acc, make_smem_desc(sa + 32 * k), make_smem_desc(sb + 32 * k), (kb | k) != 0 ? 1u : 0u);
+        else wgmma_tf32_n256(acc, make_smem_desc(sa + 32 * k), make_smem_desc(sb + 32 * k), (kb | k) != 0 ? 1u : 0u);
+      }
       wgmma_commit();
       wgmma_wait<1>();
       if (prev_s >= 0 && tid == 0) mbar_arrive(empty_bar(prev_s));
@@ -201,7 +204,8 @@
 template <int SPT>
 __global__ void __launch_bounds__(256) k_cand_select(const int* __restrict__ cand, int nseg, int c_keep, const float* __restrict__ sae_in,
                                                      const float* __restrict__ W_encT, const float* __restrict__ b_enc,
-                                                     const float* __restrict__ wnorm_max, float err_scale, int d, int k, int m_cand,
+                                                     const float* __restrict__ wnorm_max, const float* __restrict__ wlo_max, int f16,
+                                                     float acc_units, float err_scale, int d, int k, int m_cand,
                                                      int* __restrict__ out_idx, float* __restrict__ out_val, float* __restrict__ feat_count,
                                                      int* __restrict__ fb_count, int* __restrict__ fb_rows, int* __restrict__ stats) {
   pb_pdl();
@@ -226,8 +230,13 @@
       const float4 v = src[i];
       dst[i] = v;
       nsq += v.x * v.x + v.y * v.y + v.z * v.z + v.w * v.w;
-      const float lx = v.x - tf32_trunc(v.x), ly = v.y - tf32_trunc(v.y), lz = v.z - tf32_trunc(v.z), lw = v.w - tf32_trunc(v.w);
-      lsq += lx * lx + ly * ly + lz * lz + lw * lw;
+      if (f16) {
+        const float q[4] = {v.x, v.y, v.z, v.w};
+        f16x4(q, lsq);
+      } else {
+        const float lx = v.x - tf32_trunc(v.x), ly = v.y - tf32_trunc(v.y), lz = v.z - tf32_trunc(v.z), lw = v.w - tf32_trunc(v.w);
+        lsq += lx * lx + ly * ly + lz * lz + lw * lw;
+      }
     }
     nsq = warp_sum(nsq);
     lsq = warp_sum(lsq);
@@ -367,8 +376,8 @@
       const int u_rest = m_cur < G ? sel_key(items[m_cur]) : u_below;
       const int u = max(u_rest, sat_key);
       const float u_val = u == INT_MIN ? -INFINITY : ord2f((u & ~127) | 127);
-      const float acc_err = (float)((d + 7) / 8) * 4.76837158e-7f * a_norm * wnorm_max[0];
-      const float E = err_scale * (a_lo_norm * wnorm_max[0] + a_norm * wnorm_max[1]) + acc_err + fabsf(tau_exact) * 1.2207031e-4f;
+      const float acc_err = acc_units * 1.19209290e-7f * a_norm * wnorm_max[0];
+      const float E = err_scale * (a_lo_norm * wnorm_max[0] + a_norm * wlo_max[0]) + acc_err + fabsf(tau_exact) * 1.2207031e-4f;
       ok = !overflow && m_cur >= k && (u_val + E < tau_exact);
     }
     if (ok || m_cur >= Gs) break;
@@ -478,12 +487,29 @@
   }
 }
 
-template <int C_KEEP>
+__global__ void __launch_bounds__(256) k_f16_copy(const float* __restrict__ W, int64_t rows, int d, __half* __restrict__ W16, float* __restrict__ lo_max) {
+  const int lane = threadIdx.x & 31, warp = threadIdx.x >> 5, nw = blockDim.x >> 5;
+  const int nvec = d >> 2;
+  float best = 0.f;
+  for (int64_t r = (int64_t)blockIdx.x * nw + warp; r < rows; r += (int64_t)gridDim.x * nw) {
+    float l = 0.f;
+    for (int i = lane; i < nvec; i += 32) {
+      float v[4];
+      ld4(W + r * d + 4 * i, v);
+      *reinterpret_cast<uint2*>(W16 + r * d + 4 * i) = f16x4(v, l);
+    }
+    best = fmaxf(best, warp_sum(l));
+  }
+  if (lo_max && lane == 0 && best > 0.f) atomicMax(reinterpret_cast<unsigned int*>(lo_max), __float_as_uint(sqrtf(best)));
+}
+
+template <int C_KEEP, typename T>
 int launch_enc_cand(const PbSaeEncode* e, cudaStream_t st) {
+  constexpr bool F16 = sizeof(T) == 2;
   CUtensorMap tmA, tmB;
-  PB_TRY(make_map(&tmA, e->sae_in, PB_F32, e->rows, e->d, e->d, FZ_BM));
-  PB_TRY(make_map(&tmB, e->W_encT, PB_F32, e->F, e->d, e->d, FZ_BN));
-  auto kern = k_enc_cand<C_KEEP>;
+  PB_TRY(make_map(&tmA, F16 ? e->sae_in16 : (const void*)e->sae_in, F16 ? PB_F16 : PB_F32, e->rows, e->d, e->d, FZ_BM));
+  PB_TRY(make_map(&tmB, F16 ? e->W_encT16 : (const void*)e->W_encT, F16 ? PB_F16 : PB_F32, e->F, e->d, e->d, FZ_BN));
+  auto kern = k_enc_cand<C_KEEP, T>;
   static bool attr_done = false;
   if (!attr_done) {
     PB_CUDA(cudaFuncSetAttribute(kern, cudaFuncAttributeMaxDynamicSharedMemorySize, FZ_SMEM));
@@ -497,10 +523,12 @@
 }
 
 template <int SPT>
-int launch_select(const PbSaeEncode* e, int nseg, float scale, cudaStream_t st) {
+int launch_select(const PbSaeEncode* e, bool f16, int nseg, float scale, cudaStream_t st) {
   const size_t smem = sizeof(float) * e->d;
-  PB_LAUNCH_PDL(k_cand_select<SPT>, e->rows, 256, smem, st, (const int*)e->cand, nseg, e->c_keep, e->sae_in, e->W_encT, e->b_enc, e->enc_norm_max, scale,
-                e->d, e->k, e->m_cand, e->idx, e->val, e->feat_count, e->fb_count, e->fb_rows, e->fb_count + 1);
+  const float acc_units = f16 ? 8.f * (float)((e->d + 15) / 16) : 4.f * (float)((e->d + 7) / 8);
+  PB_LAUNCH_PDL(k_cand_select<SPT>, e->rows, 256, smem, st, (const int*)e->cand, nseg, e->c_keep, e->sae_in, e->W_encT, e->b_enc, e->enc_norm_max,
+                f16 ? e->enc16_lo_max : e->enc_norm_max + 1, (int)f16, acc_units, scale, e->d, e->k, e->m_cand, e->idx, e->val, e->feat_count,
+                e->fb_count, e->fb_rows, e->fb_count + 1);
   return PB_OK;
 }
 
@@ -527,21 +555,32 @@
   const int nkeys = e->F / FZ_SEG * e->c_keep;
   PB_CHECK_ARG(e->F / FZ_SEG <= 256 * 4, "pb_sae_encode_topk_fused: d_sae=%d too large for the selection kernel (max 131072)", e->F);
   PB_CHECK_ARG(e->cand_bytes >= (int64_t)e->rows * nkeys * 4, "pb_sae_encode_topk_fused: candidate buffer too small");
+  const bool f16 = e->sae_in16 != nullptr;
+  PB_CHECK_ARG(f16 == (e->W_encT16 != nullptr) && f16 == (e->enc16_lo_max != nullptr),
+               "pb_sae_encode_topk_fused: sae_in16, W_encT16 and enc16_lo_max go together");
+  PB_CHECK_ARG(!f16 || (e->d % 8 == 0 && pb_aligned16(e->sae_in16) && pb_aligned16(e->W_encT16)),
+               "pb_sae_encode_topk_fused: the fp16 candidate GEMM needs d_in %% 8 == 0 and 16-byte aligned fp16 operands (d=%d)", e->d);
   if (e->rows == 0) return PB_OK;
   cudaStream_t st = (cudaStream_t)stream;
   const int phases = (e->phases & 7) ? e->phases : (e->phases | 7);
   if (phases & 1) {
-    if (e->c_keep == 4) PB_TRY(launch_enc_cand<4>(e, st));
-    else if (e->c_keep == 6) PB_TRY(launch_enc_cand<6>(e, st));
-    else PB_TRY(launch_enc_cand<8>(e, st));
+    if (f16) {
+      if (e->c_keep == 4) PB_TRY((launch_enc_cand<4, __half>(e, st)));
+      else if (e->c_keep == 6) PB_TRY((launch_enc_cand<6, __half>(e, st)));
+      else PB_TRY((launch_enc_cand<8, __half>(e, st)));
+    } else {
+      if (e->c_keep == 4) PB_TRY((launch_enc_cand<4, float>(e, st)));
+      else if (e->c_keep == 6) PB_TRY((launch_enc_cand<6, float>(e, st)));
+      else PB_TRY((launch_enc_cand<8, float>(e, st)));
+    }
   }
   if (phases & 2) {
     if (!(phases & 8)) PB_CUDA(cudaMemsetAsync(e->fb_count, 0, 2 * sizeof(int), st));
     const float coef = e->err_coef > 0.f ? e->err_coef : 1.05f;
     const int nseg = e->F / FZ_SEG, spt = (nseg + 255) / 256;
-    if (spt <= 1) PB_TRY(launch_select<1>(e, nseg, coef, st));
-    else if (spt <= 2) PB_TRY(launch_select<2>(e, nseg, coef, st));
-    else PB_TRY(launch_select<4>(e, nseg, coef, st));
+    if (spt <= 1) PB_TRY(launch_select<1>(e, f16, nseg, coef, st));
+    else if (spt <= 2) PB_TRY(launch_select<2>(e, f16, nseg, coef, st));
+    else PB_TRY(launch_select<4>(e, f16, nseg, coef, st));
   }
   if (phases & 4) {
     PB_CHECK_ARG(e->fb_scratch && e->fb_scratch_bytes >= (int64_t)e->F * 4, "pb_sae_encode_topk_fused: fallback scratch missing");
@@ -574,4 +613,16 @@
   return PB_OK;
 }
 
+extern "C" int pb_f16_copy(const float* W, int64_t rows, int32_t d, void* W16, float* lo_max, pb_stream_t stream) {
+  PB_CHECK_ARG(W && W16 && rows >= 0 && d > 0 && d % 4 == 0 && pb_aligned16(W) && ((uintptr_t)W16 & 7) == 0, "pb_f16_copy: bad arguments");
+  cudaStream_t st = (cudaStream_t)stream;
+  if (lo_max) PB_CUDA(cudaMemsetAsync(lo_max, 0, sizeof(float), st));
+  if (rows == 0) return PB_OK;
+  int64_t grid = (rows + 7) / 8;
+  if (grid > pb_sm_count() * 4) grid = pb_sm_count() * 4;
+  k_f16_copy<<<(int)grid, 256, 0, st>>>(W, rows, d, (__half*)W16, lo_max);
+  PB_LAUNCH_CHECK();
+  return PB_OK;
+}
+
 int pb_abi_sizeof_fused(int which) { return which == 9 ? (int)sizeof(PbSaeEncode) : -1; }
diff --git a/vit-prisma_b200/csrc/sae_optim.cuh b/vit-prisma_b200/csrc/sae_optim.cuh
--- a/vit-prisma_b200/csrc/sae_optim.cuh
+++ b/vit-prisma_b200/csrc/sae_optim.cuh
@@ -56,7 +56,7 @@
 template <int CHUNKS, class Out>
 __device__ __forceinline__ void sae_adam_feature(const float* wd, const float* gd, float* md, float* vd, const float* we, const float* ge,
                                                  float* me, float* ve, float clip, const AdamHyper& h, int nvec, bool renorm,
-                                                 const Out& out, float& esq, float& elo) {
+                                                 const Out& out, float& esq, float& elo, float& e16) {
   const int lane = threadIdx.x & 31;
   float w[CHUNKS][4], gq[CHUNKS][4];
   float par = 0.f;
@@ -104,6 +104,7 @@
   }
   esq = 0.f;
   elo = 0.f;
+  e16 = 0.f;
 #pragma unroll
   for (int i = 0; i < CHUNKS; ++i) {
     const int c4 = i * 32 + lane;
@@ -123,7 +124,7 @@
       }
       st4(me + 4 * c4, mm);
       st4(ve + 4 * c4, vv);
-      out.enc(c4, p, lo);
+      out.enc(c4, p, lo, f16x4(p, e16));
     }
   }
 }
diff --git a/vit-prisma_b200/csrc/tc_common.cuh b/vit-prisma_b200/csrc/tc_common.cuh
--- a/vit-prisma_b200/csrc/tc_common.cuh
+++ b/vit-prisma_b200/csrc/tc_common.cuh
@@ -72,6 +72,15 @@
       : PB_ACC128_OUT
       : "l"(adesc), "l"(bdesc), "r"(accumulate));
 }
+__device__ __forceinline__ void wgmma_f16_n256(float (&d)[128], uint64_t adesc, uint64_t bdesc, uint32_t accumulate) {
+  asm volatile(
+      "{\n\t.reg .pred p;\n\tsetp.ne.b32 p, %130, 0;\n\t"
+      "wgmma.mma_async.sync.aligned.m64n256k16.f32.f16.f16 "
+      "{" PB_ACC128_REGS "}, "
+      "%128, %129, p, 1, 1, 0, 0;\n\t}"
+      : PB_ACC128_OUT
+      : "l"(adesc), "l"(bdesc), "r"(accumulate));
+}
 __device__ __forceinline__ void wgmma_bf16_n128(float (&d)[64], uint64_t adesc, uint64_t bdesc, uint32_t accumulate) {
   asm volatile(
       "{\n\t.reg .pred p;\n\tsetp.ne.b32 p, %66, 0;\n\t"
@@ -133,12 +142,14 @@
 int make_map(CUtensorMap* map, const void* ptr, int dtype, int64_t rows, int64_t cols, int64_t ld, int box_rows) {
   EncodeTiledFn fn = get_encode_fn();
   if (!fn) { pb_set_error("gemm_tc: cuTensorMapEncodeTiled entry point unavailable"); return PB_ECUDA; }
-  const int es = dtype == PB_BF16 ? 2 : 4;
+  const int es = dtype == PB_F32 ? 4 : 2;
   cuuint64_t gdim[2] = {(cuuint64_t)cols, (cuuint64_t)rows};
   cuuint64_t gstride[1] = {(cuuint64_t)ld * es};
   cuuint32_t box[2] = {(cuuint32_t)(128 / es), (cuuint32_t)box_rows};
   cuuint32_t estr[2] = {1, 1};
-  CUresult rc = fn(map, dtype == PB_BF16 ? CU_TENSOR_MAP_DATA_TYPE_BFLOAT16 : CU_TENSOR_MAP_DATA_TYPE_FLOAT32, 2, const_cast<void*>(ptr), gdim,
+  const CUtensorMapDataType dt = dtype == PB_BF16 ? CU_TENSOR_MAP_DATA_TYPE_BFLOAT16
+                                 : dtype == PB_F16 ? CU_TENSOR_MAP_DATA_TYPE_FLOAT16 : CU_TENSOR_MAP_DATA_TYPE_FLOAT32;
+  CUresult rc = fn(map, dt, 2, const_cast<void*>(ptr), gdim,
                    gstride, box, estr, CU_TENSOR_MAP_INTERLEAVE_NONE, CU_TENSOR_MAP_SWIZZLE_128B, CU_TENSOR_MAP_L2_PROMOTION_L2_256B,
                    CU_TENSOR_MAP_FLOAT_OOB_FILL_NONE);
   if (rc != CUDA_SUCCESS) {
diff --git a/vit-prisma_b200/vit_prisma/b200/sae_engine.py b/vit-prisma_b200/vit_prisma/b200/sae_engine.py
--- a/vit-prisma_b200/vit_prisma/b200/sae_engine.py
+++ b/vit-prisma_b200/vit_prisma/b200/sae_engine.py
@@ -26,6 +26,7 @@
             "fired", "scalars", "m_dec", "v_dec", "m_enc", "v_enc", "m_be", "v_be", "m_bd", "v_bd",
             "since_fired", "act_freq")]
         + [("global_rows", i32), ("dist", i32), ("work", vp), ("work_bytes", i64), ("enc_norm_max", vp), ("pre_zeroed", i32)]
+        + [("W_encT16", vp), ("enc16_lo_max", vp)]
     )
 
 
@@ -34,12 +35,15 @@
         [(n, i32) for n in ("rows", "d", "F", "k", "c_keep", "m_cand", "phases")] + [("err_coef", f32)]
         + [(n, vp) for n in ("sae_in", "W_encT", "b_enc", "enc_norm_max", "cand")] + [("cand_bytes", i64)]
         + [(n, vp) for n in ("idx", "val", "feat_count", "fb_count", "fb_rows", "fb_scratch")] + [("fb_scratch_bytes", i64)]
+        + [(n, vp) for n in ("sae_in16", "W_encT16", "enc16_lo_max")]
     )
 
 
 L.ABI_STRUCTS.append(PbSaeStep)
 L.register_signatures({
     "pb_sae_prep": (i32, [vp, vp, vp, vp, vp, vp, vp, i32, i32, i32, vp]),
+    "pb_sae_prep16": (i32, [vp, vp, vp, vp, vp, vp, vp, i32, i32, i32, vp]),
+    "pb_f16_copy": (i32, [vp, i64, i32, vp, vp, vp]),
     "pb_sae_topk": (i32, [vp, i32, i32, i32, vp, vp, vp, vp, i64, vp]),
     "pb_sae_scatter_acts": (i32, [vp, vp, vp, i32, i32, i32, i32, vp]),
     "pb_sae_step_reset": (i32, [C.POINTER(PbSaeStep), vp, vp]),
@@ -133,16 +137,21 @@
         dev = W_dec.device
         z = lambda *s, dt=torch.float32: torch.zeros(*s, dtype=dt, device=dev)
         fused_ok = self.d % 4 == 0 and self.d >= 32 and self.F % 128 == 0 and self.k <= 48 and self.F <= 131072
+        f16_ok = encoder == "auto" and self.d % 8 == 0 and self.d >= 64 and not self.is_data_parallel
         if encoder == "auto":
             encoder = "fused" if (fused_ok and gemm_impl == L.GEMM_AUTO) else "dense"
         if encoder == "fused" and not fused_ok:
             raise L.PrismaB200Error(f"fused encoder->TopK needs d_in % 4 == 0, d_sae % 128 == 0, k <= 48 (d={self.d} F={self.F} k={self.k})")
+        self.cand_operands = ("f16" if f16_ok else "tf32") if encoder == "fused" else None
         import os
         self.encoder, self.c_keep = encoder, int(os.environ.get("PRISMA_SAE_C_KEEP", c_keep))
         self.m_cand = int(os.environ.get("PRISMA_SAE_M_CAND", 0)) or (int(m_cand) if m_cand else self.k + 8)
         self.enc_norm_max = z(2)
         self.fb_count = z(2, dt=torch.int32)
         self.W_encT_lo = torch.empty_like(W_encT) if encoder == "dense" else None
+        f16 = self.cand_operands == "f16"
+        self.W_encT16 = torch.empty(self.F, self.d, dtype=torch.float16, device=dev) if f16 else None
+        self.enc16_lo_max = z(1) if f16 else None
         self.refresh_lo()
         self.m_dec, self.v_dec, self.m_enc, self.v_enc = z(self.F, self.d), z(self.F, self.d), z(self.F, self.d), z(self.F, self.d)
         self.m_be, self.v_be, self.m_bd, self.v_bd = z(self.F), z(self.F), z(self.d), z(self.d)
@@ -160,6 +169,9 @@
             from . import ops
             self.W_encT_lo.copy_(ops.split_tf32(self.W_encT))
         L.check(L.get_lib().pb_rownorm_max(self.W_encT.data_ptr(), self.F, self.d, self.enc_norm_max.data_ptr(), _stream()), "pb_rownorm_max")
+        if self.W_encT16 is not None:
+            L.check(L.get_lib().pb_f16_copy(self.W_encT.data_ptr(), self.F, self.d, self.W_encT16.data_ptr(), self.enc16_lo_max.data_ptr(),
+                                            _stream()), "pb_f16_copy")
 
     def _ensure_rows(self, rows: int) -> None:
         if rows == self._rows:
@@ -175,6 +187,7 @@
             self.fb_rows = e(max(rows, 1), dt=torch.int32)
             self.fb_scratch = e(min(64, max(sb.value // (4 * F), 1)) * F)
             self.sae_in_lo = self.hidden_pre = None
+            self.sae_in16 = e(rows, d, dt=torch.float16) if self.cand_operands == "f16" else None
         else:
             self.sae_in_lo, self.hidden_pre = e(rows, d), e(rows, F)
         self.idx, self.val, self.dval = e(rows, k, dt=torch.int32), e(rows, k), e(rows, k)
@@ -203,6 +216,7 @@
         s.since_fired, s.act_freq = p(since_fired), p(act_freq)
         s.work, s.work_bytes = p(self.work), self.work.numel()
         s.enc_norm_max = p(self.enc_norm_max)
+        s.W_encT16, s.enc16_lo_max = p(self.W_encT16), p(self.enc16_lo_max)
         return s
 
     def _enc_desc(self, rows: int, phases: int = 0) -> PbSaeEncode:
@@ -213,6 +227,8 @@
         e.idx, e.val, e.feat_count = self.idx.data_ptr(), self.val.data_ptr(), self.feat_count.data_ptr()
         e.fb_count, e.fb_rows = self.fb_count.data_ptr(), self.fb_rows.data_ptr()
         e.fb_scratch, e.fb_scratch_bytes = self.fb_scratch.data_ptr(), self.fb_scratch.numel() * 4
+        if self.cand_operands == "f16":
+            e.sae_in16, e.W_encT16, e.enc16_lo_max = self.sae_in16.data_ptr(), self.W_encT16.data_ptr(), self.enc16_lo_max.data_ptr()
         return e
 
     def _encoder_gemm(self, rows: int) -> None:
@@ -230,10 +246,14 @@
         lib, st = L.get_lib(), _stream()
         rows = x.shape[0]
         self._ensure_rows(rows)
-        L.check(lib.pb_sae_prep(x.data_ptr(), self.b_dec.data_ptr(), self.sae_in.data_ptr(),
-                                self.sae_in_lo.data_ptr() if (self.sae_in_lo is not None and self.gemm_impl != L.GEMM_SIMT) else None,
-                                self.mu.data_ptr(), self.sd.data_ptr(),
-                                self.xsum.data_ptr(), rows, self.d, self.norm_mode, st), "pb_sae_prep")
+        if self.cand_operands == "f16":
+            L.check(lib.pb_sae_prep16(x.data_ptr(), self.b_dec.data_ptr(), self.sae_in.data_ptr(), self.sae_in16.data_ptr(), self.mu.data_ptr(),
+                                      self.sd.data_ptr(), self.xsum.data_ptr(), rows, self.d, self.norm_mode, st), "pb_sae_prep16")
+        else:
+            L.check(lib.pb_sae_prep(x.data_ptr(), self.b_dec.data_ptr(), self.sae_in.data_ptr(),
+                                    self.sae_in_lo.data_ptr() if (self.sae_in_lo is not None and self.gemm_impl != L.GEMM_SIMT) else None,
+                                    self.mu.data_ptr(), self.sd.data_ptr(),
+                                    self.xsum.data_ptr(), rows, self.d, self.norm_mode, st), "pb_sae_prep")
         if not pre_zeroed:
             self.feat_count.zero_()
         if self.encoder == "fused":
@@ -274,7 +294,8 @@
 
     def describe_encoder(self) -> str:
         if self.encoder == "fused":
-            return (f"fused: one-pass tf32 wgmma GEMM with top-{self.c_keep}-per-128-features epilogue -> exact fp32 re-scoring of "
+            ops_ = "fp16 copies of the operands" if self.cand_operands == "f16" else "tf32"
+            return (f"fused: one-pass wgmma GEMM ({ops_}) with top-{self.c_keep}-per-128-features epilogue -> exact fp32 re-scoring of "
                     f">= {self.m_cand} candidates per token -> exact top-{self.k} with a completeness proof (no dense hidden_pre)")
         return "wgmma 3xTF32 GEMM -> dense hidden_pre -> exact k_topk" if self.gemm_impl != L.GEMM_SIMT else "exact FFMA GEMM -> k_topk"
 
@@ -288,8 +309,9 @@
     def _optimizer_stages(self, s: PbSaeStep, x: torch.Tensor, lr: float, since_fired, act_freq):
         lib, st = L.get_lib(), _stream()
         kernel = "k_sae_adam_rows" if self.W_encT_lo is not None or self.d < 64 else "k_sae_adam_bulk"
+        f16_copy = 2 * self.d * self.F if self.W_encT16 is not None else 0
         return [("adam (clip + decoder-parallel-gradient removal + Adam + row renorm)", lambda: L.check(lib.pb_sae_adam(C.byref(s), st)),
-                 dict(bytes=60 * self.d * self.F, ncu=kernel))]
+                 dict(bytes=60 * self.d * self.F + f16_copy, ncu=kernel))]
 
     def _clip_and_adam(self, x: torch.Tensor, lr: float, since_fired, act_freq, grads, extra) -> None:
         lib, st = L.get_lib(), _stream()
@@ -346,11 +368,12 @@
             self.encode_topk(x)
             flops = 2.0 * rows * self.d * self.F
             nkeys = (self.F // 128) * self.c_keep
-            return [("encode + topk, fused (prep + tf32 candidate GEMM + select / exact re-score + exact path)", lambda: self.encode_topk(x),
+            op, es = ("fp16", 2) if self.cand_operands == "f16" else ("tf32", 4)
+            return [(f"encode + topk, fused (prep + {op} candidate GEMM + select / exact re-score + exact path)", lambda: self.encode_topk(x),
                      dict(flops=flops, passes=1)),
-                    ("candidate GEMM alone (one tf32 pass, top-c-per-segment epilogue)",
+                    (f"candidate GEMM alone (one {op} pass, top-c-per-segment epilogue)",
                      lambda: L.check(lib.pb_sae_encode_topk_fused(C.byref(self._enc_desc(rows, 1)), st)),
-                     dict(flops=flops, passes=1, bytes=4 * self.d * self.F + 4 * rows * self.d + 4 * rows * nkeys, ncu=r"k_enc_cand")),
+                     dict(flops=flops, passes=1, bytes=es * self.d * self.F + es * rows * self.d + 4 * rows * nkeys, ncu=r"k_enc_cand")),
                     ("select + exact re-score alone", lambda: L.check(lib.pb_sae_encode_topk_fused(C.byref(self._enc_desc(rows, 2)), st)),
                      dict(bytes=4 * rows * nkeys + 4 * rows * self.d + 8 * rows * self.k, ncu=r"k_cand_select"))]
         return [("encode + topk (prep + encoder GEMM 3xTF32 + exact topk)", lambda: self.encode_topk(x),
```

New measurement: 2.947 million (median of 6 runs). 15.0% higher.
